# Drexubery/ViewCrafter

Measured on AMD Instinct MI355X. Metric: DDIM steps/sec (576x1024x25f latent 25x72x128, CFG 7.5, 50-step schedule), higher is better.
Workload: dtype f16; 1 GPU; ViewCrafter_25_576x1024x25; trajectories_per_gpu=1, frames=25, parallelism=trajectory-sharded x1 (no in-step collective)

## Files before the change

### include/vcx.h

```cpp
#ifndef VCX_H
#define VCX_H

#include <stddef.h>
#include <stdint.h>

#ifdef __cplusplus
extern "C" {
#endif

#define VCX_OK 0
#define VCX_EINVAL (-1)
#define VCX_ELAUNCH (-2)
#define VCX_ENODEV (-3)

#define VCX_ABI_VERSION 18

int vcx_abi_version(void);
const char* vcx_last_error(void);
int vcx_device_arch(char* name_host, int len);

#define VCX_GEMM_BIAS_N 0x1
#define VCX_GEMM_BIAS_M 0x2
#define VCX_GEMM_ROWADD 0x4
#define VCX_GEMM_RESIDUAL 0x8
#define VCX_GEMM_GEGLU 0x10
#define VCX_GEMM_OUT_F32 0x20
#define VCX_GEMM_CONV_SLABK 0x40
#define VCX_GEMM_LNFOLD 0x80
#define VCX_GEMM_LNFOLD_T 0x100
#define VCX_GEMM_COLSTATS 0x200
#define VCX_GEMM_ROWSTATS 0x400
#define VCX_GEMM_MXFP8_OUT 0x800

typedef struct vcx_gemm_desc {
    size_t struct_size;
    const void* A;
    const void* W;
    void* C;
    const float* bias;
    const float* rowadd;
    const void* residual;
    int64_t lda;
    int32_t M, N, K;
    int32_t ldw, ldc, ldr;
    int32_t mode;
    int32_t in_h, in_w, out_h, out_w, cin, kh, kw, stride, pad_h, pad_w, ups;
    int32_t rowadd_div;
    int32_t flags;
    float alpha;
    const float* ln_stats;
    const float* ln_colsum;
    float* colstats;
    int64_t ldcs;
    float* rowstats;
    float rowstats_eps;
    int32_t rowadd_ld;
    const void* tail_a0;
    const void* tail_a1;
    int64_t tail_lda0;
    int64_t tail_lda1;
    int32_t tail_k0;
    int32_t tail_k1;
} vcx_gemm_desc;

int vcx_gemm_f16(const vcx_gemm_desc* desc_host, void* stream);
int vcx_gemm_units_f16(const vcx_gemm_desc* desc_host, int unit_rows, int64_t w_unit_stride, int64_t bias_unit_stride, void* stream);

enum {
    VCX_ROUTE_REFUSED = 0,
    VCX_ROUTE_REGISTER = 1,
    VCX_ROUTE_TILED = 2,
    VCX_ROUTE_WS320 = 3,
    VCX_ROUTE_WS320_GEGLU = 4,
    VCX_ROUTE_WS320_LNF = 5,
    VCX_ROUTE_UNITS_WS320 = 6,
    VCX_ROUTE_UNITS_GROUPED = 7,
    VCX_ROUTE_UNITS_LOOP = 8
};
int vcx_gemm_route(const vcx_gemm_desc* desc_host, int unit_rows);

size_t vcx_groupnorm_ws_bytes(int n_outer, int64_t pixels, int groups);
int vcx_groupnorm_stats_f16(const void* x, float* stats, void* ws, int n_outer, int64_t pixels,
                            int C, int groups, void* stream);
int vcx_groupnorm_apply_f16(const void* x, void* y, const float* stats, const float* gamma,
                            const float* beta, int n_outer, int64_t pixels, int C, int groups,
                            float eps, int silu, void* stream);
int vcx_groupnorm_apply2_f16(const void* x1, int c1, const void* x2, void* y, const float* stats, const float* gamma, const float* beta,
                             int n_outer, int64_t pixels, int C, int groups, float eps, int silu, void* stream);
int vcx_groupnorm_stats_from_colstats_f32(const float* colstats, float* stats, void* ws, int n_outer, int64_t pixels, int C,
                                          int groups, void* stream);

int vcx_groupnorm_fold_linear_f16(const float* W, const float* bias, const float* gamma, const float* beta, const float* stats,
                                  void* Wn, float* bn, int n_outer, int N, int C, int groups, float eps, void* stream);

int vcx_rowstats_f16(const void* x, float* stats, int64_t rows, int C, float eps, void* stream);
int vcx_layernorm_f16(const void* x, void* y, const float* gamma, const float* beta,
                      int64_t rows, int C, float eps, void* stream);

int vcx_quant_mxfp8_f16(const void* x, int64_t ldx, void* q, void* scales, int64_t rows, int K, void* stream);
int vcx_layernorm_mxfp8_f16(const void* x, void* q, void* scales, const float* gamma, const float* beta, int64_t rows, int C, float eps,
                            void* stream);
int vcx_gemm_mxfp8(const void* a, const void* a_scales, const void* w, const void* w_scales, void* out, void* out_scales, const float* bias,
                   const void* residual, int64_t M, int64_t N, int64_t K, int64_t ldc, int64_t ldr, int flags, void* stream);
int vcx_gemm_mxfp8_ok(int64_t M, int64_t N, int64_t K, int flags);
int vcx_gemm_mxfp8_cfg(int64_t N, int flags, int gather_mode);
int vcx_groupnorm_apply_mxfp8_f16(const void* x, void* q, void* scales, const float* stats, const float* gamma, const float* beta, int n_outer,
                                  int64_t pixels, int C, int groups, float eps, int silu, void* stream);
int vcx_conv_t3_mxfp8(const void* a, const void* a_scales, const void* w, const void* w_scales, void* out, const float* bias, const void* residual,
                      float* colstats, int64_t B, int64_t T, int64_t P, int64_t Cin, int64_t N, int64_t ldc, int64_t ldr, int64_t ldcs, int flags,
                      void* stream);
int vcx_conv_t3_mxfp8_ok(int64_t B, int64_t T, int64_t P, int64_t Cin, int64_t N, int64_t ldc, int64_t ldr, int64_t ldcs, int64_t colstats_col,
                         int flags);
int vcx_groupnorm_apply2_mxfp8_f16(const void* x1, int c1, const void* x2, void* q, void* scales, const float* stats, const float* gamma,
                                   const float* beta, int n_outer, int64_t pixels, int C, int groups, float eps, int silu, void* stream);
// ... 109 lines not shown
```

### viewcrafter_amd/_lib.py

```python
import ctypes
import os
from ctypes import c_char_p, c_double, c_float, c_int, c_int32, c_int64, c_void_p, POINTER

_HERE = os.path.dirname(os.path.abspath(__file__))
LIB_PATH = os.path.join(_HERE, "libvcx.so")

SYMBOLS = [
    "vcx_abi_version", "vcx_last_error", "vcx_device_arch", "vcx_gemm_f16", "vcx_gemm_units_f16", "vcx_gemm_route", "vcx_quant_mxfp8_f16", "vcx_layernorm_mxfp8_f16", "vcx_gemm_mxfp8", "vcx_gemm_mxfp8_ok", "vcx_gemm_mxfp8_cfg",
    "vcx_groupnorm_apply_mxfp8_f16", "vcx_conv_t3_mxfp8", "vcx_conv_t3_mxfp8_ok",
    "vcx_groupnorm_apply2_mxfp8_f16", "vcx_conv3x3_mxfp8", "vcx_conv3x3_mxfp8_ok",
    "vcx_groupnorm_apply_mxfp8_raw_f16", "vcx_groupnorm_apply2_mxfp8_raw_f16", "vcx_conv3x3_tail_mxfp8", "vcx_conv3x3_tail_mxfp8_ok",
    "vcx_groupnorm_ws_bytes", "vcx_groupnorm_stats_f16", "vcx_groupnorm_apply_f16", "vcx_groupnorm_apply2_f16", "vcx_groupnorm_stats_from_colstats_f32", "vcx_groupnorm_fold_linear_f16", "vcx_layernorm_f16", "vcx_rowstats_f16",
    "vcx_attn_flash_d64_f16", "vcx_attn_flash_d512_f16", "vcx_attn_flash_dual_d64_f16", "vcx_attn_temporal_d64_f16", "vcx_attn_temporal_d64_masked_f16", "vcx_attn_temporal_d64_rel_f16",
    "vcx_attn_temporal_d64_mxfp8", "vcx_attn_temporal_d64_mxfp8_ok", "vcx_attn_flash_d64_mxfp8", "vcx_attn_flash_d64_mxfp8_ok",
    "vcx_attn_flash_dual_d64_mxfp8", "vcx_attn_flash_dual_d64_mxfp8_ok", "vcx_softmax_rows_f16",
    "vcx_silu_f32", "vcx_gelu_f16", "vcx_clip_preprocess_f32", "vcx_add_nchw_f32_to_nhwc_f16", "vcx_timestep_embedding_f32", "vcx_cast_f32_to_f16", "vcx_cast_f16_to_f32",
    "vcx_copy2d_f16", "vcx_avgpool2x2_f16", "vcx_upsample2x_f16", "vcx_ncthw_f32_to_nthwc_f16", "vcx_nthwc_to_ncthw_f32", "vcx_ddim_ws_bytes", "vcx_ddim_step_f32", "vcx_ddim_step3_f32",
    "vcx_dpmpp2m_step_f32", "vcx_profile_begin", "vcx_profile_end", "vcx_tune_set", "vcx_tune_get",
]

EXT_SYMBOLS = ["vcx_layernorm_pool2x2_f16", "vcx_layernorm_pool2x2_ok"]

ABI_VERSION = 18
TUNE = {"GEMM_CFG": (0, -1), "GEMM_DMA": (1, 1), "FLASH_QB": (2, 0), "XATTN_RESIDENT": (3, 1), "FLASH_IMPL": (4, 0), "EXP0": (5, 0),
        "EXP1": (6, 0), "GEMM_WS": (7, 1)}
GEMM_BIAS_N, GEMM_BIAS_M, GEMM_ROWADD, GEMM_RESIDUAL, GEMM_GEGLU, GEMM_OUT_F32, GEMM_CONV_SLABK = 1, 2, 4, 8, 16, 32, 64
GEMM_LNFOLD, GEMM_LNFOLD_T, GEMM_COLSTATS, GEMM_ROWSTATS, GEMM_MXFP8_OUT = 0x80, 0x100, 0x200, 0x400, 0x800
ROUTE_REFUSED, ROUTE_REGISTER, ROUTE_TILED, ROUTE_WS320, ROUTE_WS320_GEGLU, ROUTE_WS320_LNF, ROUTE_UNITS_WS320, ROUTE_UNITS_GROUPED, ROUTE_UNITS_LOOP = range(9)
PROF_FAMILIES = ("gemm", "flash_attn", "temporal_attn", "groupnorm", "layernorm", "elementwise")


class GemmDesc(ctypes.Structure):
    _fields_ = [
        ("struct_size", ctypes.c_size_t),
        ("A", c_void_p), ("W", c_void_p), ("C", c_void_p), ("bias", c_void_p), ("rowadd", c_void_p),
        ("residual", c_void_p), ("lda", c_int64), ("M", c_int32), ("N", c_int32), ("K", c_int32),
        ("ldw", c_int32), ("ldc", c_int32), ("ldr", c_int32), ("mode", c_int32),
        ("in_h", c_int32), ("in_w", c_int32), ("out_h", c_int32), ("out_w", c_int32), ("cin", c_int32),
        ("kh", c_int32), ("kw", c_int32), ("stride", c_int32), ("pad_h", c_int32), ("pad_w", c_int32),
        ("ups", c_int32), ("rowadd_div", c_int32), ("flags", c_int32), ("alpha", c_float),
        ("ln_stats", c_void_p), ("ln_colsum", c_void_p), ("colstats", c_void_p), ("ldcs", c_int64),
        ("rowstats", c_void_p), ("rowstats_eps", c_float), ("rowadd_ld", c_int32),
        ("tail_a0", c_void_p), ("tail_a1", c_void_p), ("tail_lda0", c_int64), ("tail_lda1", c_int64), ("tail_k0", c_int32), ("tail_k1", c_int32),
    ]

    def __init__(self, *args, **kw):
        super().__init__(*args, **kw)
        self.struct_size = ctypes.sizeof(GemmDesc)


_lib = None


class VcxError(RuntimeError):
    pass


def lib():
    global _lib
    if _lib is not None:
        return _lib
    if not os.path.exists(LIB_PATH):
        raise VcxError(
            f"{LIB_PATH} not found: build it with `make -C viewcrafter_amd/csrc` "
            "(or `python -c 'import __graft_entry__ as g; g.build()'`). There is no fallback path.")
    import torch
    L = ctypes.CDLL(LIB_PATH)
    L.vcx_abi_version.restype = c_int
    L.vcx_last_error.restype = c_char_p
    L.vcx_device_arch.argtypes = [c_char_p, c_int]
    L.vcx_gemm_f16.argtypes = [POINTER(GemmDesc), c_void_p]
    L.vcx_gemm_units_f16.argtypes = [POINTER(GemmDesc), c_int, c_int64, c_int64, c_void_p]
    L.vcx_gemm_route.argtypes = [POINTER(GemmDesc), c_int]
    L.vcx_quant_mxfp8_f16.argtypes = [c_void_p, c_int64, c_void_p, c_void_p, c_int64, c_int, c_void_p]
    L.vcx_layernorm_mxfp8_f16.argtypes = [c_void_p, c_void_p, c_void_p, c_void_p, c_void_p, c_int64, c_int, c_float, c_void_p]
    L.vcx_gemm_mxfp8.argtypes = [c_void_p, c_void_p, c_void_p, c_void_p, c_void_p, c_void_p, c_void_p, c_void_p, c_int64, c_int64, c_int64, c_int64,
                                 c_int64, c_int, c_void_p]
    L.vcx_gemm_mxfp8_ok.argtypes = [c_int64, c_int64, c_int64, c_int]
    L.vcx_gemm_mxfp8_cfg.argtypes = [c_int64, c_int, c_int]
    L.vcx_groupnorm_apply_mxfp8_f16.argtypes = [c_void_p, c_void_p, c_void_p, c_void_p, c_void_p, c_void_p, c_int, c_int64, c_int, c_int, c_float, c_int, c_void_p]
    L.vcx_conv_t3_mxfp8.argtypes = [c_void_p, c_void_p, c_void_p, c_void_p, c_void_p, c_void_p, c_void_p, c_void_p, c_int64, c_int64, c_int64, c_int64, c_int64,
                                    c_int64, c_int64, c_int64, c_int, c_void_p]
    L.vcx_conv_t3_mxfp8_ok.argtypes = [c_int64, c_int64, c_int64, c_int64, c_int64, c_int64, c_int64, c_int64, c_int64, c_int]
    L.vcx_groupnorm_apply2_mxfp8_f16.argtypes = [c_void_p, c_int, c_void_p, c_void_p, c_void_p, c_void_p, c_void_p, c_void_p, c_int, c_int64, c_int, c_int, c_float,
                                                 c_int, c_void_p]
    L.vcx_conv3x3_mxfp8.argtypes = [c_void_p, c_void_p, c_void_p, c_void_p, c_void_p, c_void_p, c_void_p, c_void_p, c_void_p, c_int64, c_int64, c_int64, c_int64,
                                    c_int64, c_int64, c_int64, c_int64, c_int64, c_int64, c_int, c_void_p]
    L.vcx_conv3x3_mxfp8_ok.argtypes = [c_int64, c_int64, c_int64, c_int64, c_int64, c_int64, c_int64, c_int64, c_int64, c_int64, c_int]
    L.vcx_groupnorm_apply_mxfp8_raw_f16.argtypes = [c_void_p, c_void_p, c_void_p, c_void_p, c_void_p, c_void_p, c_void_p, c_void_p, c_int, c_int64, c_int, c_int,
                                                    c_float, c_int, c_void_p]
    L.vcx_groupnorm_apply2_mxfp8_raw_f16.argtypes = [c_void_p, c_int, c_void_p, c_void_p, c_void_p, c_void_p, c_void_p, c_void_p, c_void_p, c_void_p, c_int, c_int64,
                                                     c_int, c_int, c_float, c_int, c_void_p]
    L.vcx_conv3x3_tail_mxfp8.argtypes = [c_void_p, c_void_p, c_void_p, c_void_p, c_void_p, c_void_p, c_void_p, c_void_p, c_void_p, c_int64, c_int64, c_int64,
                                         c_int64, c_int64, c_int64, c_int64, c_int64, c_int, c_void_p]
    L.vcx_conv3x3_tail_mxfp8_ok.argtypes = [c_int64, c_int64, c_int64, c_int64, c_int64, c_int64, c_int64, c_int64, c_int64, c_int]
    L.vcx_groupnorm_ws_bytes.argtypes = [c_int, c_int64, c_int]
    L.vcx_groupnorm_stats_f16.argtypes = [c_void_p, c_void_p, c_void_p, c_int, c_int64, c_int, c_int, c_void_p]
    L.vcx_groupnorm_apply_f16.argtypes = [c_void_p, c_void_p, c_void_p, c_void_p, c_void_p, c_int, c_int64, c_int,
                                          c_int, c_float, c_int, c_void_p]
    L.vcx_groupnorm_apply2_f16.argtypes = [c_void_p, c_int, c_void_p, c_void_p, c_void_p, c_void_p, c_void_p, c_int, c_int64, c_int,
                                           c_int, c_float, c_int, c_void_p]
    L.vcx_layernorm_f16.argtypes = [c_void_p, c_void_p, c_void_p, c_void_p, c_int64, c_int, c_float, c_void_p]
    L.vcx_rowstats_f16.argtypes = [c_void_p, c_void_p, c_int64, c_int, c_float, c_void_p]
    L.vcx_groupnorm_stats_from_colstats_f32.argtypes = [c_void_p, c_void_p, c_void_p, c_int, c_int64, c_int, c_int, c_void_p]
    L.vcx_groupnorm_fold_linear_f16.argtypes = [c_void_p, c_void_p, c_void_p, c_void_p, c_void_p, c_void_p, c_void_p, c_int, c_int, c_int, c_int,
                                                c_float, c_void_p]
    L.vcx_attn_flash_d64_f16.argtypes = [c_void_p, c_void_p, c_void_p, c_void_p, c_int, c_int, c_int, c_int, c_int,
                                         c_int, c_int64, c_int64, c_int64, c_int64, c_float, c_int, c_void_p]
    L.vcx_attn_flash_d512_f16.argtypes = [c_void_p, c_void_p, c_void_p, c_void_p, c_int, c_int, c_int, c_int, c_int64, c_int64, c_int64, c_int64, c_float, c_void_p]
    L.vcx_attn_flash_dual_d64_f16.argtypes = [c_void_p, c_void_p, c_void_p, c_void_p, c_void_p, c_void_p, c_int, c_int, c_int,
# ... 65 lines not shown
```

### viewcrafter_amd/csrc/gemm.hip

```cpp
#include "vcx_common.h"

#include "gemm_args.h"
#include <stdarg.h>
#include <stdlib.h>

using namespace vcxgemm;

namespace {

template <int BN, bool CONV, bool GEGLU, bool OUT_F32>
__global__ void __launch_bounds__(NTHREADS, 2) gemm_kernel(GemmArgs p) {
    constexpr int NFRAG = BN / 32;
    constexpr int WROWS = BN / 32;
    extern __shared__ __attribute__((aligned(16))) unsigned char smem_raw[];
    half_t* sX = reinterpret_cast<half_t*>(smem_raw);
    half_t* sW = sX + 2 * BM * BK;

    const int ntiles = p.tiles_m * p.tiles_n;
    const int G = gridDim.x;
    auto tile_coords = [&](int t, int& tm, int& tn) {
        const int q8 = ntiles >> 3, r8 = ntiles & 7;
        const int xcd = t & 7, idx = t >> 3;
        const int vid = (xcd < r8 ? xcd * (q8 + 1) : r8 * (q8 + 1) + (xcd - r8) * q8) + idx;
        tn = vid % p.tiles_n;
// ... 240 lines not shown
                }
                const bool full = (n0 + 4 <= p.N);
                if (full) {
                    if (flags & VCX_GEMM_BIAS_N) {
                        const f4 bv = *reinterpret_cast<const f4*>(p.bias + n0);
#pragma unroll
                        for (int r = 0; r < 4; ++r) v[r] += bv[r];
                    }
                    if (radd) {
                        const f4 rv = *reinterpret_cast<const f4*>(radd + n0);
#pragma unroll
                        for (int r = 0; r < 4; ++r) v[r] += rv[r];
                    }
                    if (flags & VCX_GEMM_RESIDUAL) {
                        const h4 rr = *reinterpret_cast<const h4*>(p.R + (int64_t)m * p.ldr + n0);
#pragma unroll
                        for (int r = 0; r < 4; ++r) v[r] += (float)rr[r];
                    }
                    if (OUT_F32) {
                        float* dst = reinterpret_cast<float*>(p.C) + (int64_t)m * p.ldc + n0;
                        *reinterpret_cast<f4*>(dst) = f4{v[0], v[1], v[2], v[3]};
                    } else {
                        half_t* dst = reinterpret_cast<half_t*>(p.C) + (int64_t)m * p.ldc + n0;
                        *reinterpret_cast<h4*>(dst) = h4{(half_t)v[0], (half_t)v[1], (half_t)v[2], (half_t)v[3]};
                    }
                } else {
                    for (int r = 0; r < 4 && n0 + r < p.N; ++r) {
                        float x = v[r];
                        if (flags & VCX_GEMM_BIAS_N) x += p.bias[n0 + r];
                        if (radd) x += radd[n0 + r];
                        if (flags & VCX_GEMM_RESIDUAL) x += (float)p.R[(int64_t)m * p.ldr + n0 + r];
                        if (OUT_F32)
                            reinterpret_cast<float*>(p.C)[(int64_t)m * p.ldc + n0 + r] = x;
                        else
                            reinterpret_cast<half_t*>(p.C)[(int64_t)m * p.ldc + n0 + r] = (half_t)x;
                    }
                }
            }
        }
    }
            }
#pragma unroll
            for (int a = 0; a < NFRAG; ++a)
#pragma unroll
                for (int b = 0; b < 4; ++b) acc[a][b] = f4{0.f, 0.f, 0.f, 0.f};
        }
        if (more) store_tile(cur ^ 1);
        __syncthreads();
        cur ^= 1;
        if (++ckt == nk) {
            ckt = 0;
            ctile += G;
            if (ctile >= ntiles) break;
            tile_coords(ctile, tile_m, tile_n);
        }
    }
}

}
static int grid_for(int ntiles, int blocks_per_cu, int ncu) {
    const int slots = blocks_per_cu * ncu;
    if (ntiles <= slots) return ntiles;
    const int rounds = (ntiles + slots - 1) / slots;
    int g = (ntiles + rounds - 1) / rounds;
    g = (g + 7) & ~7;
    return g < slots ? g : slots;
}
int vcxgemm::persistent_grid(int ntiles, int blocks_per_cu) {
    static std::atomic<int> cached{0};
    int ncu = cached.load(std::memory_order_relaxed);
    if (ncu == 0) {
        int dev = 0;
        hipDeviceProp_t prop;
        ncu = 256;
        if (hipGetDevice(&dev) == hipSuccess && hipGetDeviceProperties(&prop, dev) == hipSuccess && prop.multiProcessorCount > 0)
            ncu = prop.multiProcessorCount;
        cached.store(ncu, std::memory_order_relaxed);
    }
    return grid_for(ntiles, blocks_per_cu, ncu);
}

struct TileSeg { int cfg, m_begin, rows, grid; };
struct TilePlan { int n; TileSeg seg[2]; float cost; };
enum { EPI_PLAIN = 0, EPI_GEGLU = 1, EPI_PLAIN_ONLY128 = 2, EPI_GEGLU_ONLY128 = 3 };

struct TileCost {
    int tbm, tbn, bpc;
    float k_alone, k_share;
    float e;
};
static const TileCost TILE_COST[7] = {
    {128, 128, 2, 0.66f, 1.14f, 3.2f},
    {128, 160, 2, 0.70f, 1.16f, 2.8f},
    {256, 256, 1, 1.63f, 1.63f, 5.0f},
    {256, 320, 1, 2.05f, 2.05f, 5.4f},
    {64, 128, 2, 0.54f, 0.81f, 1.3f},
    {64, 64, 2, 0.46f, 0.73f, 1.3f},
    {64, 128, 2, 0.57f, 0.67f, 1.6f},
};
constexpr float LAUNCH_COST = 4.0f;

static int seg_tiles(int cfg, int rows, int N, int unit_rows) {
    const TileCost& t = TILE_COST[cfg];
    const int tiles_n = (N + t.tbn - 1) / t.tbn;
    if (unit_rows > 0) return (rows / unit_rows) * ((unit_rows + t.tbm - 1) / t.tbm) * tiles_n;
    return ((rows + t.tbm - 1) / t.tbm) * tiles_n;
}
static TileSeg plan_seg(int cfg, int m_begin, int rows, int N, int ncu, int unit_rows = 0) {
    return TileSeg{cfg, m_begin, rows, grid_for(seg_tiles(cfg, rows, N, unit_rows), TILE_COST[cfg].bpc, ncu)};
}
static float seg_cost(const TileSeg& g, int N, int K, int ncu, int unit_rows = 0) {
    const TileCost& t = TILE_COST[g.cfg];
    const int tiles = seg_tiles(g.cfg, g.rows, N, unit_rows);
    const int per_block = (tiles + g.grid - 1) / g.grid;
    const bool share = g.grid > ncu;
    return LAUNCH_COST + per_block * ((float)(K / BK) * (share ? t.k_share : t.k_alone) + t.e);
}

static TilePlan plan_tiles(int M, int N, int K, int epi, int ncu, int unit_rows = 0) {
    const bool geglu = epi == EPI_GEGLU || epi == EPI_GEGLU_ONLY128;
    const int small = (!geglu && N % 160 == 0) ? 1 : 0;
    const int big_bn = (N % 320 == 0 && !geglu) ? 320 : ((N % 256 == 0 || N >= 1024) ? 256 : 0);
    TilePlan best;
    auto consider = [&](int n, TileSeg a, TileSeg b, bool first) {
        const float c = seg_cost(a, N, K, ncu, unit_rows) + (n == 2 ? seg_cost(b, N, K, ncu, unit_rows) : 0.f);
        if (first || c < best.cost) best = TilePlan{n, {a, b}, c};
    };
    const TileSeg none{0, 0, 0, 0};
    consider(1, plan_seg(small, 0, M, N, ncu, unit_rows), none, true);
    if (!big_bn) return best;
    const int large = big_bn == 320 ? 3 : 2;
    const int tpu = unit_rows > 0 ? (unit_rows + 255) / 256 : 1, step_rows = unit_rows > 0 ? unit_rows : 256;
    const int tiles_m = unit_rows > 0 ? M / unit_rows * tpu : (M + 255) / 256, tiles_n = (N + big_bn - 1) / big_bn;
    const long long tiles = (long long)tiles_m * tiles_n;
    if (tiles < 384) return best;
    consider(1, plan_seg(large, 0, M, N, ncu, unit_rows), none, true);
    int tails[3], ntails = 0;
    tails[ntails++] = small;
    if (epi == EPI_PLAIN) { tails[ntails++] = 4; tails[ntails++] = 5; }
    if (epi == EPI_GEGLU) tails[ntails++] = 6;
    const long long full = tiles / ncu;
    for (long long r = full; r >= 1 && r >= full - 1; --r) {
        const int m1 = (int)(r * ncu / tiles_n / tpu) * step_rows;
        if (m1 <= 0 || m1 >= M) continue;
        for (int i = 0; i < ntails; ++i) consider(2, plan_seg(large, 0, m1, N, ncu, unit_rows), plan_seg(tails[i], m1, M - m1, N, ncu, unit_rows), false);
    }
    return best;
}

static TilePlan forced_plan(int M, int N, int cfg, bool geglu, int ncu) {
    TilePlan p{1, {plan_seg(cfg, 0, M, N, ncu), TileSeg{0, 0, 0, 0}}, 0.f};
    if (cfg == 2 || cfg == 3) {
        const TileCost& t = TILE_COST[cfg];
        const int tiles_n = (N + t.tbn - 1) / t.tbn;
        const long long tiles = (long long)((M + 255) / 256) * tiles_n;
        const long long full = tiles / ncu, rem = tiles % ncu;
        const int m1 = (int)(full * ncu / tiles_n) * 256;
        if (full >= 1 && rem > 0 && rem * 10 < (long long)ncu * 7 && m1 > 0 && m1 < M) {
            p.n = 2;
            p.seg[0] = plan_seg(cfg, 0, m1, N, ncu);
            p.seg[1] = plan_seg((geglu || N % 160 != 0) ? 0 : 1, m1, M - m1, N, ncu);
        }
    }
    return p;
}
namespace {

template <int BN, bool CONV, bool GEGLU, bool OUT_F32>
int launch(const GemmArgs& a, hipStream_t s) {
    constexpr size_t smem = (size_t)2 * (BM + BN) * BK * sizeof(half_t);
    static VcxLdsAttr lds;
    auto kern = gemm_kernel<BN, CONV, GEGLU, OUT_F32>;
    if (!lds.ensure(reinterpret_cast<const void*>(kern), (int)smem, "vcx_gemm_f16")) return VCX_ELAUNCH;
    const int nb = persistent_grid(a.tiles_m * a.tiles_n);
    hipLaunchKernelGGL(kern, dim3(nb), dim3(NTHREADS), smem, s, a);
    return vcx_check_launch("vcx_gemm_f16");
}

template <int BN>
int dispatch(const GemmArgs& a, bool conv, bool geglu, bool f32, hipStream_t s) {
    if (geglu) return conv ? launch<BN, true, true, false>(a, s) : launch<BN, false, true, false>(a, s);
    if (f32) return conv ? launch<BN, true, false, true>(a, s) : launch<BN, false, false, true>(a, s);
    return conv ? launch<BN, true, false, false>(a, s) : launch<BN, false, false, false>(a, s);
}

}



static int validate(const vcx_gemm_desc* d, bool ptrs) {
    VCX_REQUIRE(d != nullptr, "vcx_gemm_f16: null descriptor");
    VCX_REQUIRE(d->struct_size == sizeof(vcx_gemm_desc), "vcx_gemm_f16: descriptor struct_size %zu != %zu (sizeof(vcx_gemm_desc), ABI %d)",
                (size_t)d->struct_size, sizeof(vcx_gemm_desc), VCX_ABI_VERSION);
    VCX_REQUIRE(!ptrs || (d->A && d->W && d->C), "vcx_gemm_f16: null A/W/C");
    VCX_REQUIRE(d->M > 0 && d->N > 0 && d->K > 0, "vcx_gemm_f16: empty problem M=%d N=%d K=%d", d->M, d->N, d->K);
    VCX_REQUIRE(d->K % 8 == 0 && d->ldw % 8 == 0 && d->lda % 8 == 0,
                "vcx_gemm_f16: K (%d), ldw (%d), lda (%lld) must be multiples of 8", d->K, d->ldw, (long long)d->lda);
    VCX_REQUIRE(!ptrs || (((uintptr_t)d->A & 15) == 0 && ((uintptr_t)d->W & 15) == 0 && ((uintptr_t)d->C & 15) == 0),
                "vcx_gemm_f16: A/W/C must be 16-byte aligned");
    const int flags = d->flags;
    VCX_REQUIRE(!ptrs || !(flags & (VCX_GEMM_BIAS_N | VCX_GEMM_BIAS_M)) || d->bias, "vcx_gemm_f16: bias flag without bias");
    VCX_REQUIRE(!(flags & VCX_GEMM_ROWADD) || ((!ptrs || d->rowadd) && d->rowadd_div > 0 && (d->rowadd_ld == 0 || (d->rowadd_ld >= d->N && d->rowadd_ld % 4 == 0))),
                "vcx_gemm_f16: bad rowadd (rowadd_ld must be 0 or a multiple of 4 >= N)");
    VCX_REQUIRE(!ptrs || !(flags & VCX_GEMM_RESIDUAL) || d->residual, "vcx_gemm_f16: residual flag without pointer");
    const bool conv = d->mode == 1;
    const bool geglu = flags & VCX_GEMM_GEGLU;
    const bool f32 = flags & VCX_GEMM_OUT_F32;
    VCX_REQUIRE(!(flags & VCX_GEMM_CONV_SLABK) || (d->mode == 1 && d->cin % 64 == 0),
                "vcx_gemm_f16: VCX_GEMM_CONV_SLABK needs a convolution with cin %% 64 == 0 (cin=%d)", d->cin);
    VCX_REQUIRE(d->mode == 0 || d->mode == 1, "vcx_gemm_f16: unknown mode %d", d->mode);
    VCX_REQUIRE(!(geglu && (f32 || (flags & (VCX_GEMM_ROWADD | VCX_GEMM_RESIDUAL | VCX_GEMM_BIAS_M)))),
                "vcx_gemm_f16: GEGLU combines only with BIAS_N");
    VCX_REQUIRE(!geglu || d->N % 64 == 0, "vcx_gemm_f16: GEGLU needs N %% 64 == 0 (N=%d)", d->N);
    const int lnf = (flags & VCX_GEMM_LNFOLD) ? 1 : (flags & VCX_GEMM_LNFOLD_T) ? 2 : 0;
    if (lnf) {
        VCX_REQUIRE(!((flags & VCX_GEMM_LNFOLD) && (flags & VCX_GEMM_LNFOLD_T)), "vcx_gemm_f16: LNFOLD and LNFOLD_T are exclusive");
        VCX_REQUIRE(!ptrs || (d->ln_stats && d->ln_colsum && ((uintptr_t)d->ln_stats & 15) == 0 && ((uintptr_t)d->ln_colsum & 15) == 0),
                    "vcx_gemm_f16: LNFOLD needs 16-byte aligned ln_stats and ln_colsum");
        VCX_REQUIRE(!conv && !f32 && !(flags & VCX_GEMM_ROWADD), "vcx_gemm_f16: LNFOLD is for linear layers with fp16 output, without ROWADD");
        VCX_REQUIRE(lnf == 1 ? !(flags & VCX_GEMM_BIAS_M) : !(flags & VCX_GEMM_BIAS_N) && !geglu,
                    "vcx_gemm_f16: LNFOLD takes BIAS_N (and GEGLU), LNFOLD_T takes BIAS_M");
        VCX_REQUIRE((lnf == 1 ? d->N : d->M) % 4 == 0 && (lnf == 1 ? d->N : d->M) >= 4, "vcx_gemm_f16: LNFOLD needs the colsum side to be a multiple of 4");
    }
    if (flags & VCX_GEMM_COLSTATS) {
        VCX_REQUIRE(!ptrs || (d->colstats && ((uintptr_t)d->colstats & 15) == 0), "vcx_gemm_f16: COLSTATS needs a 16-byte aligned colstats buffer");
        VCX_REQUIRE(!geglu && !f32 && !lnf && d->M % 64 == 0 && d->N % 8 == 0,
                    "vcx_gemm_f16: COLSTATS is for fp16 outputs (no GEGLU / LNFOLD) with M %% 64 == 0 and N %% 8 == 0 (M=%d N=%d)", d->M, d->N);
        VCX_REQUIRE(d->ldcs == 0 || (d->ldcs >= d->N && d->ldcs % 2 == 0), "vcx_gemm_f16: COLSTATS ldcs (%lld) must be 0 or an even number >= N", (long long)d->ldcs);
    }
    if (conv) {
        VCX_REQUIRE(d->cin > 0 && d->cin % 8 == 0 && d->kh > 0 && d->kw > 0 && d->tail_k0 >= 0 && d->tail_k1 >= 0 &&
                        d->K == d->kh * d->kw * d->cin + d->tail_k0 + d->tail_k1,
                    "vcx_gemm_f16: conv needs cin %% 8 == 0 and K == kh*kw*cin + tail (cin=%d kh=%d kw=%d K=%d tail=%d+%d)", d->cin,
                    d->kh, d->kw, d->K, d->tail_k0, d->tail_k1);
        VCX_REQUIRE(d->out_h > 0 && d->out_w > 0 && d->in_h > 0 && d->in_w > 0 && d->stride > 0 &&
                        (d->ups == 0 || d->ups == 1 || d->ups == 2) && d->M % (d->out_h * d->out_w) == 0,
                    "vcx_gemm_f16: bad conv geometry");
        VCX_REQUIRE(d->ups != 2 || (d->kh == 2 && d->kw == 2 && d->stride == 1 && d->out_h == 2 * d->in_h && d->out_w == 2 * d->in_w && d->tail_k0 + d->tail_k1 == 0),
                    "vcx_gemm_f16: ups = 2 (folded nearest-2x + 3x3) is four 2x2 weight sets on the source grid: kh = kw = 2, stride 1, out = 2 x in, no K tail");
    }
    VCX_REQUIRE(conv || (d->tail_k0 >= 0 && d->tail_k1 >= 0 && d->tail_k0 + d->tail_k1 < d->K),
                "vcx_gemm_f16: a linear K tail needs tail_k >= 0 and K > tail_k0 + tail_k1 (K counts the tail; K=%d tail=%d+%d)", d->K, d->tail_k0, d->tail_k1);
    const int tail = d->tail_k0 + d->tail_k1;
    if (tail) {
        VCX_REQUIRE(d->tail_k0 % 64 == 0 && d->tail_k1 % 64 == 0 && (d->tail_k0 == 0 || ((!ptrs || d->tail_a0) && d->tail_lda0 >= d->tail_k0 && d->tail_lda0 % 8 == 0)) &&
                        (d->tail_k1 == 0 || ((!ptrs || d->tail_a1) && d->tail_lda1 >= d->tail_k1 && d->tail_lda1 % 8 == 0)) && !(d->tail_k0 == 0 && d->tail_k1 != 0),
                    "vcx_gemm_f16: K tail: tail_k %% 64 == 0, sources with tail_lda >= tail_k, tail_lda %% 8 == 0, tail_a0 first (tail=%d+%d)", d->tail_k0, d->tail_k1);
        VCX_REQUIRE((!ptrs || (((uintptr_t)d->tail_a0 | (uintptr_t)d->tail_a1) & 15) == 0) && (!conv || (!geglu && !f32 && !lnf)), "vcx_gemm_f16: K tail: 16-byte aligned sources, fp16 output, no GEGLU / LNFOLD");
    }
    if (!geglu) {
        VCX_REQUIRE(d->N < 4 || d->N % 4 != 0 || d->ldc % 4 == 0, "vcx_gemm_f16: ldc must be a multiple of 4");
        if (flags & VCX_GEMM_RESIDUAL)
            VCX_REQUIRE(d->ldr % 4 == 0 && (!ptrs || ((uintptr_t)d->residual & 7) == 0), "vcx_gemm_f16: residual alignment");
        if ((flags & VCX_GEMM_BIAS_N) && d->N >= 4) VCX_REQUIRE(!ptrs || ((uintptr_t)d->bias & 15) == 0, "vcx_gemm_f16: bias alignment");
        if (flags & VCX_GEMM_ROWADD) VCX_REQUIRE((!ptrs || ((uintptr_t)d->rowadd & 15) == 0) && d->N % 4 == 0, "vcx_gemm_f16: rowadd alignment");
    } else {
        VCX_REQUIRE(d->ldc % 4 == 0, "vcx_gemm_f16: ldc must be a multiple of 4");
    }
    if (flags & VCX_GEMM_ROWSTATS)
        VCX_REQUIRE((!ptrs || (d->rowstats && ((uintptr_t)d->rowstats & 7) == 0)) && d->rowstats_eps >= 0.f, "vcx_gemm_f16: ROWSTATS needs an 8-byte aligned rowstats buffer and eps >= 0");
    return VCX_OK;
}

static int validate_units(const vcx_gemm_desc* d, int unit_rows, int64_t w_unit_stride, int64_t bias_unit_stride, bool ptrs) {
    VCX_REQUIRE(d != nullptr && d->struct_size == sizeof(vcx_gemm_desc), "vcx_gemm_units_f16: null descriptor or wrong struct_size");
    VCX_REQUIRE((!ptrs || (d->A && d->W && d->C)) && d->M > 0 && d->N > 0 && d->K > 0, "vcx_gemm_units_f16: null A/W/C or empty problem");
    VCX_REQUIRE(d->mode == 0 && !(d->flags & ~(VCX_GEMM_BIAS_N | VCX_GEMM_ROWSTATS)), "vcx_gemm_units_f16: linear layers with a per-column bias (and ROWSTATS) at most (mode %d flags 0x%x)", d->mode, d->flags);
    VCX_REQUIRE(!(d->flags & VCX_GEMM_ROWSTATS) || ((!ptrs || (d->rowstats && ((uintptr_t)d->rowstats & 7) == 0)) && d->rowstats_eps >= 0.f), "vcx_gemm_units_f16: ROWSTATS needs an 8-byte aligned rowstats buffer and eps >= 0");
    VCX_REQUIRE(unit_rows > 0 && d->M % unit_rows == 0, "vcx_gemm_units_f16: M (%d) must be a whole number of units of %d rows", d->M, unit_rows);
    VCX_REQUIRE(w_unit_stride % 8 == 0 && bias_unit_stride % 4 == 0, "vcx_gemm_units_f16: unit strides must keep W 16-byte and bias 16-byte aligned");
    VCX_REQUIRE(!ptrs || !(d->flags & VCX_GEMM_BIAS_N) || d->bias, "vcx_gemm_units_f16: bias flag without bias");
    VCX_REQUIRE(d->lda % 8 == 0 && d->ldw % 8 == 0 && d->ldc % 8 == 0 && (!ptrs || ((((uintptr_t)d->A | (uintptr_t)d->W | (uintptr_t)d->C) & 15) == 0 && ((uintptr_t)d->bias & 15) == 0)),
                "vcx_gemm_units_f16: strides must be multiples of 8, pointers 16-byte aligned");
    return VCX_OK;
}

struct Knobs { int dma, ws, cfg; bool units_loop; };
static Knobs read_knobs(int unit_rows) {
    const char* loop_env = unit_rows > 0 ? getenv("VCX_GEMM_UNITS_LOOP") : nullptr;
    return Knobs{vcx_tune(VCX_TUNE_GEMM_DMA), vcx_tune(VCX_TUNE_GEMM_WS), vcx_tune(VCX_TUNE_GEMM_CFG), loop_env && loop_env[0] && loop_env[0] != '0'};
}

struct GemmRoute {
    int kind;
    int epi;
    bool ups_folded;
    unsigned long long a_bytes, w_bytes, c_bytes, r_bytes, a2_bytes, a3_bytes;
    char why[384];
};
static GemmRoute& take(GemmRoute& r, int kind) { r.kind = kind; return r; }
static GemmRoute& refuse(GemmRoute& r, const char* fmt, ...) {
    va_list ap;
    va_start(ap, fmt);
    vsnprintf(r.why, sizeof(r.why), fmt, ap);
    va_end(ap);
    return take(r, VCX_ROUTE_REFUSED);
}

static GemmRoute gemm_route(const vcx_gemm_desc& d, int unit_rows, const Knobs& k) {
    GemmRoute r;
    r.why[0] = 0;
    r.ups_folded = false;
    const int flags = d.flags;
    const bool conv = d.mode == 1, geglu = flags & VCX_GEMM_GEGLU, f32 = flags & VCX_GEMM_OUT_F32;
    const int lnf = (flags & VCX_GEMM_LNFOLD) ? 1 : (flags & VCX_GEMM_LNFOLD_T) ? 2 : 0;
    const int k2 = d.tail_k0, k3 = d.tail_k1;
    r.epi = geglu ? (conv ? EPI_GEGLU_ONLY128 : EPI_GEGLU) : ((f32 || lnf == 2) ? EPI_PLAIN_ONLY128 : EPI_PLAIN);
    const unsigned long long lim = 0xFFFF0000ull;
    r.a_bytes = conv ? 2ull * (unsigned long long)(d.M / (d.out_h * d.out_w)) * d.in_h * d.in_w * d.lda
                     : 2ull * ((unsigned long long)(d.M - 1) * d.lda + (d.K - k2 - k3));
    r.w_bytes = 2ull * ((unsigned long long)(d.N - 1) * d.ldw + d.K);
    const unsigned long long esz = f32 ? 4 : 2;
    r.c_bytes = esz * ((unsigned long long)(d.M - 1) * d.ldc + (geglu ? d.N / 2 : d.N));
    r.r_bytes = d.residual ? 2ull * ((unsigned long long)(d.M - 1) * d.ldr + d.N) : 0;
    const bool c_ok = esz * (unsigned long long)(d.M + 256) * d.ldc < lim;
    const bool out_ok = c_ok && 2ull * (unsigned long long)(d.M + 256) * d.ldr < lim;
    r.a2_bytes = k2 ? 2ull * ((unsigned long long)(d.M - 1) * d.tail_lda0 + k2) : 0;
    r.a3_bytes = k3 ? 2ull * ((unsigned long long)(d.M - 1) * d.tail_lda1 + k3) : 0;
    const bool dma_ok = k.dma != 0 && d.K % 64 == 0 && d.N % ((geglu || f32) ? 4 : 8) == 0 && (!conv || d.cin % 64 == 0) &&
                        r.a_bytes < lim && r.w_bytes < lim && (!geglu || d.N >= 64) && out_ok && r.a2_bytes < lim && r.a3_bytes < lim;
    const bool force_cfg_unset = k.cfg < 0;

    const int units = unit_rows > 0 ? d.M / unit_rows : 1;
    if (unit_rows > 0 && (k2 || k3)) return refuse(r, "vcx_gemm_units_f16: no K tail (tail_k0 / tail_k1) with per-unit weights");
    if (units > 1) {
        if (d.K == 320 && d.N == 320 && unit_rows % 32 == 0 && unit_rows >= 1024 && d.M >= 8192 && r.a_bytes < lim && c_ok && units <= 65535 &&
            k.dma != 0 && k.ws != 0 && force_cfg_unset)
            return take(r, VCX_ROUTE_UNITS_WS320);
        if (flags & VCX_GEMM_ROWSTATS)
            return refuse(r, "vcx_gemm_units_f16: ROWSTATS needs the one-launch weight-stationary form (N = K = 320, unit_rows %% 32 == 0, >= 1024, M >= 8192); M=%d N=%d K=%d unit_rows=%d",
                          d.M, d.N, d.K, unit_rows);
        if (units <= 65535 && d.K % 64 == 0 && d.N % 8 == 0 && r.a_bytes < lim && r.w_bytes < lim && c_ok && k.dma != 0 && k.cfg <= 5 && !k.units_loop) {
            vcx_gemm_desc one = d;
            one.M = unit_rows;
            if (gemm_route(one, 0, k).kind != VCX_ROUTE_WS320) return take(r, VCX_ROUTE_UNITS_GROUPED);
        }
        return take(r, VCX_ROUTE_UNITS_LOOP);
    }

    if (conv && d.ups == 2) {
        const long long hw = (long long)d.in_h * d.in_w;
        if (dma_ok && d.in_w % 16 == 0 && hw % 64 == 0 && d.cin % 64 == 0 && d.N % 8 == 0 && (flags & VCX_GEMM_CONV_SLABK) &&
            !(flags & ~(VCX_GEMM_CONV_SLABK | VCX_GEMM_BIAS_N | VCX_GEMM_COLSTATS)) && d.alpha == 1.0f && k.cfg <= 3 && 4ull * r.w_bytes < lim &&
            (unsigned long long)d.N * d.ldw * 2ull * 3ull + r.w_bytes < lim) {
            r.ups_folded = true;
            r.epi = EPI_PLAIN_ONLY128;
            return take(r, VCX_ROUTE_TILED);
        }
        return refuse(r, "vcx_gemm_f16: the folded upsample convolution (ups = 2) needs in_w %% 16 == 0, in_h in_w %% 64 == 0, cin %% 64 == 0, N %% 8 == 0, slab-major K, "
                         "a bias / column-moment epilogue, extents < 4 GiB, and GEMM_CFG <= 3; in %dx%d cin=%d N=%d flags=0x%x", d.in_h, d.in_w, d.cin, d.N, flags);
    }
    if ((k2 || k3) && !dma_ok)
        return refuse(r, "vcx_gemm_f16: a K tail needs the DMA kernel (cin %% 64 == 0, K %% 64 == 0, N %% 8 == 0, extents < 4 GiB); cin=%d K=%d N=%d", d.cin, d.K, d.N);
    if (!conv && (k2 || k3)) {
        if (geglu || f32 || lnf || (flags & VCX_GEMM_ROWSTATS))
            return refuse(r, "vcx_gemm_f16: a linear K tail takes the plain and COLSTATS epilogues only: no GEGLU / LNFOLD / ROWSTATS / fp32 output; flags=0x%x", flags);
        if (k.cfg > 5) return refuse(r, "vcx_gemm_f16: tile configuration %d (knob GEMM_CFG) has no K tail in linear mode", k.cfg);
        return take(r, VCX_ROUTE_TILED);
    }
    if (dma_ok && !conv && geglu && !f32 && !lnf && d.K == 320 && d.N % 256 == 0 && d.N <= 2560 && !(flags & ~(VCX_GEMM_GEGLU | VCX_GEMM_BIAS_N)) &&
        d.alpha == 1.0f && ((k.ws | 2) == 3 || k.ws == 5) && force_cfg_unset)
        return take(r, VCX_ROUTE_WS320_GEGLU);
    const int pad = (d.N + 255) / 256 * 256 - d.N;
    if (dma_ok && !conv && !geglu && !f32 && lnf == 1 && d.K == 320 && d.N % 64 == 0 && d.N <= 2560 &&
        ((k.ws >= 1 && k.ws <= 3 && pad <= 64 && d.N >= 512 && d.N <= 1536) || k.ws == 5) &&
        !(flags & ~(VCX_GEMM_LNFOLD | VCX_GEMM_BIAS_N)) && 8ull * (unsigned long long)d.M < lim && force_cfg_unset)
        return take(r, VCX_ROUTE_WS320_LNF);
    const bool rs_ok = !(flags & VCX_GEMM_ROWSTATS) || (d.N == 320 && !(flags & ~(VCX_GEMM_ROWSTATS | VCX_GEMM_BIAS_N | VCX_GEMM_RESIDUAL)) && 8ull * (unsigned long long)d.M < lim);
    if (dma_ok && !conv && !geglu && !f32 && !lnf && d.K == 320 && d.N % 320 == 0 && d.N <= 1280 && d.M >= 8192 && rs_ok &&
        !(flags & VCX_GEMM_BIAS_M) && k.ws != 0 && force_cfg_unset)
        return take(r, VCX_ROUTE_WS320);
    if (flags & VCX_GEMM_ROWSTATS)
        return refuse(r, "vcx_gemm_f16: ROWSTATS needs the weight-stationary kernel (linear, N = K = 320, M >= 8192, BIAS_N / RESIDUAL at most, knob GEMM_WS on); M=%d N=%d K=%d flags=0x%x",
                      d.M, d.N, d.K, flags);
    if (dma_ok) {
        if (k.cfg > 6) return refuse(r, "vcx_gemm_f16: unknown tile configuration %d (knob GEMM_CFG)", k.cfg);
        return take(r, VCX_ROUTE_TILED);
    }
    if (flags & VCX_GEMM_COLSTATS)
        return refuse(r, "vcx_gemm_f16: COLSTATS needs the DMA kernel (K / cin %% 64 == 0, extents < 4 GiB); K=%d cin=%d", d.K, d.cin);
    if (lnf) return refuse(r, "vcx_gemm_f16: LNFOLD needs the DMA kernel (K %% 64 == 0, N %% 8 == 0, extents < 4 GiB); K=%d N=%d", d.K, d.N);
    return take(r, VCX_ROUTE_REGISTER);
}

static GemmArgs fill_args(const vcx_gemm_desc& d, const GemmRoute& r, int unit_rows, int64_t w_unit_stride, int64_t bias_unit_stride) {
    GemmArgs a;
    a.A = (const half_t*)d.A; a.W = (const half_t*)d.W; a.C = d.C; a.bias = d.bias; a.rowadd = d.rowadd; a.R = (const half_t*)d.residual;
    a.lda = d.lda; a.M = d.M; a.N = d.N; a.K = d.K; a.ldw = d.ldw; a.ldc = d.ldc; a.ldr = d.ldr;
    a.in_h = d.in_h; a.in_w = d.in_w; a.out_h = d.out_h; a.out_w = d.out_w;
    a.cin = d.cin; a.kh = d.kh; a.kw = d.kw; a.stride = d.stride; a.pad_h = d.pad_h; a.pad_w = d.pad_w; a.ups = d.ups;
    a.rowadd_div = d.rowadd_div > 0 ? d.rowadd_div : 1;
    a.rowadd_ld = d.rowadd_ld > 0 ? d.rowadd_ld : d.N;
    a.flags = d.flags; a.alpha = d.alpha; a.m_begin = 0;
    const int bn = (!(d.flags & VCX_GEMM_GEGLU) && d.N % 160 == 0) ? 160 : 128;
    a.tiles_m = (d.M + BM - 1) / BM;
    a.tiles_n = (d.N + bn - 1) / bn;
    a.ln_stats = d.ln_stats; a.ln_colsum = d.ln_colsum; a.colstats = d.colstats; a.ldcs = d.ldcs > 0 ? d.ldcs : d.N;
    a.unit_rows = unit_rows; a.units = unit_rows > 0 ? d.M / unit_rows : 1; a.w_unit_stride = w_unit_stride; a.bias_unit_stride = bias_unit_stride;
    a.rowstats = d.rowstats; a.rowstats_eps = d.rowstats_eps;
    a.A2 = (const half_t*)d.tail_a0; a.A3 = (const half_t*)d.tail_a1; a.lda2 = d.tail_lda0; a.lda3 = d.tail_lda1;
    a.k2 = d.tail_k0; a.k3 = d.tail_k1;
    a.a_bytes = (unsigned)r.a_bytes; a.w_bytes = (unsigned)r.w_bytes; a.c_bytes = (unsigned)r.c_bytes; a.r_bytes = (unsigned)r.r_bytes;
    a.a2_bytes = (unsigned)r.a2_bytes; a.a3_bytes = (unsigned)r.a3_bytes;
    return a;
}

static TilePlan tile_plan(const vcx_gemm_desc& d, const GemmRoute& r, int force, int unit_rows) {
    const int ncu = persistent_grid(1 << 30, 1);
    const bool geglu = d.flags & VCX_GEMM_GEGLU;
    if (force < 0) return plan_tiles(d.M, d.N, d.K, r.epi, ncu, unit_rows);
    if (unit_rows > 0) return TilePlan{1, {plan_seg(force, 0, d.M, d.N, ncu, unit_rows), TileSeg{0, 0, 0, 0}}, 0.f};
    if (!(geglu && (force == 1 || force == 3))) return forced_plan(d.M, d.N, force, geglu, ncu);
    int cfg = 0;
    if ((d.N % 256 == 0 || d.N >= 1024) && (long long)((d.M + 255) / 256) * ((d.N + 255) / 256) >= 384) cfg = 2;
    return forced_plan(d.M, d.N, cfg, geglu, ncu);
}

static int run_plan(const GemmArgs& a, const TilePlan& plan, bool conv, hipStream_t s) {
    const bool trace = getenv("VCX_GEMM_PLAN_TRACE") != nullptr;
    for (int i = 0; i < plan.n; ++i) {
        const TileSeg& g = plan.seg[i];
        const TileCost& t = TILE_COST[g.cfg];
        const int u0 = a.unit_rows > 0 ? g.m_begin / a.unit_rows : 0, nu = a.unit_rows > 0 ? g.rows / a.unit_rows : 0;
        if (trace) {
            char per_unit[64] = "";
            if (a.unit_rows > 0) snprintf(per_unit, sizeof(per_unit), " units %d unit_rows %d", nu, a.unit_rows);
            fprintf(stderr, "[vcx] gemm plan M=%d N=%d K=%d seg %d/%d: cfg %d rows %d+%d grid %d%s\n", a.M, a.N, a.K, i + 1, plan.n, g.cfg, g.m_begin, g.rows, g.grid, per_unit);
        }
        GemmArgs c = a;
        c.m_begin = g.m_begin;
        c.M = g.m_begin + g.rows;
        c.tiles_m = a.unit_rows > 0 ? nu * ((a.unit_rows + t.tbm - 1) / t.tbm) : (g.rows + t.tbm - 1) / t.tbm;
        c.tiles_n = (a.N + t.tbn - 1) / t.tbn;
        if (a.unit_rows > 0) {
            c.units = nu;
            c.W = a.W + (int64_t)u0 * a.w_unit_stride;
            if (a.bias) c.bias = a.bias + (int64_t)u0 * a.bias_unit_stride;
        }
        const int rc = launch_dma(c, g.cfg, conv, a.flags & VCX_GEMM_GEGLU, a.flags & VCX_GEMM_OUT_F32, s, g.grid);
        if (rc) return rc;
    }
    return VCX_OK;
}

static int run(const vcx_gemm_desc& d, const GemmRoute& r, const Knobs& k, int unit_rows, int64_t w_unit_stride, int64_t bias_unit_stride, void* stream) {
    if (r.kind == VCX_ROUTE_REFUSED) {
        vcx_set_error("%s", r.why);
        return VCX_EINVAL;
    }
    if (unit_rows > 0 && r.kind != VCX_ROUTE_UNITS_WS320 && r.kind != VCX_ROUTE_UNITS_GROUPED) {
        for (int u = 0; u < d.M / unit_rows; ++u) {
            vcx_gemm_desc du = d;
            du.A = (const half_t*)d.A + (int64_t)u * unit_rows * d.lda;
            du.C = (half_t*)d.C + (int64_t)u * unit_rows * d.ldc;
            du.W = (const half_t*)d.W + (int64_t)u * w_unit_stride;
            if (d.bias) du.bias = d.bias + (int64_t)u * bias_unit_stride;
            du.M = unit_rows;
// ... 48 lines not shown
```

### viewcrafter_amd/csrc/gemm_dma.hip

```cpp
#include "gemm_epilogue.h"

using namespace vcxgemm;

namespace {

typedef __attribute__((address_space(3))) void* lds_ptr_t;
[[maybe_unused]] constexpr unsigned OOB = 0xFFFFFFFFu;

template <int TBM_, int TBN_, int NWM_, int NWN_>
struct TileCfg {
    static constexpr int TBM = TBM_, TBN = TBN_, NWM = NWM_, NWN = NWN_;
    static constexpr int THREADS = 64 * NWM * NWN;
    static constexpr int MF = TBM / NWM / 16;
    static constexpr int NF = TBN / NWN / 16;
    static constexpr int XROWS = TBM * 8 / THREADS;
    static constexpr int WROWS = TBN * 8 / THREADS;
    static constexpr int RSTEP = THREADS / 8;
    static constexpr size_t STAGES = (size_t)2 * (TBM + TBN) * BK * sizeof(half_t);
    static constexpr size_t STRIP = (size_t)TBN * NWM * sizeof(float);
    static constexpr size_t SMEM = STAGES + STRIP;
    static constexpr size_t SMEM_LNF = STAGES + 2 * STRIP;
};

template <class Cfg, bool CONV, bool GEGLU, bool OUT_F32, int LNF = 0, bool TAIL = false, bool UNITS = false, bool UPSF = false>
// ... 96 lines not shown
        half_t* dx = sX + buf * TBM * BK + wave * 8 * BK;
        half_t* dw = sW + buf * BN * BK + wave * 8 * BK;
        if (TAIL && (parts & 1) && kt >= nk_main) {
            const bool first = kt - nk_main < nk_a2;
            const __amdgpu_buffer_rsrc_t src = first ? srd_a2 : srd_a3;
            const long long ld2 = (first ? p.lda2 : p.lda3) * 2;
            const unsigned soff = (unsigned)(first ? kt - nk_main : kt - nk_main - nk_a2) * (BK * 2);
#pragma unroll
            for (int i = 0; i < XROWS; ++i) {
                const int r = r0 + RSTEP * i;
                const int m = lrow0 + r;
                const unsigned v = m < p.M ? (unsigned)((long long)m * ld2) + (unsigned)(chunk ^ ((r >> 1) & 7)) * 16u : OOB;
                __builtin_amdgcn_raw_ptr_buffer_load_lds(src, (lds_ptr_t)(dx + RSTEP * i * BK), 16, v, soff, 0, 0);
            }
        } else if (CONV && (parts & 1)) {
            if (!UPSF && p.ups) {
                const unsigned cb = (unsigned)ci0 * 2u, rowb = (unsigned)(p.in_w * (int)p.lda * 2), pixb = (unsigned)((int)p.lda * 2);
                const unsigned y0 = (unsigned)(tky >> 1) * rowb, y1 = (unsigned)((tky + 1) >> 1) * rowb;
                const unsigned x0 = (unsigned)(tkx >> 1) * pixb, x1 = (unsigned)((tkx + 1) >> 1) * pixb;
#pragma unroll
                for (int i = 0; i < XROWS; ++i) {
                    const unsigned ok = (xmask[i] >> tap) & 1u;
                    const unsigned oy_ = (xmask[i] >> 31) ? y1 : y0, ox_ = ((xmask[i] >> 30) & 1u) ? x1 : x0;
                    const unsigned v = ok ? xoff[i] + oy_ + ox_ + cb : OOB;
                    __builtin_amdgcn_raw_ptr_buffer_load_lds(srd_a, (lds_ptr_t)(dx + RSTEP * i * BK), 16, v, 0, 0, 0);
                }
            } else if (!(VCX_CONV_XSKIP_ABL && p.kw == 3 && tkx != 0)) {
#pragma unroll
                for (int i = 0; i < XROWS; ++i) {
                    const unsigned ok = (xmask[i] >> tap) & 1u;
                    const unsigned v = ok ? xoff[i] + tap_off : OOB;
                    __builtin_amdgcn_raw_ptr_buffer_load_lds(srd_a, (lds_ptr_t)(dx + RSTEP * i * BK), 16, v, 0, 0, 0);
                }
            }
            if (p.flags & VCX_GEMM_CONV_SLABK) {
                ++tap;
                if (++tkx == p.kw) { tkx = 0; ++tky; }
                if (tap == p.kh * p.kw) { tap = 0; tkx = 0; tky = 0; ci0 += BK; }
                tap_off = (unsigned)((tky * p.in_w + tkx) * (int)p.lda * 2 + ci0 * 2);
            } else {
                ci0 += BK;
                tap_off += BK * 2;
                if (ci0 == p.cin) {
                    ci0 = 0;
                    ++tap;
                    if (++tkx == p.kw) { tkx = 0; ++tky; }
                    tap_off = (unsigned)((tky * p.in_w + tkx) * (int)p.lda * 2);
                }
            }
        } else if (!CONV && (parts & 1)) {
            const unsigned soff = (unsigned)kt * (BK * 2);
#pragma unroll
            for (int i = 0; i < XROWS; ++i)
                __builtin_amdgcn_raw_ptr_buffer_load_lds(srd_a, (lds_ptr_t)(dx + RSTEP * i * BK), 16, xoff[i], soff, 0, 0);
        }
        if (parts & 2) {
            const unsigned soffw = (unsigned)kt * (BK * 2);
#pragma unroll
            for (int i = 0; i < WROWS; ++i)
                __builtin_amdgcn_raw_ptr_buffer_load_lds(PERUNIT ? srd_wu : srd_w, (lds_ptr_t)(dw + RSTEP * i * BK), 16, woff[i], soffw, 0, 0);
        }
    };

    const int wm = wave % Cfg::NWM, wn = wave / Cfg::NWM;
    const int lr = lane & 15, lg = lane >> 4;
    constexpr int WM = TBM / Cfg::NWM, WN = BN / Cfg::NWN;

    f4 acc[NFRAG][MFRAG];
#pragma unroll
    for (int a = 0; a < NFRAG; ++a)
#pragma unroll
        for (int b = 0; b < MFRAG; ++b) acc[a][b] = f4{0.f, 0.f, 0.f, 0.f};

    const int nk = p.K / BK;
    int ltile = blockIdx.x, lkt = 0;
    int ctile = blockIdx.x, ckt = 0;
    int tile_m, tile_n;
    tile_coords(ctile, ntiles, p.tiles_n, tile_m, tile_n);
    init_load(ltile);
    load_tile(0, 0);
    __builtin_amdgcn_s_waitcnt(0x0f70 | 0);
    __syncthreads();
    int cur = 0;
    for (;;) {
        if (++lkt == nk) {
            lkt = 0;
            ltile += G;
            if (ltile < ntiles) init_load(ltile);
        }
        const bool more = ltile < ntiles;
        const int late_parts = (CONV && Cfg::THREADS == 512 && wave >= 4) ? 3 : 0;
        if (more) load_tile(lkt, cur ^ 1, 3 & ~late_parts);
        const half_t* cx = sX + cur * TBM * BK;
        const half_t* cw = sW + cur * BN * BK;
        [[maybe_unused]] float ln_r0[LNF ? MFRAG : 1], ln_r1[LNF ? MFRAG : 1];
        if ((LNF == 1 || LNF == 2) && ckt == nk - 1) {
            const int mrow = p.m_begin + tile_m * TBM + wm * WM + lr;
#pragma unroll
            for (int b = 0; b < MFRAG; ++b) {
                const int mc = min(mrow + b * 16, p.M - 1);
                if (LNF == 1) {
                    const float2 st = reinterpret_cast<const float2*>(p.ln_stats)[mc];
                    ln_r0[b] = st.x;
                    ln_r1[b] = st.y;
                } else {
                    ln_r0[b] = p.ln_colsum[mc];
                    ln_r1[b] = (p.flags & VCX_GEMM_BIAS_M) ? p.bias[mc] : 0.f;
                }
            }
        }
        {
            constexpr bool NOREAD = (VCX_DMA_ABL & 8) != 0;
            h8 xf[MFRAG];
#pragma unroll
            for (int b = 0; b < MFRAG; ++b) xf[b] = *reinterpret_cast<const h8*>(cx + lds_off(wm * WM + b * 16 + lr, lg));
            h8 wcur = *reinterpret_cast<const h8*>(cw + lds_off(wn * WN + lr, lg));
            if (NOREAD) {
#pragma unroll
                for (int b = 0; b < MFRAG; ++b) asm volatile("" : "+v"(xf[b]));
                asm volatile("" : "+v"(wcur));
            }
#pragma unroll
            for (int kk = 0; kk < 2; ++kk) {
                if (kk == 1 && more && late_parts) load_tile(lkt, cur ^ 1, late_parts);
#pragma unroll
                for (int a = 0; a < NFRAG; ++a) {
                    h8 wnext = wcur;
                    if (NOREAD) asm volatile("" : "+v"(wnext));
                    else if (a + 1 < NFRAG) wnext = *reinterpret_cast<const h8*>(cw + lds_off(wn * WN + (a + 1) * 16 + lr, kk * 4 + lg));
                    else if (kk == 0) wnext = *reinterpret_cast<const h8*>(cw + lds_off(wn * WN + lr, 4 + lg));
#pragma unroll
                    for (int b = 0; b < MFRAG; ++b) {
                        acc[a][b] = __builtin_amdgcn_mfma_f32_16x16x32_f16(wcur, xf[b], acc[a][b], 0, 0, 0);
                        if (a == NFRAG - 1 && kk == 0 && !NOREAD)
                            xf[b] = *reinterpret_cast<const h8*>(cx + lds_off(wm * WM + b * 16 + lr, 4 + lg));
                    }
                    wcur = wnext;
                    __builtin_amdgcn_sched_barrier(0);
                }
            }
        }
        if (ckt == nk - 1) {
            float* sB = reinterpret_cast<float*>(smem_raw + Cfg::STAGES) + wave * WN;
            if constexpr (UNITS) {
                int cu, crow0;
                unit_of(tile_m, cu, crow0);
                GemmArgs q = p;
                q.m_begin = crow0;
                q.M = p.m_begin + (cu + 1) * p.unit_rows;
                q.bias = p.bias + (int64_t)cu * p.bias_unit_stride;
                q.c_bytes = (unsigned)(2ull * ((unsigned long long)(q.M - 1) * (unsigned)p.ldc + (unsigned)p.N));
                gemm_epilogue<Cfg, false, false, 0>(q, acc, 0, tile_n, wm, wn, lane, sB);
            } else if constexpr (UPSF) {
                int cu, crow0;
                unit_of(tile_m, cu, crow0);
                gemm_epilogue<Cfg, false, false, LNF, false, true>(p, acc, tile_m, tile_n, wm, wn, lane, sB, nullptr, nullptr, nullptr, nullptr, false, cls0 + cu,
                                                                   crow0 - (p.m_begin + cu * p.unit_rows));
            } else
            gemm_epilogue<Cfg, GEGLU, OUT_F32, LNF>(p, acc, tile_m, tile_n, wm, wn, lane, sB,
                                                    reinterpret_cast<float*>(smem_raw + Cfg::STAGES + Cfg::STRIP) + wave * WN, ln_r0, ln_r1);
#pragma unroll
            for (int a = 0; a < NFRAG; ++a)
#pragma unroll
                for (int b = 0; b < MFRAG; ++b) acc[a][b] = f4{0.f, 0.f, 0.f, 0.f};
        }
        if (!(VCX_DMA_ABL & 16)) {
            __builtin_amdgcn_s_waitcnt(0x0f70 | 0);
            __syncthreads();
        }
        cur ^= 1;
        if (++ckt == nk) {
            ckt = 0;
            ctile += G;
            if (ctile >= ntiles) break;
            tile_coords(ctile, ntiles, p.tiles_n, tile_m, tile_n);
        }
    }
#endif
}

template <class Cfg, bool CONV, bool GEGLU, bool OUT_F32, int LNF = 0, bool TAIL = false, bool UNITS = false, bool UPSF = false>
int launch(const GemmArgs& a, hipStream_t s, int grid) {
    static VcxLdsAttr lds;
    auto kern = gemm_dma_kernel<Cfg, CONV, GEGLU, OUT_F32, LNF, TAIL, UNITS, UPSF>;
    constexpr size_t smem = LNF ? Cfg::SMEM_LNF : Cfg::SMEM;
    if (!lds.ensure(reinterpret_cast<const void*>(kern), (int)smem, "vcx_gemm_f16(dma)")) return VCX_ELAUNCH;
    const int blocks_per_cu = Cfg::SMEM > 80 * 1024 ? 1 : 2;
    const int nb = grid > 0 ? grid : persistent_grid(a.tiles_m * a.tiles_n, blocks_per_cu);
    hipLaunchKernelGGL(kern, dim3(nb), dim3(Cfg::THREADS), smem, s, a, a.a_bytes, a.w_bytes);
    return vcx_check_launch("vcx_gemm_f16(dma)");
}

template <class Cfg>
int dispatch(const GemmArgs& a, bool conv, bool geglu, bool f32, hipStream_t s, int grid) {
    if (a.unit_rows > 0 && conv)
        return (a.flags & VCX_GEMM_COLSTATS) ? launch<Cfg, true, false, false, 3, false, false, true>(a, s, grid) : launch<Cfg, true, false, false, 0, false, false, true>(a, s, grid);
    if (a.unit_rows > 0)
        return launch<Cfg, false, false, false, 0, false, true>(a, s, grid);
    if (a.k2 + a.k3 > 0) {
        if (conv) return (a.flags & VCX_GEMM_COLSTATS) ? launch<Cfg, true, false, false, 3, true>(a, s, grid) : launch<Cfg, true, false, false, 0, true>(a, s, grid);
        return (a.flags & VCX_GEMM_COLSTATS) ? launch<Cfg, false, false, false, 3, true>(a, s, grid) : launch<Cfg, false, false, false, 0, true>(a, s, grid);
    }
    if (a.flags & (VCX_GEMM_LNFOLD | VCX_GEMM_LNFOLD_T)) {
        if (a.flags & VCX_GEMM_LNFOLD_T) return launch<Cfg, false, false, false, 2>(a, s, grid);
        if (!geglu) return launch<Cfg, false, false, false, 1>(a, s, grid);
        if constexpr (Cfg::NF % 4 == 0) return launch<Cfg, false, true, false, 1>(a, s, grid);
        vcx_set_error("vcx_gemm_f16(dma): GEGLU needs whole 64-column packed blocks per wave");
        return VCX_EINVAL;
    }
    if (a.flags & VCX_GEMM_COLSTATS)
        return conv ? launch<Cfg, true, false, false, 3>(a, s, grid) : launch<Cfg, false, false, false, 3>(a, s, grid);
    if (geglu) {
        if constexpr (Cfg::NF % 4 == 0) return conv ? launch<Cfg, true, true, false>(a, s, grid) : launch<Cfg, false, true, false>(a, s, grid);
        vcx_set_error("vcx_gemm_f16(dma): GEGLU needs whole 64-column packed blocks per wave");
        return VCX_EINVAL;
    }
    if (f32) return conv ? launch<Cfg, true, false, true>(a, s, grid) : launch<Cfg, false, false, true>(a, s, grid);
    return conv ? launch<Cfg, true, false, false>(a, s, grid) : launch<Cfg, false, false, false>(a, s, grid);
}

constexpr size_t TAIL_LDS = 54 * 1024;
constexpr size_t CU_LDS = 160 * 1024;
static_assert(2 * TAIL_LDS <= CU_LDS && 3 * TAIL_LDS > CU_LDS, "TAIL_LDS must cap the tail kernels at two blocks per CU");

template <class Cfg, bool CONV, bool GEGLU, int LNF = 0, bool TAIL = false, bool UNITS = false>
int launch_tail(const GemmArgs& a, hipStream_t s, int grid) {
    static VcxLdsAttr lds;
    auto kern = gemm_dma_kernel<Cfg, CONV, GEGLU, false, LNF, TAIL, UNITS>;
    constexpr size_t need = LNF ? Cfg::SMEM_LNF : Cfg::SMEM;
    constexpr size_t smem = need > TAIL_LDS ? need : TAIL_LDS;
    if (!lds.ensure(reinterpret_cast<const void*>(kern), (int)smem, "vcx_gemm_f16(dma tail)")) return VCX_ELAUNCH;
    const int nb = grid > 0 ? grid : persistent_grid(a.tiles_m * a.tiles_n, 2);
    hipLaunchKernelGGL(kern, dim3(nb), dim3(Cfg::THREADS), smem, s, a, a.a_bytes, a.w_bytes);
    return vcx_check_launch("vcx_gemm_f16(dma tail)");
}

template <class Cfg>
int dispatch_tail(const GemmArgs& a, bool conv, bool geglu, bool f32, hipStream_t s, int grid) {
    const bool cs = a.flags & VCX_GEMM_COLSTATS;
    if (f32 || (a.flags & VCX_GEMM_LNFOLD_T)) {
        vcx_set_error("vcx_gemm_f16(dma): the 64-row tile configurations have no fp32-output / LNFOLD_T epilogue");
        return VCX_EINVAL;
    }
    if (a.unit_rows > 0 && conv) {
        vcx_set_error("vcx_gemm_f16(dma): the 64-row tile configurations have no folded-upsample form");
        return VCX_EINVAL;
    }
    if constexpr (Cfg::NF % 4 == 0) {
        if (a.unit_rows > 0) {
            vcx_set_error("vcx_gemm_f16(dma): this 64-row tile configuration has no per-unit weight form");
            return VCX_EINVAL;
        }
        if (geglu && !conv && a.k2 + a.k3 == 0 && !cs)
            return (a.flags & VCX_GEMM_LNFOLD) ? launch_tail<Cfg, false, true, 1>(a, s, grid) : launch_tail<Cfg, false, true>(a, s, grid);
        vcx_set_error("vcx_gemm_f16(dma): this 64-row tile configuration is for GEGLU projections (linear) only");
        return VCX_EINVAL;
    } else {
        static_assert(Cfg::MF == 4, "COLSTATS: one moment strip per 64 rows of a wave");
        if (geglu) {
            vcx_set_error("vcx_gemm_f16(dma): GEGLU needs whole 64-column packed blocks per wave");
            return VCX_EINVAL;
        }
        if (a.unit_rows > 0) return launch_tail<Cfg, false, false, 0, false, true>(a, s, grid);
        if (a.k2 + a.k3 > 0) {
            if (conv) return cs ? launch_tail<Cfg, true, false, 3, true>(a, s, grid) : launch_tail<Cfg, true, false, 0, true>(a, s, grid);
            return cs ? launch_tail<Cfg, false, false, 3, true>(a, s, grid) : launch_tail<Cfg, false, false, 0, true>(a, s, grid);
        }
        if (a.flags & VCX_GEMM_LNFOLD) return launch_tail<Cfg, false, false, 1>(a, s, grid);
        if (cs) return conv ? launch_tail<Cfg, true, false, 3>(a, s, grid) : launch_tail<Cfg, false, false, 3>(a, s, grid);
        return conv ? launch_tail<Cfg, true, false>(a, s, grid) : launch_tail<Cfg, false, false>(a, s, grid);
    }
}

}

int vcxgemm::launch_dma(GemmArgs& a, int cfg, bool conv, bool geglu, bool f32, hipStream_t s, int grid) {
    switch (cfg) {
        case 0: return dispatch<TileCfg<128, 128, 2, 2>>(a, conv, geglu, f32, s, grid);
        case 1: return dispatch<TileCfg<128, 160, 2, 2>>(a, conv, geglu, f32, s, grid);
        case 2: return dispatch<TileCfg<256, 256, 4, 2>>(a, conv, geglu, f32, s, grid);
        case 3: return dispatch<TileCfg<256, 320, 4, 2>>(a, conv, geglu, f32, s, grid);
        case 4: return dispatch_tail<TileCfg<64, 128, 1, 4>>(a, conv, geglu, f32, s, grid);
        case 5: return dispatch_tail<TileCfg<64, 64, 1, 4>>(a, conv, geglu, f32, s, grid);
        case 6: return dispatch_tail<TileCfg<64, 128, 2, 2>>(a, conv, geglu, f32, s, grid);
    }
    vcx_set_error("vcx_gemm_f16(dma): unknown tile configuration %d", cfg);
    return VCX_EINVAL;
}
```

### viewcrafter_amd/csrc/gemm_epilogue.h

```cpp
#pragma once
#include "gemm_args.h"

namespace vcxgemm {

[[maybe_unused]] constexpr unsigned EPI_OOB = 0xFFFFFFFFu;
typedef unsigned epi_u4v __attribute__((ext_vector_type(4)));

template <class Cfg>
__device__ __forceinline__ void gemm_epilogue_fetch_residual(const GemmArgs& p, int tile_m, int tile_n, int wm, int wn, int lane,
                                                             epi_u4v (&out)[(Cfg::NF / 2 + Cfg::NF % 2) * Cfg::MF]) {
    constexpr int WM = Cfg::TBM / Cfg::NWM, WN = Cfg::TBN / Cfg::NWN, NPAIRF = Cfg::NF / 2, UNITS = NPAIRF + Cfg::NF % 2;
    typedef unsigned u2v __attribute__((ext_vector_type(2)));
    const int lr = lane & 15, lg = lane >> 4;
    const unsigned odd = lg & 1, half = lg >> 1;
    const __amdgpu_buffer_rsrc_t srd_r = __builtin_amdgcn_make_buffer_rsrc(const_cast<half_t*>(p.R), 0, (int)p.r_bytes, 0x00020000);
    const int mbase = p.m_begin + tile_m * Cfg::TBM + wm * WM + lr;
    const unsigned roff0 = ((unsigned)mbase * (unsigned)p.ldr + (unsigned)(tile_n * Cfg::TBN + wn * WN)) * 2u;
    const unsigned rstep = 32u * (unsigned)p.ldr;
#pragma unroll
    for (int b = 0; b < Cfg::MF; ++b)
#pragma unroll
        for (int u = 0; u < UNITS; ++u) {
            const int col = u < NPAIRF ? (2 * u + (int)odd) * 16 + (int)half * 8 : (2 * NPAIRF + (u - NPAIRF)) * 16 + lg * 4;
            const unsigned o = roff0 + (unsigned)b * rstep + (unsigned)col * 2u;
            if (u < NPAIRF) out[b * UNITS + u] = __builtin_amdgcn_raw_buffer_load_b128(srd_r, o, 0, 0);
            else {
                const u2v t = __builtin_amdgcn_raw_buffer_load_b64(srd_r, o, 0, 0);
                const unsigned t0 = t[0], t1 = t[1];
                out[b * UNITS + u] = epi_u4v{t0, t1, 0u, 0u};
            }
        }
}

template <class Cfg, bool GEGLU, bool OUT_F32, int LNF = 0, bool RPRE = false, bool UPSF = false>
__device__ __forceinline__ void gemm_epilogue(const GemmArgs& p, f4 (&acc)[Cfg::NF][Cfg::MF], int tile_m, int tile_n, int wm, int wn,
                                              int lane, float* sB, [[maybe_unused]] float* sS = nullptr,
                                              [[maybe_unused]] const float* ln_r0 = nullptr, [[maybe_unused]] const float* ln_r1 = nullptr,
                                              [[maybe_unused]] const epi_u4v* rpre = nullptr,
                                              bool strip_ready = false,
                                              [[maybe_unused]] int ups_cls = 0, [[maybe_unused]] int ups_q0 = 0) {
    constexpr int TBM = Cfg::TBM, BN = Cfg::TBN, NFRAG = Cfg::NF, MFRAG = Cfg::MF;
    constexpr int WM = TBM / Cfg::NWM, WN = BN / Cfg::NWN;
    [[maybe_unused]] constexpr unsigned OOB = EPI_OOB;
    const int lr = lane & 15, lg = lane >> 4;
    const int flags = p.flags;
    const int mbase = p.m_begin + tile_m * TBM + wm * WM + lr;
    const int nbase = tile_n * BN + wn * WN + lg * 4;
    if (GEGLU) {
        auto xfrag = [](int a) { return 4 * (a >> 1) + (a & 1); };
        f4 bx[NFRAG / 2 + 1], bg[NFRAG / 2 + 1];
        [[maybe_unused]] f4 sx[LNF ? NFRAG / 2 + 1 : 1], sg[LNF ? NFRAG / 2 + 1 : 1];
#pragma unroll
        for (int a = 0; a < NFRAG / 2; ++a) {
            const int nx = min(nbase + xfrag(a) * 16, p.N - 36);
            bx[a] = (flags & VCX_GEMM_BIAS_N) ? *reinterpret_cast<const f4*>(p.bias + nx) : f4{0.f, 0.f, 0.f, 0.f};
            bg[a] = (flags & VCX_GEMM_BIAS_N) ? *reinterpret_cast<const f4*>(p.bias + nx + 32) : f4{0.f, 0.f, 0.f, 0.f};
            if (LNF) {
                sx[a] = *reinterpret_cast<const f4*>(p.ln_colsum + nx);
                sg[a] = *reinterpret_cast<const f4*>(p.ln_colsum + nx + 32);
            }
        }
        typedef unsigned u2v __attribute__((ext_vector_type(2)));
        typedef unsigned u4v __attribute__((ext_vector_type(4)));
        const __amdgpu_buffer_rsrc_t srd_c = __builtin_amdgcn_make_buffer_rsrc(p.C, 0, (int)p.c_bytes, 0x00020000);
        constexpr int NOUT = NFRAG / 2;
        const int jstrip = tile_n * (BN / 2) + wn * (WN / 2);
        const unsigned coff0 = ((unsigned)mbase * (unsigned)p.ldc + (unsigned)jstrip) * 2u;
        const unsigned cstep = 32u * (unsigned)p.ldc;
        const unsigned odd = lg & 1, half = lg >> 1;
#pragma unroll
        for (int b = 0; b < MFRAG; ++b) {
            u2v packed[NOUT ? NOUT : 1];
            [[maybe_unused]] float rb = 0.f, qb = 0.f;
            if (LNF) {
                rb = p.alpha * ln_r1[b];
                qb = -rb * ln_r0[b];
            }
#pragma unroll
            for (int a = 0; a < NOUT; ++a) {
                half_t o[4];
#pragma unroll
                for (int r = 0; r < 4; ++r) {
                    float xv, gv;
                    if (LNF) {
                        xv = __builtin_fmaf(acc[xfrag(a)][b][r], rb, __builtin_fmaf(qb, sx[a][r], bx[a][r]));
                        gv = __builtin_fmaf(acc[xfrag(a) + 2][b][r], rb, __builtin_fmaf(qb, sg[a][r], bg[a][r]));
                    } else {
                        xv = acc[xfrag(a)][b][r] * p.alpha + bx[a][r];
                        gv = acc[xfrag(a) + 2][b][r] * p.alpha + bg[a][r];
                    }
                    o[r] = (half_t)(xv * gelu_erf(gv));
                }
                packed[a] = __builtin_bit_cast(u2v, h4{o[0], o[1], o[2], o[3]});
            }
            const unsigned crow = coff0 + (unsigned)b * cstep;
#pragma unroll
            for (int a = 0; a < NOUT; a += 2) {
                if (a + 1 < NOUT) {
                    const unsigned a0 = packed[a][0], a1 = packed[a][1], b0 = packed[a + 1][0], b1 = packed[a + 1][1];
                    const auto s0 = __builtin_amdgcn_permlane16_swap(a0, b0, false, false);
                    const auto s1 = __builtin_amdgcn_permlane16_swap(a1, b1, false, false);
                    const int col = (a + (int)odd) * 16 + (int)half * 8;
                    const int nx = tile_n * BN + wn * WN + xfrag(a + (int)odd) * 16;
                    const unsigned voff = nx + 48 <= p.N ? crow + (unsigned)col * 2u : OOB;
                    __builtin_amdgcn_raw_buffer_store_b128(u4v{s0[0], s1[0], s0[1], s1[1]}, srd_c, voff, 0, 0);
                } else {
                    const int nx = tile_n * BN + wn * WN + xfrag(a) * 16;
                    const unsigned voff = nx + 48 <= p.N ? crow + (unsigned)(a * 16 + lg * 4) * 2u : OOB;
                    __builtin_amdgcn_raw_buffer_store_b64(packed[a], srd_c, voff, 0, 0);
                }
            }
        }
    } else {
        constexpr int ES = OUT_F32 ? 4 : 2;
        const __amdgpu_buffer_rsrc_t srd_c = __builtin_amdgcn_make_buffer_rsrc(p.C, 0, (int)p.c_bytes, 0x00020000);
        const __amdgpu_buffer_rsrc_t srd_r = __builtin_amdgcn_make_buffer_rsrc(const_cast<half_t*>(p.R), 0, (int)p.r_bytes, 0x00020000);
        const unsigned cstep = 16u * (unsigned)p.ldc * ES, rstep = 32u * (unsigned)p.ldr;
        const bool has_res = flags & VCX_GEMM_RESIDUAL;
        const int m_first = p.m_begin + tile_m * TBM;
        const int radd_row = m_first / p.rowadd_div;
        const bool radd_tile = (flags & VCX_GEMM_ROWADD) && (min(m_first + TBM, p.M) - 1) / p.rowadd_div == radd_row;
        const bool per_row = (flags & VCX_GEMM_BIAS_M) || ((flags & VCX_GEMM_ROWADD) && !radd_tile);
        typedef unsigned u2v __attribute__((ext_vector_type(2)));
        typedef unsigned u4v __attribute__((ext_vector_type(4)));
        constexpr int NPAIRF = OUT_F32 ? 0 : NFRAG / 2;
        constexpr int UNITS = NPAIRF + (NFRAG - 2 * NPAIRF);
        constexpr int NUNIT = UNITS * MFRAG;
        constexpr int RDU = RPRE ? NUNIT : UNITS;
        const unsigned odd = lg & 1, half = lg >> 1;
        auto unit_col = [&](int u) { return u < NPAIRF ? (2 * u + (int)odd) * 16 + (int)half * 8 : (2 * NPAIRF + (u - NPAIRF)) * 16 + lg * 4; };
        const int nstrip = tile_n * BN + wn * WN;
        const unsigned coff0 = ((unsigned)mbase * (unsigned)p.ldc + (unsigned)nstrip) * ES;
        const unsigned roff0 = ((unsigned)mbase * (unsigned)p.ldr + (unsigned)nstrip) * 2u;
        u4v rr[RDU];
        auto fetch = [&](int i) {
            const int u = i % UNITS;
            const unsigned o = roff0 + (unsigned)(i / UNITS) * rstep + (unsigned)unit_col(u) * 2u;
            if (u < NPAIRF) rr[i % RDU] = __builtin_amdgcn_raw_buffer_load_b128(srd_r, o, 0, 0);
            else {
                const u2v t = __builtin_amdgcn_raw_buffer_load_b64(srd_r, o, 0, 0);
                const unsigned t0 = t[0], t1 = t[1];
                rr[i % RDU] = u4v{t0, t1, 0u, 0u};
            }
        };
        if (RPRE) {
#pragma unroll
            for (int i = 0; i < RDU; ++i) rr[i] = rpre[i];
        } else if (has_res) {
#pragma unroll
            for (int i = 0; i < RDU; ++i) fetch(i);
        }
        if (lane < WN / 4 && !strip_ready) {
            const int nc = min(nstrip + lane * 4, p.N - 4);
            if (LNF == 2) {
                const f4 s01 = *reinterpret_cast<const f4*>(p.ln_stats + 2 * nc), s23 = *reinterpret_cast<const f4*>(p.ln_stats + 2 * nc + 4);
                f4 cs = {p.alpha * s01[1], p.alpha * s01[3], p.alpha * s23[1], p.alpha * s23[3]};
                f4 cq = {-cs[0] * s01[0], -cs[1] * s01[2], -cs[2] * s23[0], -cs[3] * s23[2]};
                asm volatile("" : "+v"(cs), "+v"(cq));
                *reinterpret_cast<f4*>(sB + lane * 4) = cs;
                *reinterpret_cast<f4*>(sS + lane * 4) = cq;
                asm volatile("" : : "v"(cs), "v"(cq));
            } else {
                f4 t = (flags & VCX_GEMM_BIAS_N) ? *reinterpret_cast<const f4*>(p.bias + nc) : f4{0.f, 0.f, 0.f, 0.f};
                if (radd_tile) {
                    const f4 rv = *reinterpret_cast<const f4*>(p.rowadd + (int64_t)radd_row * p.rowadd_ld + nc);
#pragma unroll
                    for (int r = 0; r < 4; ++r) t[r] += rv[r];
                }
                *reinterpret_cast<f4*>(sB + lane * 4) = t;
                if (LNF == 1) *reinterpret_cast<f4*>(sS + lane * 4) = *reinterpret_cast<const f4*>(p.ln_colsum + nc);
            }
        }
        constexpr bool FOLD = LNF == 1 || LNF == 2;
        [[maybe_unused]] float ln_a[FOLD ? MFRAG : 1], ln_b[FOLD ? MFRAG : 1];
        if (FOLD) {
#pragma unroll
            for (int b = 0; b < MFRAG; ++b) {
                if (LNF == 1) {
                    ln_a[b] = p.alpha * ln_r1[b];
                    ln_b[b] = -ln_a[b] * ln_r0[b];
                } else {
                    ln_a[b] = ln_r0[b];
                    ln_b[b] = ln_r1[b];
                }
            }
        }
        [[maybe_unused]] float gs[LNF == 3 ? UNITS : 1][8], gq[LNF == 3 ? UNITS : 1][8], gk[LNF == 3 ? UNITS : 1][2];
        if (LNF == 3) {
#pragma unroll
            for (int u = 0; u < UNITS; ++u)
#pragma unroll
                for (int e = 0; e < 8; ++e) gs[u][e] = gq[u][e] = 0.f;
        }
        int bopaque = 0;
        auto finish = [&](int a, int b, float (&v)[4]) {
            if (FOLD) {
                const f4 t = *reinterpret_cast<const f4*>(sB + bopaque + a * 16 + lg * 4);
                const f4 u = *reinterpret_cast<const f4*>(sS + bopaque + a * 16 + lg * 4);
                typedef float f2v __attribute__((ext_vector_type(2)));
                f2v la = {ln_a[b], ln_a[b]}, lb = {ln_b[b], ln_b[b]};
                asm volatile("" : "+v"(la), "+v"(lb));
#pragma unroll
                for (int r = 0; r < 4; ++r)
                    v[r] = LNF == 1 ? __builtin_fmaf(acc[a][b][r], la[r & 1], __builtin_fmaf(lb[r & 1], u[r], t[r]))
                                    : __builtin_fmaf(acc[a][b][r], t[r], __builtin_fmaf(u[r], la[r & 1], lb[r & 1]));
            } else if (per_row) {
                const int mc = min(mbase + b * 16, p.M - 1);
                f4 t = *reinterpret_cast<const f4*>(sB + bopaque + a * 16 + lg * 4);
                if (flags & VCX_GEMM_ROWADD) {
                    const f4 rv = *reinterpret_cast<const f4*>(p.rowadd + (int64_t)(mc / p.rowadd_div) * p.rowadd_ld + min(nbase + a * 16, p.N - 4));
#pragma unroll
                    for (int r = 0; r < 4; ++r) t[r] += rv[r];
                }
#pragma unroll
                for (int r = 0; r < 4; ++r) v[r] = __builtin_fmaf(acc[a][b][r], p.alpha, t[r]);
                if (flags & VCX_GEMM_BIAS_M) {
                    const float bm = p.bias[mc];
#pragma unroll
                    for (int r = 0; r < 4; ++r) v[r] += bm;
                }
            } else {
                const f4 t = *reinterpret_cast<const f4*>(sB + bopaque + a * 16 + lg * 4);
#pragma unroll
                for (int r = 0; r < 4; ++r) v[r] = __builtin_fmaf(acc[a][b][r], p.alpha, t[r]);
            }
        };
#pragma unroll
        for (int b = 0; b < MFRAG; ++b) {
            unsigned crow = coff0 + (unsigned)b * cstep;
            [[maybe_unused]] bool fvalid = true;
            if constexpr (UPSF) {
                const int qf = ups_q0 + wm * WM + b * 16;
                const int hw = p.out_h * p.out_w;
                fvalid = qf < p.unit_rows;
                const int qc = fvalid ? qf : 0;
                const int img = qc / hw, rem = qc - img * hw;
                const int i = rem / p.out_w, j0 = rem - i * p.out_w;
                const unsigned pix = ((unsigned)img * 2u * (unsigned)p.out_h + 2u * (unsigned)i + (unsigned)(ups_cls >> 1)) * 2u * (unsigned)p.out_w + 2u * (unsigned)j0 + (unsigned)(ups_cls & 1);
                crow = ((pix + 2u * (unsigned)lr) * (unsigned)p.ldc + (unsigned)nstrip) * ES;
            }
            asm volatile("" : "+v"(bopaque));
#pragma unroll
            for (int u = 0; u < UNITS; ++u) {
                const int i = b * UNITS + u;
                const bool wide = u < NPAIRF;
                const int a = wide ? 2 * u : 2 * NPAIRF + (u - NPAIRF);
                const unsigned voff = (nstrip + unit_col(u) < p.N && (!UPSF || fvalid)) ? crow + (unsigned)unit_col(u) * ES : OOB;
                float v0[4], v1[4] = {0.f, 0.f, 0.f, 0.f};
                finish(a, b, v0);
                if (wide) finish(a + 1, b, v1);
                if (has_res) {
                    const u4v raw = rr[i % RDU];
                    if (i + RDU < NUNIT) fetch(i + RDU);
                    unsigned w0 = raw[0], w1 = raw[1], w2 = raw[2], w3 = raw[3];
                    if (wide) {
                        const auto s0 = __builtin_amdgcn_permlane16_swap(w0, w2, false, false);
                        const auto s1 = __builtin_amdgcn_permlane16_swap(w1, w3, false, false);
                        w0 = s0[0]; w2 = s0[1]; w1 = s1[0]; w3 = s1[1];
                    }
                    const h4 r0 = __builtin_bit_cast(h4, u2v{w0, w1});
                    const h4 r1 = __builtin_bit_cast(h4, u2v{w2, w3});
#pragma unroll
                    for (int r = 0; r < 4; ++r) { v0[r] += (float)r0[r]; v1[r] += (float)r1[r]; }
                }
                [[maybe_unused]] const h4 o0 = {(half_t)v0[0], (half_t)v0[1], (half_t)v0[2], (half_t)v0[3]};
                [[maybe_unused]] const h4 o1 = {(half_t)v1[0], (half_t)v1[1], (half_t)v1[2], (half_t)v1[3]};
                [[maybe_unused]] u2v pk0 = __builtin_bit_cast(u2v, o0), pk1 = __builtin_bit_cast(u2v, o1);
                if (LNF == 3) {
                    unsigned q0 = pk0[0], q1 = pk0[1], q2 = pk1[0], q3 = pk1[1];
                    asm volatile("" : "+v"(q0), "+v"(q1), "+v"(q2), "+v"(q3));
                    pk0 = u2v{q0, q1};
                    pk1 = u2v{q2, q3};
                    typedef _Float16 h2v __attribute__((ext_vector_type(2)));
                    const h2v a01 = __builtin_bit_cast(h2v, q0), a23 = __builtin_bit_cast(h2v, q1);
                    const h2v b01 = __builtin_bit_cast(h2v, q2), b23 = __builtin_bit_cast(h2v, q3);
                    const float w0[4] = {(float)a01[0], (float)a01[1], (float)a23[0], (float)a23[1]};
                    const float w1[4] = {(float)b01[0], (float)b01[1], (float)b23[0], (float)b23[1]};
                    if (b == 0) {
                        gk[u][0] = __builtin_bit_cast(float, __builtin_amdgcn_update_dpp(0, __builtin_bit_cast(int, w0[0]), 0x150, 0xf, 0xf, true));
                        gk[u][1] = __builtin_bit_cast(float, __builtin_amdgcn_update_dpp(0, __builtin_bit_cast(int, w1[0]), 0x150, 0xf, 0xf, true));
                    }
#pragma unroll
                    for (int r = 0; r < 4; ++r) {
                        const float d0 = w0[r] - gk[u][0], d1 = w1[r] - gk[u][1];
                        gs[u][r] += d0;
                        gq[u][r] = __builtin_fmaf(d0, d0, gq[u][r]);
                        gs[u][4 + r] += d1;
                        gq[u][4 + r] = __builtin_fmaf(d1, d1, gq[u][4 + r]);
                    }
                }
                if (OUT_F32) {
                    __builtin_amdgcn_raw_buffer_store_b128(__builtin_bit_cast(u4v, f4{v0[0], v0[1], v0[2], v0[3]}), srd_c, voff, 0, 0);
                } else {
                    const u2v p0 = pk0;
                    if (wide) {
                        const u2v p1 = pk1;
                        const unsigned a0 = p0[0], a1 = p0[1], b0 = p1[0], b1 = p1[1];
                        const auto s0 = __builtin_amdgcn_permlane16_swap(a0, b0, false, false);
                        const auto s1 = __builtin_amdgcn_permlane16_swap(a1, b1, false, false);
                        __builtin_amdgcn_raw_buffer_store_b128(u4v{s0[0], s1[0], s0[1], s1[1]}, srd_c, voff, 0, 0);
                    } else {
                        __builtin_amdgcn_raw_buffer_store_b64(p0, srd_c, voff, 0, 0);
                    }
                }
            }
        }
        if (LNF == 3) {
            auto row_sum = [](float x) {
                x += __builtin_bit_cast(float, __builtin_amdgcn_update_dpp(0, __builtin_bit_cast(int, x), 0x140, 0xf, 0xf, true));
                x += __builtin_bit_cast(float, __builtin_amdgcn_update_dpp(0, __builtin_bit_cast(int, x), 0x141, 0xf, 0xf, true));
                x += __builtin_bit_cast(float, __builtin_amdgcn_update_dpp(0, __builtin_bit_cast(int, x), 0x4E, 0xf, 0xf, true));
                x += __builtin_bit_cast(float, __builtin_amdgcn_update_dpp(0, __builtin_bit_cast(int, x), 0xB1, 0xf, 0xf, true));
                return x;
            };
            int strip = (p.m_begin + tile_m * TBM + wm * WM) >> 6;
            [[maybe_unused]] bool svalid = true;
            if constexpr (UPSF) {
                static_assert(!UPSF || WM == 64, "UPSF column moments: one strip per 64 rows of a wave");
                const int qs = ups_q0 + wm * WM, s64 = (p.out_h * p.out_w) >> 6;
                svalid = qs < p.unit_rows;
                const int qq = svalid ? qs >> 6 : 0;
                const int img = qq / s64;
                strip = img * 4 * s64 + ups_cls * s64 + (qq - img * s64);
            }
            float* dst = p.colstats + ((size_t)strip * (size_t)p.ldcs + nstrip) * 2;
#pragma unroll
            for (int u = 0; u < UNITS; ++u) {
                float mo[8], qo[8];
#pragma unroll
                for (int e = 0; e < 8; ++e) {
                    const float s1 = row_sum(gs[u][e]), s2 = row_sum(gq[u][e]);
                    mo[e] = gk[u][e >> 2] + s1 * (1.0f / 64.0f);
                    qo[e] = __builtin_fmaf(-s1 * (1.0f / 64.0f), s1, s2);
                }
                if (lr == 0 && (UPSF ? svalid : strip * 64 < p.M)) {
                    const bool wide = u < NPAIRF;
                    const int c0 = wide ? (2 * u) * 16 + lg * 4 : (2 * NPAIRF + (u - NPAIRF)) * 16 + lg * 4;
                    if (nstrip + c0 < p.N) {
                        *reinterpret_cast<f4*>(dst + c0 * 2) = f4{mo[0], qo[0], mo[1], qo[1]};
                        *reinterpret_cast<f4*>(dst + c0 * 2 + 4) = f4{mo[2], qo[2], mo[3], qo[3]};
                    }
                    if (wide && nstrip + c0 + 16 < p.N) {
                        *reinterpret_cast<f4*>(dst + (c0 + 16) * 2) = f4{mo[4], qo[4], mo[5], qo[5]};
                        *reinterpret_cast<f4*>(dst + (c0 + 16) * 2 + 4) = f4{mo[6], qo[6], mo[7], qo[7]};
                    }
                }
            }
        }
    }
}

}
```

### viewcrafter_amd/lvdm/modules/attention.py

```python
import math
import os

import torch
from torch import nn

from ... import ops
from ...packing import fold_layernorm, pack_ff_out_folded, pack_geglu, pack_mxfp8
from ..common import default
from .flow import GN_STATS_LEVEL, out_kwargs


def _f16(t):
    return t.detach().to(torch.float16).contiguous()


def _f32(t):
    return t.detach().to(torch.float32).contiguous()


FOLD_LAYERNORM = os.environ.get("VCX_LN_FOLD", "1") != "0"
FOLD_LAYERNORM_FF = os.environ.get("VCX_LN_FOLD_FF", "1") != "0"
FOLD_LAYERNORM_FF_MIN_DIM = int(os.environ.get("VCX_LN_FOLD_FF_MIN_DIM", "640"))
FF_MXFP8 = os.environ.get("VCX_FF_MXFP8", "0") == "1"
FF_MXFP8_SKIP_DIMS = frozenset(int(v) for v in os.environ.get("VCX_FF_MXFP8_SKIP_DIMS", "320").split(",") if v.strip())
TATTN_MXFP8 = os.environ.get("VCX_TATTN_MXFP8", "0") == "1"
TATTN_MXFP8_SKIP_DIMS = frozenset(int(v) for v in os.environ.get("VCX_TATTN_MXFP8_SKIP_DIMS", "320").split(",") if v.strip())
SATTN_MXFP8 = os.environ.get("VCX_SATTN_MXFP8", "0") == "1"
SATTN_MXFP8_SKIP_DIMS = frozenset(int(v) for v in os.environ.get("VCX_SATTN_MXFP8_SKIP_DIMS", "320").split(",") if v.strip())
_KV_POOL_MODES = {"mean": ops.POOL_MEAN, "nearest": ops.POOL_NEAREST}


def _parse_kv_pool(value):
    if value in ("", "0"):
        return None
    if value not in _KV_POOL_MODES:
        raise ValueError(f"VCX_SATTN_KV_POOL={value!r}: expected 0 (off), mean or nearest")
    return value


SATTN_KV_POOL = _parse_kv_pool(os.environ.get("VCX_SATTN_KV_POOL", "0"))
SATTN_KV_POOL_MIN_TOKENS = int(os.environ.get("VCX_SATTN_KV_POOL_MIN_TOKENS", "4096"))


def kv_pool_plan(H, W, C):
    if SATTN_KV_POOL is None or H % 2 or W % 2 or H * W < SATTN_KV_POOL_MIN_TOKENS or (H // 2) * (W // 2) % 8:
        return None
    if not ops.layer_norm_pool2x2_ok(1, H, W, C, _KV_POOL_MODES[SATTN_KV_POOL]):
        return None
    return H // 2, W // 2

FF_OUT_FOLD = os.environ.get("VCX_FF_OUT_FOLD", "1") != "0"
FF_OUT_FOLD_SKIP_DIMS = frozenset(int(v) for v in os.environ.get("VCX_FF_OUT_FOLD_SKIP_DIMS", "1280").split(",") if v.strip())


GN_FOLD = os.environ.get("VCX_GN_FOLD", "1") != "0"
GN_FOLD_MIN_BYTES = int(os.environ.get("VCX_GN_FOLD_MIN_BYTES", str(16 << 20)))
GN_FOLD_SPATIAL = {"0": 0, "2": 2}.get(os.environ.get("VCX_GN_FOLD_SPATIAL", "1"), 1)


def spatial_fold_ok(n, pixels, C, D):
    if (GN_FOLD and GN_FOLD_SPATIAL == 2 and n > 1 and pixels % 8 == 0 and 2 * n * pixels * C >= GN_FOLD_MIN_BYTES and fold_extent_ok(n * pixels, max(C, D))
            and ops.units_route(n * pixels, D, C, pixels) == "grouped"):
        return True
    return (GN_FOLD and GN_FOLD_SPATIAL and C == 320 and D == 320 and pixels % 32 == 0 and pixels >= 1024 and n * pixels >= 8192
            and 2 * n * pixels * C >= GN_FOLD_MIN_BYTES and fold_extent_ok(n * pixels, C) and ops.tune_get("GEMM_DMA") != 0
            and ops.tune_get("GEMM_WS") != 0 and ops.tune_get("GEMM_CFG") < 0)


def fold_extent_ok(rows, C):
    return 2 * (rows + 256) * C < 0xFFFF0000


def _folded(pj, rows, K, lda, transposed=False):
    return pj["colsum"] is not None and ops.lnfold_ok(rows, pj["w"].shape[0], K, lda=lda, transposed=transposed)


def _ln_projection(w, ln, alpha=1.0, bias=None):
    if ln is not None:
        wf, colsum, bias_f = fold_layernorm(w, ln.weight, ln.bias, None)
        bias_f = bias_f * alpha
        if bias is not None:
            bias_f = bias_f + bias.detach().float()
        return dict(w=wf, colsum=colsum, bias=bias_f.contiguous(), eps=ln.eps, _src=(w, bias), _plain=None)
    return dict(w=_f16(w), colsum=None, bias=None if bias is None else _f32(bias), eps=None)


def _plain_of(pj):
    if pj["_plain"] is None:
        w, bias = pj["_src"]
        with torch.no_grad():
            pj["_plain"] = (_f16(w), None if bias is None else _f32(bias))
    return pj["_plain"]


def ln_linear(t, pj, lnp, alpha=1.0, stats=None, **kw):
    rows, K = t.shape
    if pj["colsum"] is not None and ops.lnfold_ok(rows, pj["w"].shape[0], K, lda=t.stride(0)):
        st = stats if stats is not None else ops.row_stats(t, lnp[2])
        return ops.linear(t, pj["w"], pj["bias"], alpha=alpha, ln_stats=st, ln_colsum=pj["colsum"], **kw)
    w, bias = (pj["w"], pj["bias"]) if pj["colsum"] is None else _plain_of(pj)
    return ops.linear(ops.layer_norm(t, *lnp), w, bias, alpha=alpha, **kw)


def ln_linear_t(t, pj, lnp, stats=None):
    tokens, K = t.shape
    D = pj["w"].shape[0]
    if pj["colsum"] is not None and ops.lnfold_ok(tokens, D, K, lda=t.stride(0), transposed=True):
        st = stats if stats is not None else ops.row_stats(t, lnp[2])
        return ops.gemm(pj["w"], t, M=D, N=tokens, K=K, lda=K, ldw=t.stride(0), bias=pj["bias"], bias_m=True, ln_stats=st,
                        ln_colsum=pj["colsum"], ln_t=True)
    w, bias = (pj["w"], pj["bias"]) if pj["colsum"] is None else _plain_of(pj)
    return ops.gemm(w, ops.layer_norm(t, *lnp), M=D, N=tokens, K=K, lda=K, bias=bias, bias_m=bias is not None)


def _sig(tensors):
    return tuple((p.data_ptr(), p._version) for p in tensors)


class PackedModule(nn.Module):

    def __init__(self):
        super().__init__()
        self._pk = None
        self._pk_sig = None
        self.register_load_state_dict_post_hook(lambda module, incompatible: module._drop_packed())

    def _drop_packed(self):
        self._pk = None

    def _apply(self, fn, recurse=True):
        self._pk = None
        return super()._apply(fn, recurse)

    def _foreign_params(self):
        pre = getattr(self, "_pre_norm", None)
        return [pre[0].weight, pre[0].bias] if pre else []

    def packed(self):
        foreign = self._foreign_params()
        if self._pk is not None and foreign and _sig(foreign) != self._pk_sig:
            self._pk = None
        if self._pk is None:
            with torch.no_grad():
                self._pk = self._pack()
            self._pk_sig = _sig(foreign)
        return self._pk

    def _pack(self):
        raise NotImplementedError


class RelativePosition(nn.Module):

    def __init__(self, num_units, max_relative_position):
        super().__init__()
        self.num_units, self.max_relative_position = num_units, max_relative_position
        self.embeddings_table = nn.Parameter(torch.empty(max_relative_position * 2 + 1, num_units))
        nn.init.xavier_uniform_(self.embeddings_table)


class CrossAttention(PackedModule):

    def __init__(self, query_dim, context_dim=None, heads=8, dim_head=64, dropout=0., relative_position=False,
                 temporal_length=None, video_length=None, image_cross_attention=False, image_cross_attention_scale=1.0,
                 image_cross_attention_scale_learnable=False, text_context_len=77):
        super().__init__()
        if relative_position and (temporal_length is None or 2 * temporal_length + 1 > 64 or context_dim is not None):
            raise NotImplementedError("relative_position: temporal self-attention with temporal_length <= 31 (2R + 1 table rows in 64 slots)")
        if image_cross_attention_scale_learnable:
            raise NotImplementedError("image_cross_attention_scale_learnable is not used by the ViewCrafter configs")
        if dim_head != 64:
            raise NotImplementedError(f"libvcx attention kernels are built for head dim 64 (got {dim_head})")
        if image_cross_attention and image_cross_attention_scale != 1.0:
            raise NotImplementedError("image_cross_attention_scale != 1.0 (the dual-softmax kernel sums the two outputs unweighted; "
                                      "the ViewCrafter configs keep the constant 1.0, attention.py:62)")
        inner_dim = dim_head * heads
        self.is_self = context_dim is None
        context_dim = default(context_dim, query_dim)
        self.scale = dim_head ** -0.5
        self.heads, self.dim_head, self.inner_dim = heads, dim_head, inner_dim
        self.to_q = nn.Linear(query_dim, inner_dim, bias=False)
        self.to_k = nn.Linear(context_dim, inner_dim, bias=False)
# ... 25 lines not shown
            pk["qkv"] = _ln_projection(torch.cat([wq, wk, wv], 0), ln)
        else:
            pk["qk"] = _ln_projection(torch.cat([wq, wk], 0), ln, alpha=math.sqrt(self.scale * ops.LOG2E))
            pk["v"] = _ln_projection(wv, ln)
        if self.image_cross_attention:
            pk["wk_ip"], pk["wv_ip"] = _f16(self.to_k_ip.weight), _f16(self.to_v_ip.weight)
        if self.relative_position:
            ek, ev = self.relative_position_k.embeddings_table.detach(), self.relative_position_v.embeddings_table.detach()
            wk_rel = torch.zeros((64, 64), dtype=torch.float32, device=ek.device)
            wv_rel = torch.zeros((64, 64), dtype=torch.float32, device=ek.device)
            wk_rel[:ek.shape[0]] = ek.float()
            wv_rel[:, :ev.shape[0]] = ev.float().t()
            pk["rel_k"], pk["rel_v"], pk["rel_R"] = _f16(wk_rel), _f16(wv_rel), self.relative_position_k.max_relative_position
        return pk

    def mx_packed(self):
        pk = self.packed()
        if "mx" not in pk:
            with torch.no_grad():
                wq, wk, wv = self.to_q.weight.detach().float(), self.to_k.weight.detach().float(), self.to_v.weight.detach().float()
                zeros = lambda n: torch.zeros(n, dtype=torch.float32, device=wq.device)
                if self.kind == "temporal":
                    wqkv = _f16(torch.cat([self.to_q.weight.detach(), self.to_k.weight.detach(), self.to_v.weight.detach()], 0))
                    mx = dict(wqkv=pack_mxfp8(wqkv), zero=zeros(wqkv.shape[0]))
                elif self.is_self:
                    wqk = _f16(torch.cat([wq, wk], 0) * math.sqrt(self.scale * ops.LOG2E))
                    mx = dict(wqk=pack_mxfp8(wqk), wv=pack_mxfp8(_f16(wv)), zero=zeros(wqk.shape[0]))
                else:
                    wq2 = _f16(wq * (self.scale * ops.LOG2E))
                    mx = dict(wq=pack_mxfp8(wq2), zero=zeros(wq2.shape[0]))
                pk["mx"] = dict(mx, wo=pack_mxfp8(pk["wo"]), bo=pk["bo"])
        return pk["mx"]

    def kv_pool_packed(self):
        pk = self.packed()
        if "kv_pool" not in pk:
            with torch.no_grad():
                ln = self._pre_norm[0] if pk["qk"]["colsum"] is not None else None
                pv = pk["v"]
                pk["kv_pool"] = dict(q=_ln_projection(self.to_q.weight.detach(), ln, alpha=math.sqrt(self.scale * ops.LOG2E)),
                                     wk=_f16(self.to_k.weight), wv=pv["w"] if pv["colsum"] is None else _plain_of(pv)[0])
        return pk["kv_pool"]

    def forward(self, *args, **kwargs):
        raise RuntimeError("CrossAttention is driven by SpatialTransformer/TemporalTransformer in this package")


class GEGLU(nn.Module):
    def __init__(self, dim_in, dim_out):
        super().__init__()
        self.proj = nn.Linear(dim_in, dim_out * 2)


class FeedForward(PackedModule):

    def __init__(self, dim, dim_out=None, mult=4, glu=False, dropout=0.):
        super().__init__()
        if not glu:
            raise NotImplementedError("only the gated (GEGLU) feed-forward is on the ViewCrafter path")
        inner_dim = int(dim * mult)
        dim_out = default(dim_out, dim)
        self.net = nn.Sequential(GEGLU(dim, inner_dim), nn.Dropout(dropout), nn.Linear(inner_dim, dim_out))
        self.dim = dim
        self._pre_norm = None

    def _pack(self):
        proj = self.net[0].proj
        ln = self._pre_norm[0] if (self._pre_norm and FOLD_LAYERNORM and FOLD_LAYERNORM_FF and self.dim % 64 == 0 and self.dim >= FOLD_LAYERNORM_FF_MIN_DIM) else None
        p1 = _ln_projection(proj.weight.detach(), ln, bias=proj.bias)
        w1, b1 = pack_geglu(p1["w"], p1["bias"])
        colsum = None if p1["colsum"] is None else pack_geglu(p1["w"], p1["colsum"])[1]
        return dict(w1=w1, b1=b1, colsum=colsum, w2=_f16(self.net[2].weight), b2=_f32(self.net[2].bias))

    def _mx_ok(self, t):
        proj, out = self.net[0].proj, self.net[2]
        rows = t.shape[0]
        return (self.dim not in FF_MXFP8_SKIP_DIMS and t.is_contiguous() and proj.bias is not None and out.bias is not None
                and ops.linear_mxfp8_ok(rows, proj.out_features, self.dim, geglu=True, mx_out=True)
                and ops.linear_mxfp8_ok(rows, out.out_features, out.in_features, residual=True))

    def on_fp16_route(self, t):
        return not (FF_MXFP8 and self._mx_ok(t))

    def glu(self, t, ln_params):
        pk = self.packed()
        if pk["colsum"] is not None and ops.lnfold_ok(t.shape[0], pk["w1"].shape[0], t.shape[1], lda=t.stride(0)):
            return ops.linear(t, pk["w1"], pk["b1"], geglu=True, ln_stats=ops.row_stats(t, ln_params[2]), ln_colsum=pk["colsum"])
        if pk["colsum"] is not None and "w1_plain" not in pk:
            proj = self.net[0].proj
            pk["w1_plain"], pk["b1_plain"] = pack_geglu(_f16(proj.weight), _f32(proj.bias))
        w1, b1 = (pk["w1"], pk["b1"]) if pk["colsum"] is None else (pk["w1_plain"], pk["b1_plain"])
        return ops.linear(ops.layer_norm(t, *ln_params), w1, b1, geglu=True)

    def run(self, t, ln_params):
        pk = self.packed()
        if FF_MXFP8 and self._mx_ok(t):
            if "mx" not in pk:
                proj = self.net[0].proj
                w1, b1 = pack_geglu(_f16(proj.weight), _f32(proj.bias))
                pk["mx"] = dict(w1=pack_mxfp8(w1), b1=b1, w2=pack_mxfp8(pk["w2"]))
            mx = pk["mx"]
            a = ops.layer_norm_mxfp8(t, *ln_params)
            g = ops.linear_mxfp8(a, mx["w1"], mx["b1"], K=self.dim, geglu=True, mx_out=True)
            return ops.linear_mxfp8(g, mx["w2"], pk["b2"], K=pk["w2"].shape[1], residual=t)
        return ops.linear(self.glu(t, ln_params), pk["w2"], pk["b2"], residual=t)


class BasicTransformerBlock(PackedModule):

    def __init__(self, dim, n_heads, d_head, dropout=0., context_dim=None, gated_ff=True, checkpoint=True,
                 disable_self_attn=False, attention_cls=None, video_length=None, image_cross_attention=False,
                 image_cross_attention_scale=1.0, image_cross_attention_scale_learnable=False, text_context_len=77):
        super().__init__()
        if disable_self_attn:
            raise NotImplementedError("disable_self_attn is not used by the ViewCrafter configs")
        attn_cls = CrossAttention if attention_cls is None else attention_cls
        self.attn1 = attn_cls(query_dim=dim, heads=n_heads, dim_head=d_head, dropout=dropout, context_dim=None)
        self.ff = FeedForward(dim, dropout=dropout, glu=gated_ff)
        self.attn2 = attn_cls(query_dim=dim, context_dim=context_dim, heads=n_heads, dim_head=d_head, dropout=dropout,
                              video_length=video_length, image_cross_attention=image_cross_attention,
                              image_cross_attention_scale=image_cross_attention_scale,
                              image_cross_attention_scale_learnable=image_cross_attention_scale_learnable,
                              text_context_len=text_context_len)
        self.image_cross_attention = image_cross_attention
        self.norm1 = nn.LayerNorm(dim)
        self.norm2 = nn.LayerNorm(dim)
        self.norm3 = nn.LayerNorm(dim)
        self.checkpoint = checkpoint
        self.attn1._pre_norm, self.attn2._pre_norm, self.ff._pre_norm = [self.norm1], [self.norm2], [self.norm3]

    def set_kind(self, kind):
        self.attn1.kind = self.attn2.kind = kind

    def _drop_packed(self):
        super()._drop_packed()
        for m in (self.attn1, self.attn2, self.ff):
            m._drop_packed()

    def _pack(self):
        return [(_f32(n.weight), _f32(n.bias), n.eps) for n in (self.norm1, self.norm2, self.norm3)]

    def ln_params(self):
        return self.packed()


def ff_proj_out(tr, t, ln_params, xin, kw, video_rows):
    pk, ff = tr.packed(), tr.transformer_blocks[-1].ff
    tokens, D = t.shape
    C = pk["wout"].shape[0]
    fold = (FF_OUT_FOLD and t.is_cuda and D not in FF_OUT_FOLD_SKIP_DIMS and ff.net[2].bias is not None and ff.on_fp16_route(t)
            and all(ops.linear_tail_ok(m, C, ff.net[2].in_features, [D], ldc=kw.get("ldc"), residual=True, colstats="colstats" in kw)
                    for m in sorted({video_rows, tokens})))
    if not fold:
        return ops.linear(ff.run(t, ln_params), pk["wout"], pk["bout"], residual=xin, **kw)
    if "wcat" not in pk:
        pk["wcat"], pk["bcat"] = pack_ff_out_folded(ff.net[2].weight, ff.net[2].bias, pk["wout"], pk["bout"])
    return ops.linear(ff.glu(t, ln_params), pk["wcat"], pk["bcat"], tail=[t], residual=xin, **kw)


def _last_ff_params(tr):
    ff2 = tr.transformer_blocks[-1].ff.net[2]
    return [ff2.weight] + ([] if ff2.bias is None else [ff2.bias])


class ContextKV:
    __slots__ = ("k_txt", "vt_txt", "k_img", "vt_img", "n_txt_rows", "n_txt", "n_img", "img_per_frame")


def project_context(attn2, ctx):
    pk = attn2.packed()
    kv = ContextKV()
    txt = ctx["txt"]
    D = txt.shape[1]
    C = attn2.inner_dim
    kv.k_txt = ops.linear(txt, pk["wk"])
    kv.vt_txt = ops.gemm(pk["wv"], txt, M=C, N=txt.shape[0], K=D, lda=D)
    kv.n_txt_rows = txt.shape[0]
    kv.n_txt = int(ctx.get("n_txt", attn2.text_context_len))
    kv.k_img = kv.vt_img = None
    kv.n_img, kv.img_per_frame = ctx.get("n_img", 0), ctx.get("per_frame", False)
    if attn2.image_cross_attention and ctx.get("img") is not None:
        img = ctx["img"]
        kv.k_img = ops.linear(img, pk["wk_ip"])
        kv.vt_img = ops.gemm(pk["wv_ip"], img, M=C, N=img.shape[0], K=D, lda=D)
    return kv


class SpatialTransformer(PackedModule):

    def __init__(self, in_channels, n_heads, d_head, depth=1, dropout=0., context_dim=None, use_checkpoint=True,
                 disable_self_attn=False, use_linear=False, video_length=None, image_cross_attention=False,
                 image_cross_attention_scale_learnable=False):
        super().__init__()
        self.in_channels = in_channels
        inner_dim = n_heads * d_head
        self.n_heads = n_heads
        self.norm = nn.GroupNorm(num_groups=32, num_channels=in_channels, eps=1e-6, affine=True)
        self.proj_in = nn.Linear(in_channels, inner_dim) if use_linear else nn.Conv2d(in_channels, inner_dim, kernel_size=1, stride=1, padding=0)
        self.transformer_blocks = nn.ModuleList([
            BasicTransformerBlock(inner_dim, n_heads, d_head, dropout=dropout, context_dim=context_dim,
                                  disable_self_attn=disable_self_attn, checkpoint=use_checkpoint, attention_cls=None,
                                  video_length=video_length, image_cross_attention=image_cross_attention,
                                  image_cross_attention_scale_learnable=image_cross_attention_scale_learnable)
            for _ in range(depth)])
        for blk in self.transformer_blocks:
            blk.set_kind("spatial")
        self.proj_out = nn.Linear(inner_dim, in_channels) if use_linear else nn.Conv2d(inner_dim, in_channels, kernel_size=1, stride=1, padding=0)
        nn.init.zeros_(self.proj_out.weight)
        nn.init.zeros_(self.proj_out.bias)
        self.use_linear = use_linear

    def _foreign_params(self):
        return _last_ff_params(self)

    def _pack(self):
        win = self.proj_in.weight.detach().reshape(self.proj_in.weight.shape[0], -1)
        wout = self.proj_out.weight.detach().reshape(self.proj_out.weight.shape[0], -1)
        return dict(gn_w=_f32(self.norm.weight), gn_b=_f32(self.norm.bias), win=_f16(win), win32=_f32(win),
                    bin=_f32(self.proj_in.bias), wout=_f16(wout), bout=_f32(self.proj_out.bias))

    def project_context(self, ctx):
        return [project_context(blk.attn2, ctx) for blk in self.transformer_blocks]

    def _mx_route(self, x, context_kv, frames_per_video, cfg_repeat, N, D, pool=None):
        n, H, W, _ = x.shape
        if pool is not None:
            return None
        if not SATTN_MXFP8 or D in SATTN_MXFP8_SKIP_DIMS:
            return False
        attns = [a for blk in self.transformer_blocks for a in (blk.attn1, blk.attn2)]
        if any(a.to_out[0].bias is None or a.inner_dim != D or a.query_dim != D for a in attns):
            return False
        N_img, heads = H * W, self.n_heads
        for frames in sorted({frames_per_video, n, n * cfg_repeat}):
            tokens = frames * N
            if not (ops.linear_mxfp8_ok(tokens, 2 * D, D) and ops.linear_t_mxfp8_ok(tokens, D, D) and ops.linear_mxfp8_ok(tokens, D, D)
                    and ops.linear_mxfp8_ok(tokens, D, D, residual=True)
                    and ops.flash_attn_mxfp8_ok(n_groups=frames, heads=heads, nq=N, nk=N_img, kv_rows=N, kv_div=1, ldq=2 * D, ldk=2 * D, ldvt=tokens)):
                return False
            for kv in context_kv:
                nb = kv.n_txt_rows // 80
                if kv.k_img is not None:
                    ok = ops.flash_attn_dual_mxfp8_ok(n_groups=frames, heads=heads, nq=N, nk1=kv.n_txt, kv_rows1=80, kv_div1=frames_per_video, ldk1=D,
                                                      ldvt1=nb * 80, nk2=kv.n_img, kv_rows2=kv.n_img, kv_div2=1 if kv.img_per_frame else frames_per_video,
                                                      ldk2=D, ldvt2=kv.vt_img.shape[1], ldq=D)
                else:
                    ok = ops.flash_attn_mxfp8_ok(n_groups=frames, heads=heads, nq=N, nk=kv.n_txt, kv_rows=80, kv_div=frames_per_video, ldq=D, ldk=D,
                                                 ldvt=nb * 80)
                if not ok:
                    return False
        return True

    def forward(self, x, context_kv=None, frames_per_video=1, cfg_repeat=1, colstats=None, want_colstats=False, **kwargs):
        n, H, W, C = x.shape
        N_img = H * W
        pk = self.packed()
        pool = kv_pool_plan(H, W, pk["win"].shape[0])
        mx = self._mx_route(x, context_kv, frames_per_video, cfg_repeat, (N_img + 7) // 8 * 8, pk["win"].shape[0], pool)
        stats = None if colstats is None else ops.group_norm_stats_from_colstats(colstats, n, N_img, C)
        D_in = pk["win"].shape[0]
        fold = N_img % 8 == 0 and spatial_fold_ok(frames_per_video, N_img, C, D_in) and fold_extent_ok(n * N_img, max(C, D_in))
        a = None if fold else ops.group_norm(x.view(n, N_img, C), pk["gn_w"], pk["gn_b"], self.norm.eps, False, stats=stats)
        N = (N_img + 7) // 8 * 8
        xin = x.reshape(n * N_img, C)
        if N != N_img:
            def pad_frames(src):
                dst = torch.zeros((n * N, C), dtype=torch.float16, device=x.device)
                ops.copy2d(src, dst, n, N_img * C, N_img * C, N * C)
                return dst
            xin, a = pad_frames(xin), pad_frames(a.view(n * N_img, C))
        tokens = n * N
        if fold:
            if stats is None:
                stats = ops.group_norm_stats(x.view(n, N_img, C))
            wn, bn = ops.group_norm_fold_linear(pk["win32"], pk["bin"], pk["gn_w"], pk["gn_b"], stats, self.norm.eps)
        blk0 = self.transformer_blocks[0]
        rs_eps = blk0.norm1.eps
        rs = None
        video_rows = frames_per_video * N
        p1 = blk0.attn1.kv_pool_packed()["q"] if pool is not None else blk0.attn1.packed()["qk"]
        if not mx and _folded(p1, tokens, D_in, D_in) and ops.rowstats_ok(tokens, D_in, C, lda=C, unit_rows=N_img if fold else None,
                                                                                      video_rows=video_rows):
            rs = ops.rowstats_buffer(tokens, x.device)
        if fold:
            t = ops.gemm_units(xin, wn, bn, unit_rows=N_img, rowstats=rs, rowstats_eps=rs_eps)
        else:
            t = ops.linear(a.view(tokens, C), pk["win"], pk["bin"], rowstats=rs, rowstats_eps=rs_eps)
        D, heads = t.shape[1], self.n_heads
        for bi, (blk, kv) in enumerate(zip(self.transformer_blocks, context_kv)):
            ln = blk.ln_params()
            if mx:
                t, n, tokens, xin = _sattn_mx_block(blk, kv, ln, t, xin, n, N, N_img, D, heads, frames_per_video, cfg_repeat if bi == 0 else 1)
                if bi + 1 < len(self.transformer_blocks):
                    t = blk.ff.run(t, ln[2])
                continue
            a1, a2 = blk.attn1.packed(), blk.attn2.packed()
            pqk, pv, qk_alpha = a1["qk"], a1["v"], math.sqrt(blk.attn1.scale * ops.LOG2E)
            if pool is not None:
                o = _sattn_kv_pool(blk, ln[0], t, n, H, W, pool, heads, rs if bi == 0 else None)
            else:
                st = rs if (bi == 0 and rs is not None) else (ops.row_stats(t, ln[0][2]) if pqk["colsum"] is not None else None)
                qk = ln_linear(t, pqk, ln[0], alpha=qk_alpha, stats=st)
                vt = ln_linear_t(t, pv, ln[0], stats=st)
                o = torch.empty((tokens, D), dtype=torch.float16, device=x.device)
                ops.flash_attn(qk, qk[:, D:], vt, o, n_groups=n, heads=heads, nq=N, nk=N_img, kv_rows=N, kv_div=1, ldq=2 * D,
                               ldk=2 * D, ldvt=tokens, ldo=D, scale=blk.attn1.scale, log2_logits=True)
            st2 = ops.rowstats_buffer(tokens, x.device) if (_folded(a2["q"], tokens, D, D) and ops.rowstats_ok(tokens, D, D, ldr=D, video_rows=video_rows)) else None
            t = ops.linear(o, a1["wo"], a1["bo"], residual=t, rowstats=st2, rowstats_eps=ln[1][2])
            q2 = ln_linear(t, a2["q"], ln[1], alpha=blk.attn2.scale * ops.LOG2E, stats=st2)
            if bi == 0 and cfg_repeat > 1:
                t, q2, xin = ops.repeat_rows(t, cfg_repeat), ops.repeat_rows(q2, cfg_repeat), ops.repeat_rows(xin, cfg_repeat)
                n, tokens = n * cfg_repeat, tokens * cfg_repeat
            o2 = torch.empty((tokens, D), dtype=torch.float16, device=x.device)
            nb = kv.n_txt_rows // 80
            if kv.k_img is not None:
                ops.flash_attn_dual(q2, kv.k_txt, kv.vt_txt, kv.k_img, kv.vt_img, o2, n_groups=n, heads=heads, nq=N,
                                    nk1=kv.n_txt, kv_rows1=80, kv_div1=frames_per_video, ldk1=D, ldvt1=nb * 80,
                                    nk2=kv.n_img, kv_rows2=kv.n_img, kv_div2=1 if kv.img_per_frame else frames_per_video,
                                    ldk2=D, ldvt2=kv.vt_img.shape[1], ldq=D, ldo=D, scale=blk.attn2.scale, log2_logits=True)
            else:
                ops.flash_attn(q2, kv.k_txt, kv.vt_txt, o2, n_groups=n, heads=heads, nq=N, nk=kv.n_txt,
                               kv_rows=80, kv_div=frames_per_video, ldq=D, ldk=D, ldvt=nb * 80, ldo=D, scale=blk.attn2.scale,
                               log2_logits=True)
            t = ops.linear(o2, a2["wo"], a2["bo"], residual=t)
            if bi + 1 < len(self.transformer_blocks):
                t = blk.ff.run(t, ln[2])
        kw, cs_out = out_kwargs(None, want_colstats and N == N_img, tokens, N_img, D, C, x.device)
        out = ff_proj_out(self, t, ln[2], xin, kw, video_rows)
        if N != N_img:
            unpadded = torch.empty((n * N_img, C), dtype=torch.float16, device=x.device)
            ops.copy2d(out, unpadded, n, N_img * C, N * C, N_img * C)
            out = unpadded
        return out.view(n, H, W, C), cs_out


def _sattn_kv_pool(blk, lnp, t, n, H, W, pool, heads, rs):
    pp = blk.attn1.kv_pool_packed()
    tokens, D = t.shape
    N, Np = H * W, pool[0] * pool[1]
    alpha = math.sqrt(blk.attn1.scale * ops.LOG2E)
    q = ln_linear(t, pp["q"], lnp, alpha=alpha, stats=rs)
    p = ops.layer_norm_pool2x2(t, *lnp, n, H, W, _KV_POOL_MODES[SATTN_KV_POOL])
    k = ops.linear(p, pp["wk"], None, alpha=alpha)
    vt = ops.gemm(pp["wv"], p, M=D, N=n * Np, K=D, lda=D)
    o = torch.empty((tokens, D), dtype=torch.float16, device=t.device)
    return ops.flash_attn(q, k, vt, o, n_groups=n, heads=heads, nq=N, nk=Np, kv_rows=Np, kv_div=1, ldq=D, ldk=D, ldvt=n * Np, ldo=D,
                          scale=blk.attn1.scale, log2_logits=True)


def _sattn_mx_block(blk, kv, ln, t, xin, n, N, N_img, D, heads, frames_per_video, cfg_repeat):
    m1, m2 = blk.attn1.mx_packed(), blk.attn2.mx_packed()
    tokens = n * N
    an = ops.layer_norm_mxfp8(t, *ln[0])
    qk = ops.linear_mxfp8(an, m1["wqk"], m1["zero"], K=D)
    vt = ops.linear_t_mxfp8(an, m1["wv"], K=D)
    o = ops.flash_attn_mxfp8(qk, qk[:, D:], vt, n_groups=n, heads=heads, nq=N, nk=N_img, kv_rows=N, kv_div=1, ldq=2 * D, ldk=2 * D, ldvt=tokens,
                             scale=blk.attn1.scale)
    t = ops.linear_mxfp8(o, m1["wo"], m1["bo"], K=D, residual=t)
    an2 = ops.layer_norm_mxfp8(t, *ln[1])
    q2 = ops.linear_mxfp8(an2, m2["wq"], m2["zero"], K=D)
    if cfg_repeat > 1:
        t, q2, xin = ops.repeat_rows(t, cfg_repeat), ops.repeat_rows(q2, cfg_repeat), ops.repeat_rows(xin, cfg_repeat)
        n, tokens = n * cfg_repeat, tokens * cfg_repeat
    nb = kv.n_txt_rows // 80
    if kv.k_img is not None:
        o2 = ops.flash_attn_dual_mxfp8(q2, kv.k_txt, kv.vt_txt, kv.k_img, kv.vt_img, n_groups=n, heads=heads, nq=N, nk1=kv.n_txt, kv_rows1=80,
                                       kv_div1=frames_per_video, ldk1=D, ldvt1=nb * 80, nk2=kv.n_img, kv_rows2=kv.n_img,
                                       kv_div2=1 if kv.img_per_frame else frames_per_video, ldk2=D, ldvt2=kv.vt_img.shape[1], ldq=D, scale=blk.attn2.scale)
    else:
        o2 = ops.flash_attn_mxfp8(q2, kv.k_txt, kv.vt_txt, n_groups=n, heads=heads, nq=N, nk=kv.n_txt, kv_rows=80, kv_div=frames_per_video, ldq=D, ldk=D,
                                  ldvt=nb * 80, scale=blk.attn2.scale)
    t = ops.linear_mxfp8(o2, m2["wo"], m2["bo"], K=D, residual=t)
    return t, n, tokens, xin


class TemporalTransformer(PackedModule):

    def __init__(self, in_channels, n_heads, d_head, depth=1, dropout=0., context_dim=None, use_checkpoint=True,
                 use_linear=False, only_self_att=True, causal_attention=False, causal_block_size=1,
                 relative_position=False, temporal_length=None):
        super().__init__()
        if not only_self_att:
            raise NotImplementedError("ViewCrafter uses temporal self-attention only")
        if relative_position and temporal_length is None:
            raise AssertionError("relative_position needs temporal_length (reference attention.py:339)")
        if causal_attention and temporal_length is None:
            raise AssertionError("causal_attention needs temporal_length (reference attention.py:344)")
        self.causal_attention = bool(causal_attention)
        self.temporal_length = temporal_length
        self.only_self_att = only_self_att
        self.in_channels = in_channels
        inner_dim = n_heads * d_head
        self.n_heads = n_heads
        self.norm = nn.GroupNorm(num_groups=32, num_channels=in_channels, eps=1e-6, affine=True)
        if not use_linear:
            self.proj_in = nn.Conv1d(in_channels, inner_dim, kernel_size=1, stride=1, padding=0)
            self.proj_out = nn.Conv1d(inner_dim, in_channels, kernel_size=1, stride=1, padding=0)
        else:
            self.proj_in = nn.Linear(in_channels, inner_dim)
            self.proj_out = nn.Linear(inner_dim, in_channels)
        nn.init.zeros_(self.proj_out.weight)
        nn.init.zeros_(self.proj_out.bias)

        def attention_cls(**kw):
            return CrossAttention(temporal_length=temporal_length, relative_position=bool(relative_position), **kw)
        self.transformer_blocks = nn.ModuleList([
            BasicTransformerBlock(inner_dim, n_heads, d_head, dropout=dropout, context_dim=None,
                                  attention_cls=attention_cls, checkpoint=use_checkpoint) for _ in range(depth)])
        for blk in self.transformer_blocks:
            blk.set_kind("temporal")
        self.use_linear = use_linear

    def _foreign_params(self):
        return _last_ff_params(self)

    def _pack(self):
        win = self.proj_in.weight.detach().reshape(self.proj_in.weight.shape[0], -1)
        wout = self.proj_out.weight.detach().reshape(self.proj_out.weight.shape[0], -1)
        return dict(gn_w=_f32(self.norm.weight), gn_b=_f32(self.norm.bias), win=_f16(win), win32=_f32(win), bin=_f32(self.proj_in.bias),
                    wout=_f16(wout), bout=_f32(self.proj_out.bias))

    def _mx_route(self, x, D):
        B, T, P, _ = x.shape
        if not TATTN_MXFP8 or D in TATTN_MXFP8_SKIP_DIMS or T > 32 or not x.is_contiguous():
            return False
        attns = [a for blk in self.transformer_blocks for a in (blk.attn1, blk.attn2)]
        if any(a.relative_position or a.to_out[0].bias is None or a.inner_dim != D or a.query_dim != D for a in attns):
            return False
        return all(ops.linear_mxfp8_ok(b * T * P, 3 * D, D) and ops.linear_mxfp8_ok(b * T * P, D, D, residual=True)
                   and ops.temporal_attn_mxfp8_ok(b, T, P, self.n_heads, 3 * D, causal=self.causal_attention) for b in sorted({1, B}))

    def forward(self, x, context=None, colstats=None, want_colstats=False, target=None):
        B, T, P, C = x.shape
        pk = self.packed()
        tokens = B * T * P
        xin = x.reshape(tokens, C)
        D, heads = pk["win"].shape[0], self.n_heads
        mx = self._mx_route(x, D)
        stats = None if (colstats is None or GN_STATS_LEVEL < 2) else ops.group_norm_stats_from_colstats(colstats, B, T * P, C)
        rows = T * P
        if GN_FOLD and C % 64 == 0 and 2 * rows * C >= GN_FOLD_MIN_BYTES and 2 * rows * max(C, D) < 0xFFFF0000 and ops.tune_get("GEMM_DMA") != 0:
            if stats is None:
                stats = ops.group_norm_stats(x.view(B, rows, C))
            wn, bn = ops.group_norm_fold_linear(pk["win32"], pk["bin"], pk["gn_w"], pk["gn_b"], stats, self.norm.eps)
            fold = True
        else:
            a = ops.group_norm(x.view(B, rows, C), pk["gn_w"], pk["gn_b"], self.norm.eps, False, stats=stats)
            fold = False
        blk0 = self.transformer_blocks[0]
        st = None
        if not mx and _folded(blk0.attn1.packed()["qkv"], tokens, D, D) and ops.rowstats_ok(tokens, D, C, lda=C, unit_rows=rows if fold else None, video_rows=rows):
            st = ops.rowstats_buffer(tokens, x.device)
        if fold:
            t = ops.gemm_units(xin, wn, bn, unit_rows=rows, rowstats=st, rowstats_eps=blk0.norm1.eps)
        else:
            t = ops.linear(a.view(tokens, C), pk["win"], pk["bin"], rowstats=st, rowstats_eps=blk0.norm1.eps)
        for blk in self.transformer_blocks:
            ln = blk.ln_params()
            for ai, (attn, lnp) in enumerate(((blk.attn1, ln[0]), (blk.attn2, ln[1]))):
                if mx:
                    am = attn.mx_packed()
                    an = ops.layer_norm_mxfp8(t, *lnp)
                    qkv = ops.linear_mxfp8(an, am["wqkv"], am["zero"], K=D)
                    o = ops.temporal_attn_mxfp8(qkv, B=B, T=T, P=P, heads=heads, ld=3 * D, k_off=D, v_off=2 * D, scale=attn.scale,
                                                causal=self.causal_attention)
                    t = ops.linear_mxfp8(o, am["wo"], am["bo"], K=D, residual=t)
                    continue
                ap = attn.packed()
                qkv = ln_linear(t, ap["qkv"], lnp, stats=st)
                o = torch.empty((tokens, D), dtype=torch.float16, device=x.device)
                if attn.relative_position:
                    relg = torch.empty((tokens, heads, 64), dtype=torch.float16, device=x.device)
                    relp = torch.zeros((tokens, heads, 64), dtype=torch.float16, device=x.device)
                    for h_ in range(heads):
                        ops.gemm(qkv[:, h_ * 64:], ap["rel_k"], M=tokens, N=64, K=64, lda=3 * D, out=relg[:, h_], ldc=heads * 64)
                    ops.temporal_attn_rel(qkv, o, relg, relp, R=ap["rel_R"], B=B, T=T, P=P, heads=heads, ld=3 * D, k_off=D, v_off=2 * D, ldo=D,
                                          scale=attn.scale, causal=self.causal_attention)
                    for h_ in range(heads):
                        ops.gemm(relp[:, h_], ap["rel_v"], M=tokens, N=64, K=64, lda=heads * 64, out=o[:, h_ * 64:], ldc=D, residual=o[:, h_ * 64:], ldr=D)
                else:
                    ops.temporal_attn(qkv, o, B=B, T=T, P=P, heads=heads, ld=3 * D, k_off=D, v_off=2 * D, ldo=D,
                                      scale=attn.scale, causal=self.causal_attention)
                st = None
                if ai == 0 and _folded(blk.attn2.packed()["qkv"], tokens, D, D) and ops.rowstats_ok(tokens, D, D, ldr=D, video_rows=rows):
                    st = ops.rowstats_buffer(tokens, x.device)
                t = ops.linear(o, ap["wo"], ap["bo"], residual=t, rowstats=st, rowstats_eps=ln[1][2])
            if blk is not self.transformer_blocks[-1]:
                t = blk.ff.run(t, ln[2])
        kw, cs_out = out_kwargs(target, want_colstats, tokens, P, D, C, x.device)
        out = ff_proj_out(self, t, ln[2], xin, kw, rows)
        return out.view(B, T, P, -1), cs_out
```

### viewcrafter_amd/ops.py

```python
import ctypes
import os

import torch

from ._lib import (GEMM_BIAS_M, GEMM_BIAS_N, GEMM_COLSTATS, GEMM_CONV_SLABK, GEMM_GEGLU, GEMM_LNFOLD, GEMM_LNFOLD_T, GEMM_MXFP8_OUT, GEMM_OUT_F32, GEMM_RESIDUAL, GEMM_ROWADD, GEMM_ROWSTATS, PROF_FAMILIES,
                   ROUTE_UNITS_GROUPED, ROUTE_UNITS_LOOP, ROUTE_UNITS_WS320, TUNE, GemmDesc, VcxError, check, lib)
from .packing import conv_slab_major

_f16 = torch.float16
_f32 = torch.float32
LN_ROWSTATS = os.environ.get("VCX_LN_ROWSTATS", "1") != "0"


def _stream():
    return torch.cuda.current_stream().cuda_stream


def _ptr(t):
    return t.data_ptr() if t is not None else None


def _dev16(*tensors):
    for t in tensors:
        if t is not None and (t.dtype is not _f16 or not t.is_cuda):
            raise VcxError(f"expected a GPU fp16 tensor, got {t.dtype} on {t.device}")


def _dev32(*tensors):
    for t in tensors:
        if t is not None and (t.dtype is not _f32 or not t.is_cuda):
            raise VcxError(f"expected a GPU fp32 tensor, got {t.dtype} on {t.device}")


def require_gpu():
    if not torch.cuda.is_available():
        raise VcxError("viewcrafter_amd needs an MI355X (gfx950) GPU: torch.cuda.is_available() is False "
                       "and there is no CPU fallback")
    lib()


def _gemm_desc(M, N, K, lda, ldc, *, ldw=None, ldr=0, conv=None, tail=(), flags=0, alpha=1.0):
    ldw = K if ldw is None else ldw
    if max(M, N, K, ldw, ldc, ldr, conv["in_w"] if conv else 0) >= 1 << 31:
        raise VcxError(f"gemm: M={M} N={N} K={K} ldw={ldw} ldc={ldc} ldr={ldr} do not fit the descriptor's 32-bit fields")
    d = GemmDesc()
    d.lda, d.M, d.N, d.K, d.ldw, d.ldc, d.ldr = lda, M, N, K, ldw, ldc, ldr
    if conv is not None:
        d.mode = 1
        d.in_h, d.in_w, d.out_h, d.out_w = conv["in_h"], conv["in_w"], conv["out_h"], conv["out_w"]
        d.cin, d.kh, d.kw = conv["cin"], conv["kh"], conv["kw"]
        d.stride, d.pad_h, d.pad_w, d.ups = conv["stride"], conv["pad_h"], conv["pad_w"], conv.get("ups", 0)
        if conv.get("slabk", conv_slab_major(conv["cin"], conv["kh"] * conv["kw"])):
            flags |= GEMM_CONV_SLABK
    for j, (k, ld) in zip("01", tail):
        setattr(d, "tail_k" + j, k)
        setattr(d, "tail_lda" + j, ld)
    d.flags, d.alpha = flags, alpha
    return d


def _takes(M, N, K, lda, ldc, unit_rows=0, **kw):
    try:
        return lib().vcx_gemm_route(ctypes.byref(_gemm_desc(M, N, K, lda, ldc, **kw)), unit_rows) > 0
    except VcxError:
        return False


def gemm(a, w, *, M, N, K, lda, out=None, ldc=None, bias=None, bias_m=False, residual=None, ldr=None, rowadd=None,
         rowadd_div=0, geglu=False, out_f32=False, alpha=1.0, conv=None, ldw=None, ln_stats=None, ln_colsum=None, ln_t=False, colstats=None,
         colstats_ld=None, colstats_col=0, rowstats=None, rowstats_eps=1e-5, tail=None):
    n_out = N // 2 if geglu else N
    _dev16(a, w, residual)
    _dev32(bias, rowadd)
    if out is None:
        out = torch.empty((M, n_out), dtype=_f32 if out_f32 else _f16, device=a.device)
        ldc = n_out
    elif ldc is None:
        ldc = out.stride(0)
    if tail and len(tail) > 2:
        raise VcxError("gemm: a K tail has one or two sources")
    for j, t in enumerate(tail or ()):
        if t.dim() != 2 or t.shape[0] != M or t.stride(1) != 1:
            raise VcxError(f"gemm: tail source {j} must be [M = {M}, k] with unit column stride, got {tuple(t.shape)}")
    d = _gemm_desc(M, N, K, lda, ldc, ldw=ldw, conv=conv, tail=[(t.shape[1], t.stride(0)) for t in tail or ()], alpha=alpha)
    d.A, d.W, d.C = a.data_ptr(), w.data_ptr(), out.data_ptr()
    flags = d.flags
    if bias is not None:
        d.bias = bias.data_ptr()
        flags |= GEMM_BIAS_M if bias_m else GEMM_BIAS_N
    if rowadd is not None:
        if rowadd.dim() != 2 or rowadd.stride(1) != 1 or rowadd.shape[1] != n_out:
            raise VcxError(f"rowadd must be [rows, N = {n_out}] fp32 with unit column stride (a column slice of a wider matrix is fine), got {tuple(rowadd.shape)}")
        d.rowadd = rowadd.data_ptr()
        d.rowadd_div = rowadd_div
        d.rowadd_ld = rowadd.stride(0) if rowadd.shape[0] > 1 else n_out
        flags |= GEMM_ROWADD
    if residual is not None:
        d.residual = residual.data_ptr()
        d.ldr = ldr if ldr is not None else residual.stride(0)
        flags |= GEMM_RESIDUAL
    if geglu:
        flags |= GEMM_GEGLU
    if out_f32:
        flags |= GEMM_OUT_F32
    if ln_stats is not None:
        _dev32(ln_stats, ln_colsum)
        d.ln_stats, d.ln_colsum = ln_stats.data_ptr(), ln_colsum.data_ptr()
        flags |= GEMM_LNFOLD_T if ln_t else GEMM_LNFOLD
    if colstats is not None:
        _dev32(colstats)
        cld = n_out if colstats_ld is None else int(colstats_ld)
        if colstats.numel() != (M // 64) * cld * 2 or colstats_col < 0 or colstats_col + n_out > cld:
            raise VcxError(f"colstats must hold [M / 64, {cld}, 2] floats (M={M}, N={n_out}, first column {colstats_col}), got {tuple(colstats.shape)}")
        d.colstats = colstats.data_ptr() + 8 * int(colstats_col)
        d.ldcs = cld
        flags |= GEMM_COLSTATS
    if rowstats is not None:
        _dev32(rowstats)
        if rowstats.numel() != 2 * M or not rowstats.is_contiguous():
            raise VcxError(f"rowstats must hold [M = {M}, 2] floats, got {tuple(rowstats.shape)}")
        d.rowstats, d.rowstats_eps = rowstats.data_ptr(), float(rowstats_eps)
        flags |= GEMM_ROWSTATS
    if tail:
        _dev16(*tail)
        d.tail_a0 = tail[0].data_ptr()
        if len(tail) > 1:
            d.tail_a1 = tail[1].data_ptr()
    d.flags = flags
    check(lib().vcx_gemm_f16(ctypes.byref(d), _stream()), "vcx_gemm_f16")
    return out


def rowstats_ok(M, N, K, *, lda=None, ldc=None, ldr=0, unit_rows=None, video_rows=None):
    per_video = M if video_rows is None else video_rows
    if not LN_ROWSTATS or M < per_video:
        return False
    flags = GEMM_ROWSTATS | GEMM_BIAS_N | (GEMM_RESIDUAL if ldr else 0)
    lda, ldc = K if lda is None else lda, N if ldc is None else ldc
    calls = {per_video, M} | ({2 * per_video} if unit_rows else set())
    return all(_takes(m, N, K, lda, ldc, unit_rows or 0, ldr=ldr, flags=flags) for m in sorted(calls))


def rowstats_buffer(M, device):
    return torch.empty((M, 2), dtype=_f32, device=device)


def gemm_units(a, wn, bn, *, unit_rows, out=None, rowstats=None, rowstats_eps=1e-5):
    M, K = a.shape
    units, N, K2 = wn.shape
    _dev16(a, wn, out)
    _dev32(bn)
    if K2 != K or M != units * unit_rows or tuple(bn.shape) != (units, N) or not wn.is_contiguous() or not bn.is_contiguous():
        raise VcxError(f"gemm_units: a {tuple(a.shape)} / wn {tuple(wn.shape)} / bn {tuple(bn.shape)} do not describe {units} units of {unit_rows} rows")
    if out is None:
        out = torch.empty((M, N), dtype=_f16, device=a.device)
    d = _gemm_desc(M, N, K, a.stride(0), out.stride(0), flags=GEMM_BIAS_N)
    d.A, d.W, d.C, d.bias = a.data_ptr(), wn.data_ptr(), out.data_ptr(), bn.data_ptr()
    if rowstats is not None:
        _dev32(rowstats)
        if rowstats.numel() != 2 * M or not rowstats.is_contiguous():
            raise VcxError(f"rowstats must hold [M = {M}, 2] floats, got {tuple(rowstats.shape)}")
        d.rowstats, d.rowstats_eps = rowstats.data_ptr(), float(rowstats_eps)
        d.flags |= GEMM_ROWSTATS
    check(lib().vcx_gemm_units_f16(ctypes.byref(d), int(unit_rows), N * K, N, _stream()), "vcx_gemm_units_f16")
    return out


def units_route(M, N, K, unit_rows, *, lda=None, ldc=None):
    if unit_rows <= 0 or M <= 0 or M % unit_rows != 0:
        raise VcxError(f"units_route: M ({M}) must be a whole number of units of {unit_rows} rows")
    d = _gemm_desc(M, N, K, K if lda is None else lda, N if ldc is None else ldc, flags=GEMM_BIAS_N)
    route = lib().vcx_gemm_route(ctypes.byref(d), unit_rows)
    if route <= 0:
        raise VcxError("units_route: " + lib().vcx_last_error().decode("utf-8", "replace"))
    return {ROUTE_UNITS_WS320: "ws320", ROUTE_UNITS_GROUPED: "grouped", ROUTE_UNITS_LOOP: "loop"}.get(route, "single")


def units_one_launch_ok(M, N, K, unit_rows, *, lda=None, ldc=None):
    return units_route(M, N, K, unit_rows, lda=lda, ldc=ldc) in ("ws320", "grouped")


def lnfold_ok(rows, n_out, K, *, lda=None, ldc=None, transposed=False):
    lda = K if lda is None else lda
    if transposed:
        return _takes(n_out, rows, K, K, rows if ldc is None else ldc, ldw=lda, flags=GEMM_LNFOLD_T | GEMM_BIAS_M)
    return _takes(rows, n_out, K, lda, n_out if ldc is None else ldc, flags=GEMM_LNFOLD | GEMM_BIAS_N)


def linear(x, w, bias=None, **kw):
    rows, K = x.shape
    K += sum(t.shape[1] for t in kw.get("tail") or ())
    return gemm(x, w, M=rows, N=w.shape[0], K=K, lda=x.stride(0), bias=bias, **kw)


def linear_tail_ok(M, N, K, tail_ks, lda=None, ldc=None, residual=False, colstats=False):
    if not 0 < len(tail_ks) <= 2 or any(k <= 0 for k in tail_ks):
        return False
    flags = GEMM_BIAS_N | (GEMM_RESIDUAL if residual else 0) | (GEMM_COLSTATS if colstats else 0)
    return _takes(M, N, K + sum(tail_ks), K if lda is None else lda, N if ldc is None else ldc, ldr=N if residual else 0, tail=[(k, k) for k in tail_ks], flags=flags)


def conv2d(x, w, bias, *, kh, kw, stride=1, pad_h=None, pad_w=None, ups=0, out_hw=None, **kwargs):
    n, H, W, cin = x.shape
    if pad_h is None:
        pad_h = kh // 2
    if pad_w is None:
        pad_w = kw // 2
    if out_hw is None:
        He, We = H << ups, W << ups
        out_hw = ((He + 2 * pad_h - kh) // stride + 1, (We + 2 * pad_w - kw) // stride + 1)
    Ho, Wo = out_hw
    cout = w.shape[0]
    geom = dict(in_h=H, in_w=W, out_h=Ho, out_w=Wo, cin=cin, kh=kh, kw=kw, stride=stride, pad_h=pad_h, pad_w=pad_w,
                ups=ups)
    tail_k = sum(t.shape[1] for t in kwargs.get("tail") or ())
    out = gemm(x, w, M=n * Ho * Wo, N=cout, K=kh * kw * cin + tail_k, lda=x.stride(2), bias=bias, conv=geom, **kwargs)
    return out.view(n, Ho, Wo, -1)


UPS_FOLD = os.environ.get("VCX_UPS_FOLD", "1") != "0"


def _ups_folded_desc(n, H, W, cin, cout, lda, ldc, colstats):
    geom = dict(in_h=H, in_w=W, out_h=2 * H, out_w=2 * W, cin=cin, kh=2, kw=2, stride=1, pad_h=1, pad_w=1, ups=2)
    return dict(M=n * 4 * H * W, N=cout, K=4 * cin, lda=lda, ldc=ldc, conv=geom, flags=GEMM_BIAS_N | (GEMM_COLSTATS if colstats else 0))


def conv2d_ups_folded_ok(n, H, W, cin, cout, *, lda=None, ldc=None, colstats=False):
    if not UPS_FOLD:
        return False
    d = _ups_folded_desc(n, H, W, cin, cout, cin if lda is None else lda, cout if ldc is None else ldc, colstats)
    return _takes(d.pop("M"), d.pop("N"), d.pop("K"), d.pop("lda"), d.pop("ldc"), **d)


def conv2d_ups_folded(x, wf, bias, *, out=None, ldc=None, colstats=None, colstats_ld=None, colstats_col=0):
    n, H, W, cin = x.shape
    cout = wf.shape[1]
    if wf.dim() != 3 or wf.shape[0] != 4 or wf.shape[2] != 4 * cin or not wf.is_contiguous():
        raise VcxError(f"conv2d_ups_folded: weights must be contiguous [4, Cout, 4 * {cin}], got {tuple(wf.shape)}")
    geom = _ups_folded_desc(n, H, W, cin, cout, 0, 0, False)["conv"]
    res = gemm(x, wf, M=n * 4 * H * W, N=cout, K=4 * cin, lda=x.stride(2), bias=bias, conv=geom, out=out, ldc=ldc, colstats=colstats,
               colstats_ld=colstats_ld, colstats_col=colstats_col)
    return res.view(n, 2 * H, 2 * W, -1)


def _rows_geom(M, in_rows, cin, taps):
    return dict(in_h=1, in_w=M if in_rows is None else in_rows, out_h=1, out_w=M, cin=cin, kh=taps, kw=1, stride=1, pad_h=0, pad_w=0)


def conv_tail_ok(M, cin, cout, taps, tail_ks, in_rows=None):
    return (0 < len(tail_ks) <= 2 and all(k > 0 for k in tail_ks)
            and _takes(M, cout, taps * cin + sum(tail_ks), cin, cout, conv=_rows_geom(M, in_rows, cin, taps), tail=[(k, k) for k in tail_ks]))


def temporal_conv3(x, w, bias, **kwargs):
    B, T, P, C = x.shape
    geom = dict(in_h=T, in_w=P, out_h=T, out_w=P, cin=C, kh=3, kw=1, stride=1, pad_h=1, pad_w=0, ups=0)
    out = gemm(x, w, M=B * T * P, N=w.shape[0], K=3 * C, lda=x.stride(2), bias=bias, conv=geom, **kwargs)
    return out.view(B, T, P, -1)


def colstats_ok(M, pixels, cin, cout, in_rows=None):
    return (pixels % 64 == 0 and M % 64 == 0
            and _takes(M, cout, cin, cin, cout, conv=None if in_rows is None else _rows_geom(M, in_rows, cin, 1), flags=GEMM_COLSTATS))


def colstats_buffer(M, cout, device):
    return torch.empty((M // 64, cout, 2), dtype=_f32, device=device)

# ... 679 lines not shown
```

Measured before the change: 5.667 DDIM steps/s.

## Emit per-80-column partial row moments from tiled GEMM epilogue for LN folding

Extends the ROWSTATS producer epilogue to the tiled DMA GEMM at N=640/1280, so each 80-column block writes partial mean and M2 per row. A new LNFOLD_PARTS consumer mode merges these partial moments in-kernel with permlane swaps to form mean and rstd. The aim is to remove the standalone layernorm/rowstats pass before the FF and proj_out GEMMs at the wider transformer levels. This adds more template instantiations, register pressure and routing complexity, plus a new buffer layout.

```diff
diff --git a/include/vcx.h b/include/vcx.h
--- a/include/vcx.h
+++ b/include/vcx.h
@@ -30,6 +30,7 @@
 #define VCX_GEMM_LNFOLD_T 0x100
 #define VCX_GEMM_COLSTATS 0x200
 #define VCX_GEMM_ROWSTATS 0x400
+#define VCX_GEMM_LNFOLD_PARTS 0x1000
 #define VCX_GEMM_MXFP8_OUT 0x800
 
 typedef struct vcx_gemm_desc {
diff --git a/viewcrafter_amd/_lib.py b/viewcrafter_amd/_lib.py
--- a/viewcrafter_amd/_lib.py
+++ b/viewcrafter_amd/_lib.py
@@ -25,7 +25,7 @@
 TUNE = {"GEMM_CFG": (0, -1), "GEMM_DMA": (1, 1), "FLASH_QB": (2, 0), "XATTN_RESIDENT": (3, 1), "FLASH_IMPL": (4, 0), "EXP0": (5, 0),
         "EXP1": (6, 0), "GEMM_WS": (7, 1)}
 GEMM_BIAS_N, GEMM_BIAS_M, GEMM_ROWADD, GEMM_RESIDUAL, GEMM_GEGLU, GEMM_OUT_F32, GEMM_CONV_SLABK = 1, 2, 4, 8, 16, 32, 64
-GEMM_LNFOLD, GEMM_LNFOLD_T, GEMM_COLSTATS, GEMM_ROWSTATS, GEMM_MXFP8_OUT = 0x80, 0x100, 0x200, 0x400, 0x800
+GEMM_LNFOLD, GEMM_LNFOLD_T, GEMM_COLSTATS, GEMM_ROWSTATS, GEMM_MXFP8_OUT, GEMM_LNFOLD_PARTS = 0x80, 0x100, 0x200, 0x400, 0x800, 0x1000
 ROUTE_REFUSED, ROUTE_REGISTER, ROUTE_TILED, ROUTE_WS320, ROUTE_WS320_GEGLU, ROUTE_WS320_LNF, ROUTE_UNITS_WS320, ROUTE_UNITS_GROUPED, ROUTE_UNITS_LOOP = range(9)
 PROF_FAMILIES = ("gemm", "flash_attn", "temporal_attn", "groupnorm", "layernorm", "elementwise")
 
diff --git a/viewcrafter_amd/csrc/gemm.hip b/viewcrafter_amd/csrc/gemm.hip
--- a/viewcrafter_amd/csrc/gemm.hip
+++ b/viewcrafter_amd/csrc/gemm.hip
@@ -346,7 +346,7 @@
 
 struct TileSeg { int cfg, m_begin, rows, grid; };
 struct TilePlan { int n; TileSeg seg[2]; float cost; };
-enum { EPI_PLAIN = 0, EPI_GEGLU = 1, EPI_PLAIN_ONLY128 = 2, EPI_GEGLU_ONLY128 = 3 };
+enum { EPI_PLAIN = 0, EPI_GEGLU = 1, EPI_PLAIN_ONLY128 = 2, EPI_GEGLU_ONLY128 = 3, EPI_ROWSTATS = 4 };
 
 struct TileCost {
     int tbm, tbn, bpc;
@@ -485,6 +485,7 @@
         VCX_REQUIRE(lnf == 1 ? !(flags & VCX_GEMM_BIAS_M) : !(flags & VCX_GEMM_BIAS_N) && !geglu,
                     "vcx_gemm_f16: LNFOLD takes BIAS_N (and GEGLU), LNFOLD_T takes BIAS_M");
         VCX_REQUIRE((lnf == 1 ? d->N : d->M) % 4 == 0 && (lnf == 1 ? d->N : d->M) >= 4, "vcx_gemm_f16: LNFOLD needs the colsum side to be a multiple of 4");
+        VCX_REQUIRE(!(flags & VCX_GEMM_LNFOLD_PARTS) || d->rowstats_eps >= 0.f, "vcx_gemm_f16: LNFOLD_PARTS forms rstd with rowstats_eps, which must be >= 0");
     }
     if (flags & VCX_GEMM_COLSTATS) {
         VCX_REQUIRE(!ptrs || (d->colstats && ((uintptr_t)d->colstats & 15) == 0), "vcx_gemm_f16: COLSTATS needs a 16-byte aligned colstats buffer");
@@ -584,6 +585,9 @@
     const bool dma_ok = k.dma != 0 && d.K % 64 == 0 && d.N % ((geglu || f32) ? 4 : 8) == 0 && (!conv || d.cin % 64 == 0) &&
                         r.a_bytes < lim && r.w_bytes < lim && (!geglu || d.N >= 64) && out_ok && r.a2_bytes < lim && r.a3_bytes < lim;
     const bool force_cfg_unset = k.cfg < 0;
+    const bool rsp = (flags & VCX_GEMM_ROWSTATS) && dma_ok && !conv && !geglu && !f32 && !lnf && (d.N == 640 || d.N == 1280) && d.K != 320 &&
+                     !(flags & ~(VCX_GEMM_ROWSTATS | VCX_GEMM_BIAS_N | VCX_GEMM_RESIDUAL)) && (k.cfg < 0 || k.cfg == 1 || k.cfg == 3);
+    if (rsp) r.epi = EPI_ROWSTATS;
 
     const int units = unit_rows > 0 ? d.M / unit_rows : 1;
     if (unit_rows > 0 && (k2 || k3)) return refuse(r, "vcx_gemm_units_f16: no K tail (tail_k0 / tail_k1) with per-unit weights");
@@ -591,14 +595,16 @@
         if (d.K == 320 && d.N == 320 && unit_rows % 32 == 0 && unit_rows >= 1024 && d.M >= 8192 && r.a_bytes < lim && c_ok && units <= 65535 &&
             k.dma != 0 && k.ws != 0 && force_cfg_unset)
             return take(r, VCX_ROUTE_UNITS_WS320);
-        if (flags & VCX_GEMM_ROWSTATS)
-            return refuse(r, "vcx_gemm_units_f16: ROWSTATS needs the one-launch weight-stationary form (N = K = 320, unit_rows %% 32 == 0, >= 1024, M >= 8192); M=%d N=%d K=%d unit_rows=%d",
-                          d.M, d.N, d.K, unit_rows);
+        if ((flags & VCX_GEMM_ROWSTATS) && !rsp)
+            return refuse(r, "vcx_gemm_units_f16: ROWSTATS needs the one-launch weight-stationary form (N = K = 320, unit_rows %% 32 == 0, >= 1024, M >= 8192), or at "
+                             "N = 640 / 1280 the tiled engine's per-unit form; M=%d N=%d K=%d unit_rows=%d", d.M, d.N, d.K, unit_rows);
         if (units <= 65535 && d.K % 64 == 0 && d.N % 8 == 0 && r.a_bytes < lim && r.w_bytes < lim && c_ok && k.dma != 0 && k.cfg <= 5 && !k.units_loop) {
             vcx_gemm_desc one = d;
             one.M = unit_rows;
+            one.flags &= ~VCX_GEMM_ROWSTATS;
             if (gemm_route(one, 0, k).kind != VCX_ROUTE_WS320) return take(r, VCX_ROUTE_UNITS_GROUPED);
         }
+        if (rsp) return refuse(r, "vcx_gemm_units_f16: ROWSTATS at N = %d needs the tiled engine's per-unit form (VCX_GEMM_UNITS_LOOP unset); unit_rows=%d", d.N, unit_rows);
         return take(r, VCX_ROUTE_UNITS_LOOP);
     }
 
@@ -617,8 +623,8 @@
     if ((k2 || k3) && !dma_ok)
         return refuse(r, "vcx_gemm_f16: a K tail needs the DMA kernel (cin %% 64 == 0, K %% 64 == 0, N %% 8 == 0, extents < 4 GiB); cin=%d K=%d N=%d", d.cin, d.K, d.N);
     if (!conv && (k2 || k3)) {
-        if (geglu || f32 || lnf || (flags & VCX_GEMM_ROWSTATS))
-            return refuse(r, "vcx_gemm_f16: a linear K tail takes the plain and COLSTATS epilogues only: no GEGLU / LNFOLD / ROWSTATS / fp32 output; flags=0x%x", flags);
+        if (geglu || f32 || lnf || ((flags & VCX_GEMM_ROWSTATS) && !rsp))
+            return refuse(r, "vcx_gemm_f16: a linear K tail takes the plain and COLSTATS epilogues only: no GEGLU / LNFOLD / fp32 output, ROWSTATS at N = 640 / 1280 only; flags=0x%x", flags);
         if (k.cfg > 5) return refuse(r, "vcx_gemm_f16: tile configuration %d (knob GEMM_CFG) has no K tail in linear mode", k.cfg);
         return take(r, VCX_ROUTE_TILED);
     }
@@ -634,9 +640,12 @@
     if (dma_ok && !conv && !geglu && !f32 && !lnf && d.K == 320 && d.N % 320 == 0 && d.N <= 1280 && d.M >= 8192 && rs_ok &&
         !(flags & VCX_GEMM_BIAS_M) && k.ws != 0 && force_cfg_unset)
         return take(r, VCX_ROUTE_WS320);
-    if (flags & VCX_GEMM_ROWSTATS)
-        return refuse(r, "vcx_gemm_f16: ROWSTATS needs the weight-stationary kernel (linear, N = K = 320, M >= 8192, BIAS_N / RESIDUAL at most, knob GEMM_WS on); M=%d N=%d K=%d flags=0x%x",
+    if ((flags & VCX_GEMM_ROWSTATS) && !rsp)
+        return refuse(r, "vcx_gemm_f16: ROWSTATS needs the weight-stationary kernel (linear, N = K = 320, M >= 8192, BIAS_N / RESIDUAL at most, knob GEMM_WS on), or at "
+                         "N = 640 / 1280 the tiled engine (linear, K %% 64 == 0, K != 320, BIAS_N / RESIDUAL / K tail at most, GEMM_CFG unset, 1 or 3); M=%d N=%d K=%d flags=0x%x",
                       d.M, d.N, d.K, flags);
+    if ((flags & VCX_GEMM_LNFOLD_PARTS) && !(dma_ok && lnf == 1 && (d.K == 640 || d.K == 1280)))
+        return refuse(r, "vcx_gemm_f16: LNFOLD_PARTS (row statistics from partial moments) needs LNFOLD on the DMA kernel at K = 640 or 1280; K=%d flags=0x%x", d.K, flags);
     if (dma_ok) {
         if (k.cfg > 6) return refuse(r, "vcx_gemm_f16: unknown tile configuration %d (knob GEMM_CFG)", k.cfg);
         return take(r, VCX_ROUTE_TILED);
diff --git a/viewcrafter_amd/csrc/gemm_dma.hip b/viewcrafter_amd/csrc/gemm_dma.hip
--- a/viewcrafter_amd/csrc/gemm_dma.hip
+++ b/viewcrafter_amd/csrc/gemm_dma.hip
@@ -202,6 +202,7 @@
     __builtin_amdgcn_s_waitcnt(0x0f70 | 0);
     __syncthreads();
     int cur = 0;
+    [[maybe_unused]] float ln_m4[LNF == 4 ? MFRAG : 1] = {}, ln_s4[LNF == 4 ? MFRAG : 1] = {};
     for (;;) {
         if (++lkt == nk) {
             lkt = 0;
@@ -214,6 +215,15 @@
         const half_t* cx = sX + cur * TBM * BK;
         const half_t* cw = sW + cur * BN * BK;
         [[maybe_unused]] float ln_r0[LNF ? MFRAG : 1], ln_r1[LNF ? MFRAG : 1];
+        [[maybe_unused]] f4 ln_p[2];
+        [[maybe_unused]] const int ln_b = ckt - (nk - MFRAG);
+        if (LNF == 4 && ln_b >= 0) {
+            const int nblk = p.K / 80, per = nblk >> 2;
+            const int mc = min(p.m_begin + tile_m * TBM + wm * WM + lr + ln_b * 16, p.M - 1);
+            const f4* src = reinterpret_cast<const f4*>(p.ln_stats + ((size_t)mc * (size_t)nblk + (size_t)(lg * per)) * 2);
+            ln_p[0] = src[0];
+            ln_p[1] = src[per == 4 ? 1 : 0];
+        }
         if ((LNF == 1 || LNF == 2) && ckt == nk - 1) {
             const int mrow = p.m_begin + tile_m * TBM + wm * WM + lr;
 #pragma unroll
@@ -257,6 +267,57 @@
                     }
                     wcur = wnext;
                     __builtin_amdgcn_sched_barrier(0);
+                }
+            }
+        }
+        if constexpr (LNF == 4) {
+            if (ln_b >= 0) {
+                auto merge = [](float& ma, float& qa, float mb, float qb, float half_n) {
+                    float d = mb - ma;
+                    float q = qa + qb;
+                    asm("" : "+v"(d), "+v"(q));
+                    float e = d * d;
+                    asm("" : "+v"(e));
+                    ma = __builtin_fmaf(0.5f, d, ma);
+                    qa = __builtin_fmaf(e, half_n, q);
+                    asm("" : "+v"(ma), "+v"(qa));
+                };
+                auto swap16 = [](float x, float& lo, float& hi) {
+                    const unsigned xi = __builtin_bit_cast(unsigned, x);
+                    const auto s = __builtin_amdgcn_permlane16_swap(xi, xi, false, false);
+                    lo = __builtin_bit_cast(float, (unsigned)s[0]);
+                    hi = __builtin_bit_cast(float, (unsigned)s[1]);
+                };
+                auto swap32 = [](float x, float& lo, float& hi) {
+                    const unsigned xi = __builtin_bit_cast(unsigned, x);
+                    const auto s = __builtin_amdgcn_permlane32_swap(xi, xi, false, false);
+                    lo = __builtin_bit_cast(float, (unsigned)s[0]);
+                    hi = __builtin_bit_cast(float, (unsigned)s[1]);
+                };
+                const bool four = p.K == 1280;
+                const float lane_half = four ? 160.f : 80.f;
+                const float inv_k = four ? 1.0f / 1280.0f : 1.0f / 640.0f;
+                float m = ln_p[0][0], q = ln_p[0][1];
+                merge(m, q, ln_p[0][2], ln_p[0][3], 40.f);
+                if (four) {
+                    float m1 = ln_p[1][0], q1 = ln_p[1][1];
+                    merge(m1, q1, ln_p[1][2], ln_p[1][3], 40.f);
+                    merge(m, q, m1, q1, 80.f);
+                }
+                float ma, mb, qa, qb;
+                swap16(m, ma, mb);
+                swap16(q, qa, qb);
+                merge(ma, qa, mb, qb, lane_half);
+                swap32(ma, m, mb);
+                swap32(qa, q, qb);
+                merge(m, q, mb, qb, 2.f * lane_half);
+                float var = __builtin_fmaf(q, inv_k, p.rowstats_eps);
+                asm("" : "+v"(var));
+                const float rstd = __builtin_amdgcn_rsqf(var);
+#pragma unroll
+                for (int b = 0; b < MFRAG; ++b) {
+                    ln_m4[b] = ln_b == b ? m : ln_m4[b];
+                    ln_s4[b] = ln_b == b ? rstd : ln_s4[b];
                 }
             }
         }
@@ -270,7 +331,7 @@
                 q.M = p.m_begin + (cu + 1) * p.unit_rows;
                 q.bias = p.bias + (int64_t)cu * p.bias_unit_stride;
                 q.c_bytes = (unsigned)(2ull * ((unsigned long long)(q.M - 1) * (unsigned)p.ldc + (unsigned)p.N));
-                gemm_epilogue<Cfg, false, false, 0>(q, acc, 0, tile_n, wm, wn, lane, sB);
+                gemm_epilogue<Cfg, false, false, LNF == 5 ? 5 : 0>(q, acc, 0, tile_n, wm, wn, lane, sB);
             } else if constexpr (UPSF) {
                 int cu, crow0;
                 unit_of(tile_m, cu, crow0);
@@ -278,7 +339,8 @@
                                                                    crow0 - (p.m_begin + cu * p.unit_rows));
             } else
             gemm_epilogue<Cfg, GEGLU, OUT_F32, LNF>(p, acc, tile_m, tile_n, wm, wn, lane, sB,
-                                                    reinterpret_cast<float*>(smem_raw + Cfg::STAGES + Cfg::STRIP) + wave * WN, ln_r0, ln_r1);
+                                                    reinterpret_cast<float*>(smem_raw + Cfg::STAGES + Cfg::STRIP) + wave * WN, LNF == 4 ? ln_m4 : ln_r0,
+                                                    LNF == 4 ? ln_s4 : ln_r1);
 #pragma unroll
             for (int a = 0; a < NFRAG; ++a)
 #pragma unroll
@@ -303,7 +365,7 @@
 int launch(const GemmArgs& a, hipStream_t s, int grid) {
     static VcxLdsAttr lds;
     auto kern = gemm_dma_kernel<Cfg, CONV, GEGLU, OUT_F32, LNF, TAIL, UNITS, UPSF>;
-    constexpr size_t smem = LNF ? Cfg::SMEM_LNF : Cfg::SMEM;
+    constexpr size_t smem = (LNF && LNF != 5) ? Cfg::SMEM_LNF : Cfg::SMEM;
     if (!lds.ensure(reinterpret_cast<const void*>(kern), (int)smem, "vcx_gemm_f16(dma)")) return VCX_ELAUNCH;
     const int blocks_per_cu = Cfg::SMEM > 80 * 1024 ? 1 : 2;
     const int nb = grid > 0 ? grid : persistent_grid(a.tiles_m * a.tiles_n, blocks_per_cu);
@@ -313,6 +375,15 @@
 
 template <class Cfg>
 int dispatch(const GemmArgs& a, bool conv, bool geglu, bool f32, hipStream_t s, int grid) {
+    if (a.flags & VCX_GEMM_ROWSTATS) {
+        if constexpr ((Cfg::TBN / Cfg::NWN) % 80 == 0) {
+            if (a.unit_rows > 0) return launch<Cfg, false, false, false, 5, false, true>(a, s, grid);
+            if (a.k2 + a.k3 > 0) return launch<Cfg, false, false, false, 5, true>(a, s, grid);
+            return launch<Cfg, false, false, false, 5>(a, s, grid);
+        }
+        vcx_set_error("vcx_gemm_f16(dma): ROWSTATS needs a tile configuration whose wave strip is whole 80-column blocks (128 x 160, 256 x 320)");
+        return VCX_EINVAL;
+    }
     if (a.unit_rows > 0 && conv)
         return (a.flags & VCX_GEMM_COLSTATS) ? launch<Cfg, true, false, false, 3, false, false, true>(a, s, grid) : launch<Cfg, true, false, false, 0, false, false, true>(a, s, grid);
     if (a.unit_rows > 0)
@@ -323,8 +394,9 @@
     }
     if (a.flags & (VCX_GEMM_LNFOLD | VCX_GEMM_LNFOLD_T)) {
         if (a.flags & VCX_GEMM_LNFOLD_T) return launch<Cfg, false, false, false, 2>(a, s, grid);
-        if (!geglu) return launch<Cfg, false, false, false, 1>(a, s, grid);
-        if constexpr (Cfg::NF % 4 == 0) return launch<Cfg, false, true, false, 1>(a, s, grid);
+        const bool parts = a.flags & VCX_GEMM_LNFOLD_PARTS;
+        if (!geglu) return parts ? launch<Cfg, false, false, false, 4>(a, s, grid) : launch<Cfg, false, false, false, 1>(a, s, grid);
+        if constexpr (Cfg::NF % 4 == 0) return parts ? launch<Cfg, false, true, false, 4>(a, s, grid) : launch<Cfg, false, true, false, 1>(a, s, grid);
         vcx_set_error("vcx_gemm_f16(dma): GEGLU needs whole 64-column packed blocks per wave");
         return VCX_EINVAL;
     }
@@ -358,8 +430,9 @@
 template <class Cfg>
 int dispatch_tail(const GemmArgs& a, bool conv, bool geglu, bool f32, hipStream_t s, int grid) {
     const bool cs = a.flags & VCX_GEMM_COLSTATS;
-    if (f32 || (a.flags & VCX_GEMM_LNFOLD_T)) {
-        vcx_set_error("vcx_gemm_f16(dma): the 64-row tile configurations have no fp32-output / LNFOLD_T epilogue");
+    [[maybe_unused]] const bool parts = a.flags & VCX_GEMM_LNFOLD_PARTS;
+    if (f32 || (a.flags & (VCX_GEMM_LNFOLD_T | VCX_GEMM_ROWSTATS))) {
+        vcx_set_error("vcx_gemm_f16(dma): the 64-row tile configurations have no fp32-output / LNFOLD_T / ROWSTATS epilogue");
         return VCX_EINVAL;
     }
     if (a.unit_rows > 0 && conv) {
@@ -372,7 +445,8 @@
             return VCX_EINVAL;
         }
         if (geglu && !conv && a.k2 + a.k3 == 0 && !cs)
-            return (a.flags & VCX_GEMM_LNFOLD) ? launch_tail<Cfg, false, true, 1>(a, s, grid) : launch_tail<Cfg, false, true>(a, s, grid);
+            return (a.flags & VCX_GEMM_LNFOLD) ? (parts ? launch_tail<Cfg, false, true, 4>(a, s, grid) : launch_tail<Cfg, false, true, 1>(a, s, grid))
+                                               : launch_tail<Cfg, false, true>(a, s, grid);
         vcx_set_error("vcx_gemm_f16(dma): this 64-row tile configuration is for GEGLU projections (linear) only");
         return VCX_EINVAL;
     } else {
@@ -386,7 +460,7 @@
             if (conv) return cs ? launch_tail<Cfg, true, false, 3, true>(a, s, grid) : launch_tail<Cfg, true, false, 0, true>(a, s, grid);
             return cs ? launch_tail<Cfg, false, false, 3, true>(a, s, grid) : launch_tail<Cfg, false, false, 0, true>(a, s, grid);
         }
-        if (a.flags & VCX_GEMM_LNFOLD) return launch_tail<Cfg, false, false, 1>(a, s, grid);
+        if (a.flags & VCX_GEMM_LNFOLD) return parts ? launch_tail<Cfg, false, false, 4>(a, s, grid) : launch_tail<Cfg, false, false, 1>(a, s, grid);
         if (cs) return conv ? launch_tail<Cfg, true, false, 3>(a, s, grid) : launch_tail<Cfg, false, false, 3>(a, s, grid);
         return conv ? launch_tail<Cfg, true, false>(a, s, grid) : launch_tail<Cfg, false, false>(a, s, grid);
     }
diff --git a/viewcrafter_amd/csrc/gemm_epilogue.h b/viewcrafter_amd/csrc/gemm_epilogue.h
--- a/viewcrafter_amd/csrc/gemm_epilogue.h
+++ b/viewcrafter_amd/csrc/gemm_epilogue.h
@@ -32,13 +32,14 @@
         }
 }
 
-template <class Cfg, bool GEGLU, bool OUT_F32, int LNF = 0, bool RPRE = false, bool UPSF = false>
+template <class Cfg, bool GEGLU, bool OUT_F32, int LNF_ = 0, bool RPRE = false, bool UPSF = false>
 __device__ __forceinline__ void gemm_epilogue(const GemmArgs& p, f4 (&acc)[Cfg::NF][Cfg::MF], int tile_m, int tile_n, int wm, int wn,
                                               int lane, float* sB, [[maybe_unused]] float* sS = nullptr,
                                               [[maybe_unused]] const float* ln_r0 = nullptr, [[maybe_unused]] const float* ln_r1 = nullptr,
                                               [[maybe_unused]] const epi_u4v* rpre = nullptr,
                                               bool strip_ready = false,
                                               [[maybe_unused]] int ups_cls = 0, [[maybe_unused]] int ups_q0 = 0) {
+    constexpr int LNF = LNF_ == 4 ? 1 : LNF_;
     constexpr int TBM = Cfg::TBM, BN = Cfg::TBN, NFRAG = Cfg::NF, MFRAG = Cfg::MF;
     constexpr int WM = TBM / Cfg::NWM, WN = BN / Cfg::NWN;
     [[maybe_unused]] constexpr unsigned OOB = EPI_OOB;
@@ -168,6 +169,11 @@
                     for (int r = 0; r < 4; ++r) t[r] += rv[r];
                 }
                 *reinterpret_cast<f4*>(sB + lane * 4) = t;
+                if (LNF_ == 4) {
+                    f4 cs = *reinterpret_cast<const f4*>(p.ln_colsum + nc);
+                    *reinterpret_cast<f4*>(sS + lane * 4) = cs;
+                    asm volatile("s_nop 1" : : "v"(t), "v"(cs) : "memory");
+                } else
                 if (LNF == 1) *reinterpret_cast<f4*>(sS + lane * 4) = *reinterpret_cast<const f4*>(p.ln_colsum + nc);
             }
         }
@@ -192,6 +198,38 @@
 #pragma unroll
                 for (int e = 0; e < 8; ++e) gs[u][e] = gq[u][e] = 0.f;
         }
+        constexpr bool RSP = LNF == 5;
+        static_assert(!RSP || (WN % 80 == 0 && !OUT_F32 && !UPSF), "partial row moments: whole 80-column blocks per wave strip, fp16 output");
+        constexpr int RBLK = RSP ? WN / 80 : 1;
+        [[maybe_unused]] float rs_s[RBLK], rs_q[RBLK], rs_k[RBLK];
+        [[maybe_unused]] auto rs_lanes = [](float x) {
+            const unsigned xi = __builtin_bit_cast(unsigned, x);
+            const auto s = __builtin_amdgcn_permlane16_swap(xi, xi, false, false);
+            float y = __builtin_bit_cast(float, (unsigned)s[0]) + __builtin_bit_cast(float, (unsigned)s[1]);
+            asm("" : "+v"(y));
+            const unsigned yi = __builtin_bit_cast(unsigned, y);
+            const auto t = __builtin_amdgcn_permlane32_swap(yi, yi, false, false);
+            float z = __builtin_bit_cast(float, (unsigned)t[0]) + __builtin_bit_cast(float, (unsigned)t[1]);
+            asm("" : "+v"(z));
+            return z;
+        };
+        [[maybe_unused]] auto rs_frag = [&](int f, const float (&w)[4]) {
+            const int k = f / 5;
+            if (f % 5 == 0) {
+                const unsigned wi = __builtin_bit_cast(unsigned, w[0]);
+                const unsigned s = __builtin_amdgcn_permlane16_swap(wi, wi, false, false)[0];
+                rs_k[k] = __builtin_bit_cast(float, (unsigned)__builtin_amdgcn_permlane32_swap(s, s, false, false)[0]);
+                rs_s[k] = rs_q[k] = 0.f;
+            }
+#pragma unroll
+            for (int r = 0; r < 4; ++r) {
+                float d = w[r] - rs_k[k];
+                asm("" : "+v"(d));
+                rs_s[k] += d;
+                rs_q[k] = __builtin_fmaf(d, d, rs_q[k]);
+                asm("" : "+v"(rs_s[k]), "+v"(rs_q[k]));
+            }
+        };
         int bopaque = 0;
         auto finish = [&](int a, int b, float (&v)[4]) {
             if (FOLD) {
@@ -289,6 +327,19 @@
                         gq[u][4 + r] = __builtin_fmaf(d1, d1, gq[u][4 + r]);
                     }
                 }
+                if (RSP) {
+                    unsigned q0 = pk0[0], q1 = pk0[1], q2 = pk1[0], q3 = pk1[1];
+                    asm volatile("" : "+v"(q0), "+v"(q1), "+v"(q2), "+v"(q3));
+                    pk0 = u2v{q0, q1};
+                    pk1 = u2v{q2, q3};
+                    typedef _Float16 h2v __attribute__((ext_vector_type(2)));
+                    const h2v a01 = __builtin_bit_cast(h2v, q0), a23 = __builtin_bit_cast(h2v, q1);
+                    const h2v b01 = __builtin_bit_cast(h2v, q2), b23 = __builtin_bit_cast(h2v, q3);
+                    const float w0[4] = {(float)a01[0], (float)a01[1], (float)a23[0], (float)a23[1]};
+                    const float w1[4] = {(float)b01[0], (float)b01[1], (float)b23[0], (float)b23[1]};
+                    rs_frag(a, w0);
+                    if (wide) rs_frag(a + 1, w1);
+                }
                 if (OUT_F32) {
                     __builtin_amdgcn_raw_buffer_store_b128(__builtin_bit_cast(u4v, f4{v0[0], v0[1], v0[2], v0[3]}), srd_c, voff, 0, 0);
                 } else {
@@ -303,6 +354,24 @@
                         __builtin_amdgcn_raw_buffer_store_b64(p0, srd_c, voff, 0, 0);
                     }
                 }
+            }
+            if (RSP) {
+                const int m = mbase + b * 16;
+                float mo = 0.f, qo = 0.f;
+#pragma unroll
+                for (int k = 0; k < RBLK; ++k) {
+                    const float s1 = rs_lanes(rs_s[k]), s2 = rs_lanes(rs_q[k]);
+                    float mean = __builtin_fmaf(s1, 1.0f / 80.0f, rs_k[k]);
+                    float t = -s1 * (1.0f / 80.0f);
+                    asm("" : "+v"(mean), "+v"(t));
+                    float m2 = __builtin_fmaf(t, s1, s2);
+                    asm("" : "+v"(m2));
+                    m2 = m2 > 0.f ? m2 : 0.f;
+                    mo = lg == k ? mean : mo;
+                    qo = lg == k ? m2 : qo;
+                }
+                if (lg < RBLK && m < p.M && nstrip + lg * 80 < p.N)
+                    *reinterpret_cast<float2*>(p.rowstats + ((size_t)m * (size_t)(p.N / 80) + (size_t)(nstrip / 80 + lg)) * 2) = make_float2(mo, qo);
             }
         }
         if (LNF == 3) {
diff --git a/viewcrafter_amd/lvdm/modules/attention.py b/viewcrafter_amd/lvdm/modules/attention.py
--- a/viewcrafter_amd/lvdm/modules/attention.py
+++ b/viewcrafter_amd/lvdm/modules/attention.py
@@ -75,6 +75,16 @@
     return pj["colsum"] is not None and ops.lnfold_ok(rows, pj["w"].shape[0], K, lda=lda, transposed=transposed)
 
 
+def _producer_stats(want, tokens, D, K, device, **kw):
+    if not (want and ops.rowstats_ok(tokens, D, K, **kw)):
+        return None
+    return ops.rowstats_parts_buffer(tokens, device, D) if D in ops.ROWSTATS_PART_WIDTHS else ops.rowstats_buffer(tokens, device)
+
+
+def _parts_eps(st, eps):
+    return dict(ln_eps=eps) if st.dim() == 3 else {}
+
+
 def _ln_projection(w, ln, alpha=1.0, bias=None):
     if ln is not None:
         wf, colsum, bias_f = fold_layernorm(w, ln.weight, ln.bias, None)
@@ -97,7 +107,7 @@
     rows, K = t.shape
     if pj["colsum"] is not None and ops.lnfold_ok(rows, pj["w"].shape[0], K, lda=t.stride(0)):
         st = stats if stats is not None else ops.row_stats(t, lnp[2])
-        return ops.linear(t, pj["w"], pj["bias"], alpha=alpha, ln_stats=st, ln_colsum=pj["colsum"], **kw)
+        return ops.linear(t, pj["w"], pj["bias"], alpha=alpha, ln_stats=st, ln_colsum=pj["colsum"], **_parts_eps(st, lnp[2]), **kw)
     w, bias = (pj["w"], pj["bias"]) if pj["colsum"] is None else _plain_of(pj)
     return ops.linear(ops.layer_norm(t, *lnp), w, bias, alpha=alpha, **kw)
 
@@ -289,17 +299,22 @@
     def on_fp16_route(self, t):
         return not (FF_MXFP8 and self._mx_ok(t))
 
-    def glu(self, t, ln_params):
+    def folded(self, t):
         pk = self.packed()
-        if pk["colsum"] is not None and ops.lnfold_ok(t.shape[0], pk["w1"].shape[0], t.shape[1], lda=t.stride(0)):
-            return ops.linear(t, pk["w1"], pk["b1"], geglu=True, ln_stats=ops.row_stats(t, ln_params[2]), ln_colsum=pk["colsum"])
+        return pk["colsum"] is not None and ops.lnfold_ok(t.shape[0], pk["w1"].shape[0], t.shape[1], lda=t.stride(0))
+
+    def glu(self, t, ln_params, stats=None):
+        pk = self.packed()
+        if self.folded(t):
+            st = stats if stats is not None else ops.row_stats(t, ln_params[2])
+            return ops.linear(t, pk["w1"], pk["b1"], geglu=True, ln_stats=st, ln_colsum=pk["colsum"], **_parts_eps(st, ln_params[2]))
         if pk["colsum"] is not None and "w1_plain" not in pk:
             proj = self.net[0].proj
             pk["w1_plain"], pk["b1_plain"] = pack_geglu(_f16(proj.weight), _f32(proj.bias))
         w1, b1 = (pk["w1"], pk["b1"]) if pk["colsum"] is None else (pk["w1_plain"], pk["b1_plain"])
         return ops.linear(ops.layer_norm(t, *ln_params), w1, b1, geglu=True)
 
-    def run(self, t, ln_params):
+    def run(self, t, ln_params, stats=None):
         pk = self.packed()
         if FF_MXFP8 and self._mx_ok(t):
             if "mx" not in pk:
@@ -310,7 +325,7 @@
             a = ops.layer_norm_mxfp8(t, *ln_params)
             g = ops.linear_mxfp8(a, mx["w1"], mx["b1"], K=self.dim, geglu=True, mx_out=True)
             return ops.linear_mxfp8(g, mx["w2"], pk["b2"], K=pk["w2"].shape[1], residual=t)
-        return ops.linear(self.glu(t, ln_params), pk["w2"], pk["b2"], residual=t)
+        return ops.linear(self.glu(t, ln_params, stats), pk["w2"], pk["b2"], residual=t)
 
 
 class BasicTransformerBlock(PackedModule):
@@ -351,7 +366,7 @@
         return self.packed()
 
 
-def ff_proj_out(tr, t, ln_params, xin, kw, video_rows):
+def ff_proj_out(tr, t, ln_params, xin, kw, video_rows, stats=None):
     pk, ff = tr.packed(), tr.transformer_blocks[-1].ff
     tokens, D = t.shape
     C = pk["wout"].shape[0]
@@ -359,10 +374,10 @@
             and all(ops.linear_tail_ok(m, C, ff.net[2].in_features, [D], ldc=kw.get("ldc"), residual=True, colstats="colstats" in kw)
                     for m in sorted({video_rows, tokens})))
     if not fold:
-        return ops.linear(ff.run(t, ln_params), pk["wout"], pk["bout"], residual=xin, **kw)
+        return ops.linear(ff.run(t, ln_params, stats), pk["wout"], pk["bout"], residual=xin, **kw)
     if "wcat" not in pk:
         pk["wcat"], pk["bcat"] = pack_ff_out_folded(ff.net[2].weight, ff.net[2].bias, pk["wout"], pk["bout"])
-    return ops.linear(ff.glu(t, ln_params), pk["wcat"], pk["bcat"], tail=[t], residual=xin, **kw)
+    return ops.linear(ff.glu(t, ln_params, stats), pk["wcat"], pk["bcat"], tail=[t], residual=xin, **kw)
 
 
 def _last_ff_params(tr):
@@ -486,14 +501,15 @@
         rs = None
         video_rows = frames_per_video * N
         p1 = blk0.attn1.kv_pool_packed()["q"] if pool is not None else blk0.attn1.packed()["qk"]
-        if not mx and _folded(p1, tokens, D_in, D_in) and ops.rowstats_ok(tokens, D_in, C, lda=C, unit_rows=N_img if fold else None,
-                                                                                      video_rows=video_rows):
-            rs = ops.rowstats_buffer(tokens, x.device)
+        if not mx:
+            rs = _producer_stats(_folded(p1, tokens, D_in, D_in), tokens, D_in, C, x.device, lda=C, unit_rows=N_img if fold else None, video_rows=video_rows,
+                                 parts=pool is not None)
         if fold:
             t = ops.gemm_units(xin, wn, bn, unit_rows=N_img, rowstats=rs, rowstats_eps=rs_eps)
         else:
             t = ops.linear(a.view(tokens, C), pk["win"], pk["bin"], rowstats=rs, rowstats_eps=rs_eps)
         D, heads = t.shape[1], self.n_heads
+        st3 = None
         for bi, (blk, kv) in enumerate(zip(self.transformer_blocks, context_kv)):
             ln = blk.ln_params()
             if mx:
@@ -512,7 +528,7 @@
                 o = torch.empty((tokens, D), dtype=torch.float16, device=x.device)
                 ops.flash_attn(qk, qk[:, D:], vt, o, n_groups=n, heads=heads, nq=N, nk=N_img, kv_rows=N, kv_div=1, ldq=2 * D,
                                ldk=2 * D, ldvt=tokens, ldo=D, scale=blk.attn1.scale, log2_logits=True)
-            st2 = ops.rowstats_buffer(tokens, x.device) if (_folded(a2["q"], tokens, D, D) and ops.rowstats_ok(tokens, D, D, ldr=D, video_rows=video_rows)) else None
+            st2 = _producer_stats(_folded(a2["q"], tokens, D, D), tokens, D, D, x.device, ldr=D, video_rows=video_rows)
             t = ops.linear(o, a1["wo"], a1["bo"], residual=t, rowstats=st2, rowstats_eps=ln[1][2])
             q2 = ln_linear(t, a2["q"], ln[1], alpha=blk.attn2.scale * ops.LOG2E, stats=st2)
             if bi == 0 and cfg_repeat > 1:
@@ -529,11 +545,12 @@
                 ops.flash_attn(q2, kv.k_txt, kv.vt_txt, o2, n_groups=n, heads=heads, nq=N, nk=kv.n_txt,
                                kv_rows=80, kv_div=frames_per_video, ldq=D, ldk=D, ldvt=nb * 80, ldo=D, scale=blk.attn2.scale,
                                log2_logits=True)
-            t = ops.linear(o2, a2["wo"], a2["bo"], residual=t)
+            st3 = _producer_stats(blk.ff.on_fp16_route(t) and blk.ff.folded(t), tokens, D, D, x.device, ldr=D, video_rows=video_rows)
+            t = ops.linear(o2, a2["wo"], a2["bo"], residual=t, rowstats=st3, rowstats_eps=ln[2][2])
             if bi + 1 < len(self.transformer_blocks):
-                t = blk.ff.run(t, ln[2])
+                t = blk.ff.run(t, ln[2], st3)
         kw, cs_out = out_kwargs(None, want_colstats and N == N_img, tokens, N_img, D, C, x.device)
-        out = ff_proj_out(self, t, ln[2], xin, kw, video_rows)
+        out = ff_proj_out(self, t, ln[2], xin, kw, video_rows, st3)
         if N != N_img:
             unpadded = torch.empty((n * N_img, C), dtype=torch.float16, device=x.device)
             ops.copy2d(out, unpadded, n, N_img * C, N * C, N_img * C)
@@ -656,8 +673,8 @@
             fold = False
         blk0 = self.transformer_blocks[0]
         st = None
-        if not mx and _folded(blk0.attn1.packed()["qkv"], tokens, D, D) and ops.rowstats_ok(tokens, D, C, lda=C, unit_rows=rows if fold else None, video_rows=rows):
-            st = ops.rowstats_buffer(tokens, x.device)
+        if not mx:
+            st = _producer_stats(_folded(blk0.attn1.packed()["qkv"], tokens, D, D), tokens, D, C, x.device, lda=C, unit_rows=rows if fold else None, video_rows=rows)
         if fold:
             t = ops.gemm_units(xin, wn, bn, unit_rows=rows, rowstats=st, rowstats_eps=blk0.norm1.eps)
         else:
@@ -688,12 +705,12 @@
                 else:
                     ops.temporal_attn(qkv, o, B=B, T=T, P=P, heads=heads, ld=3 * D, k_off=D, v_off=2 * D, ldo=D,
                                       scale=attn.scale, causal=self.causal_attention)
+                want = _folded(blk.attn2.packed()["qkv"], tokens, D, D) if ai == 0 else (blk.ff.on_fp16_route(t) and blk.ff.folded(t))
+                st = _producer_stats(want, tokens, D, D, x.device, ldr=D, video_rows=rows)
+                t = ops.linear(o, ap["wo"], ap["bo"], residual=t, rowstats=st, rowstats_eps=ln[ai + 1][2])
+            if blk is not self.transformer_blocks[-1]:
+                t = blk.ff.run(t, ln[2], st)
                 st = None
-                if ai == 0 and _folded(blk.attn2.packed()["qkv"], tokens, D, D) and ops.rowstats_ok(tokens, D, D, ldr=D, video_rows=rows):
-                    st = ops.rowstats_buffer(tokens, x.device)
-                t = ops.linear(o, ap["wo"], ap["bo"], residual=t, rowstats=st, rowstats_eps=ln[1][2])
-            if blk is not self.transformer_blocks[-1]:
-                t = blk.ff.run(t, ln[2])
         kw, cs_out = out_kwargs(target, want_colstats, tokens, P, D, C, x.device)
-        out = ff_proj_out(self, t, ln[2], xin, kw, rows)
+        out = ff_proj_out(self, t, ln[2], xin, kw, rows, st)
         return out.view(B, T, P, -1), cs_out
diff --git a/viewcrafter_amd/ops.py b/viewcrafter_amd/ops.py
--- a/viewcrafter_amd/ops.py
+++ b/viewcrafter_amd/ops.py
@@ -1,15 +1,17 @@
 import ctypes
+import math
 import os
 
 import torch
 
-from ._lib import (GEMM_BIAS_M, GEMM_BIAS_N, GEMM_COLSTATS, GEMM_CONV_SLABK, GEMM_GEGLU, GEMM_LNFOLD, GEMM_LNFOLD_T, GEMM_MXFP8_OUT, GEMM_OUT_F32, GEMM_RESIDUAL, GEMM_ROWADD, GEMM_ROWSTATS, PROF_FAMILIES,
+from ._lib import (GEMM_BIAS_M, GEMM_BIAS_N, GEMM_COLSTATS, GEMM_CONV_SLABK, GEMM_GEGLU, GEMM_LNFOLD, GEMM_LNFOLD_PARTS, GEMM_LNFOLD_T, GEMM_MXFP8_OUT, GEMM_OUT_F32, GEMM_RESIDUAL, GEMM_ROWADD, GEMM_ROWSTATS, PROF_FAMILIES,
                    ROUTE_UNITS_GROUPED, ROUTE_UNITS_LOOP, ROUTE_UNITS_WS320, TUNE, GemmDesc, VcxError, check, lib)
 from .packing import conv_slab_major
 
 _f16 = torch.float16
 _f32 = torch.float32
 LN_ROWSTATS = os.environ.get("VCX_LN_ROWSTATS", "1") != "0"
+ROWSTATS_PART_WIDTHS = (640, 1280)
 
 
 def _stream():
@@ -68,7 +70,7 @@
 
 def gemm(a, w, *, M, N, K, lda, out=None, ldc=None, bias=None, bias_m=False, residual=None, ldr=None, rowadd=None,
          rowadd_div=0, geglu=False, out_f32=False, alpha=1.0, conv=None, ldw=None, ln_stats=None, ln_colsum=None, ln_t=False, colstats=None,
-         colstats_ld=None, colstats_col=0, rowstats=None, rowstats_eps=1e-5, tail=None):
+         colstats_ld=None, colstats_col=0, rowstats=None, rowstats_eps=1e-5, tail=None, ln_eps=1e-5):
     n_out = N // 2 if geglu else N
     _dev16(a, w, residual)
     _dev32(bias, rowadd)
@@ -107,6 +109,11 @@
         _dev32(ln_stats, ln_colsum)
         d.ln_stats, d.ln_colsum = ln_stats.data_ptr(), ln_colsum.data_ptr()
         flags |= GEMM_LNFOLD_T if ln_t else GEMM_LNFOLD
+        if ln_stats.dim() == 3:
+            if ln_t or tuple(ln_stats.shape) != (M, K // 80, 2) or not ln_stats.is_contiguous() or rowstats is not None:
+                raise VcxError(f"partial row moments serve VCX_GEMM_LNFOLD only, as a contiguous [M = {M}, K / 80 = {K // 80}, 2] buffer; got {tuple(ln_stats.shape)}")
+            d.rowstats_eps = float(ln_eps)
+            flags |= GEMM_LNFOLD_PARTS
     if colstats is not None:
         _dev32(colstats)
         cld = n_out if colstats_ld is None else int(colstats_ld)
@@ -117,8 +124,9 @@
         flags |= GEMM_COLSTATS
     if rowstats is not None:
         _dev32(rowstats)
-        if rowstats.numel() != 2 * M or not rowstats.is_contiguous():
-            raise VcxError(f"rowstats must hold [M = {M}, 2] floats, got {tuple(rowstats.shape)}")
+        want = (M, N // 80, 2) if N in ROWSTATS_PART_WIDTHS else (M, 2)
+        if rowstats.numel() != math.prod(want) or not rowstats.is_contiguous():
+            raise VcxError(f"rowstats (VCX_GEMM_ROWSTATS) must hold {list(want)} floats (M = {M}, N = {N}), got {tuple(rowstats.shape)}")
         d.rowstats, d.rowstats_eps = rowstats.data_ptr(), float(rowstats_eps)
         flags |= GEMM_ROWSTATS
     if tail:
@@ -131,9 +139,9 @@
     return out
 
 
-def rowstats_ok(M, N, K, *, lda=None, ldc=None, ldr=0, unit_rows=None, video_rows=None):
+def rowstats_ok(M, N, K, *, lda=None, ldc=None, ldr=0, unit_rows=None, video_rows=None, parts=True):
     per_video = M if video_rows is None else video_rows
-    if not LN_ROWSTATS or M < per_video:
+    if not LN_ROWSTATS or M < per_video or (N in ROWSTATS_PART_WIDTHS and not parts):
         return False
     flags = GEMM_ROWSTATS | GEMM_BIAS_N | (GEMM_RESIDUAL if ldr else 0)
     lda, ldc = K if lda is None else lda, N if ldc is None else ldc
@@ -143,6 +151,10 @@
 
 def rowstats_buffer(M, device):
     return torch.empty((M, 2), dtype=_f32, device=device)
+
+
+def rowstats_parts_buffer(M, device, N):
+    return torch.empty((M, N // 80, 2), dtype=_f32, device=device)
 
 
 def gemm_units(a, wn, bn, *, unit_rows, out=None, rowstats=None, rowstats_eps=1e-5):
@@ -158,8 +170,9 @@
     d.A, d.W, d.C, d.bias = a.data_ptr(), wn.data_ptr(), out.data_ptr(), bn.data_ptr()
     if rowstats is not None:
         _dev32(rowstats)
-        if rowstats.numel() != 2 * M or not rowstats.is_contiguous():
-            raise VcxError(f"rowstats must hold [M = {M}, 2] floats, got {tuple(rowstats.shape)}")
+        want = (M, N // 80, 2) if N in ROWSTATS_PART_WIDTHS else (M, 2)
+        if rowstats.numel() != math.prod(want) or not rowstats.is_contiguous():
+            raise VcxError(f"rowstats (VCX_GEMM_ROWSTATS) must hold {list(want)} floats (M = {M}, N = {N}), got {tuple(rowstats.shape)}")
         d.rowstats, d.rowstats_eps = rowstats.data_ptr(), float(rowstats_eps)
         d.flags |= GEMM_ROWSTATS
     check(lib().vcx_gemm_units_f16(ctypes.byref(d), int(unit_rows), N * K, N, _stream()), "vcx_gemm_units_f16")
@@ -180,11 +193,11 @@
     return units_route(M, N, K, unit_rows, lda=lda, ldc=ldc) in ("ws320", "grouped")
 
 
-def lnfold_ok(rows, n_out, K, *, lda=None, ldc=None, transposed=False):
+def lnfold_ok(rows, n_out, K, *, lda=None, ldc=None, transposed=False, parts=False):
     lda = K if lda is None else lda
     if transposed:
         return _takes(n_out, rows, K, K, rows if ldc is None else ldc, ldw=lda, flags=GEMM_LNFOLD_T | GEMM_BIAS_M)
-    return _takes(rows, n_out, K, lda, n_out if ldc is None else ldc, flags=GEMM_LNFOLD | GEMM_BIAS_N)
+    return _takes(rows, n_out, K, lda, n_out if ldc is None else ldc, flags=GEMM_LNFOLD | GEMM_BIAS_N | (GEMM_LNFOLD_PARTS if parts else 0))
 
 
 def linear(x, w, bias=None, **kw):
```

Measured after the change: 5.679 DDIM steps/s (median of 6 runs). About the same (+0.2%).
